# LuoweiZhou/VLP

Hardware: AMD Instinct MI355X
Metric: samples/sec/node (COCO 100-region, seq64, bs64xN) fp16 (higher is better)
Workload: dtype f16; 1 GPU; COCO Captions fine-tune shape: BERT-base 12L, 100 regions x 2048-d, seq_len 64 (L=167), bs 64/GPU, fwd+bwd+FP16 FusedAdam, dropout 0.1, dynamic loss scale; global_batch=64, parallelism=dp1, batch_pool=8, skipped_steps=0, rccl_ranks=1, optimizer=replicated, first_leg_packed=False

## Files before the change

include/vlp_hip.h:

```cpp
#ifndef VLP_HIP_H
#define VLP_HIP_H

#include <stdint.h>

#ifdef __cplusplus
extern "C" {
#endif

#define VLP_ABI_VERSION 5

typedef enum {
    VLP_OK = 0,
    VLP_ERR_BAD_ARG = -1,
    VLP_ERR_HIP = -2,
    VLP_ERR_WORKSPACE = -3
} vlp_status;

enum { VLP_ACT_NONE = 0, VLP_ACT_GELU = 1, VLP_ACT_RELU = 2, VLP_ACT_TANH = 3,
       VLP_ACT_GELU_SAVE_GRAD = 4  };
enum { VLP_MUL_NONE = 0, VLP_MUL_GELU_GRAD = 1, VLP_MUL_RELU_MASK = 2, VLP_MUL_PLAIN = 3  };

int vlp_version(void);
const char* vlp_last_error_string(void);
int vlp_lab_build(void);
void vlp_debug_device_lookup_stats(unsigned long long* lookups, unsigned long long* driver_queries);

typedef struct {
    const void* X; int64_t ldx;
    const void* W; int64_t ldw;
    void* Y; int64_t ldy;
    const void* bias;
    const void* residual; int64_t ldr;
    void* preact; int64_t ldp;
    const void* mul_src; int64_t ldm;
    int32_t M, N, K;
    int32_t act;
    int32_t mul_mode;
    float alpha;
    float dropout_p; uint64_t seed; uint32_t rng_stream;
    int32_t variant;
    const int32_t* row_map;
} vlp_gemm_nt_args;
int vlp_gemm_nt(const vlp_gemm_nt_args* a, void* stream);
int vlp_gemm_nt_resolved_variant(void);
int64_t vlp_gemm_nt_splitk_workspace_bytes(int32_t M, int32_t N, int32_t splits);
int vlp_gemm_nt_splitk(const vlp_gemm_nt_args* a, int32_t splits, void* workspace, int64_t workspace_bytes, void* stream);

typedef struct {
    const void* A; int64_t lda;
    const void* B; int64_t ldb;
    void* C; int64_t ldc;
    int32_t M, N, K;
    int32_t beta;
    void* workspace; int64_t workspace_bytes;
    int32_t variant;
    int32_t splits;
    void* bias_out;
} vlp_gemm_tn_args;
int64_t vlp_gemm_tn_workspace_bytes(int32_t M, int32_t N, int32_t K);
int vlp_gemm_tn(const vlp_gemm_tn_args* a, void* stream);
int vlp_gemm_tn_grouped(const vlp_gemm_tn_args* list, int32_t count, void* stream);
int64_t vlp_gemm_tn_grouped_workspace_bytes(int32_t tiles);

typedef struct {
    const void* A; int64_t lda; int32_t M, N;
    void* out;
    int32_t beta;
    void* workspace; int64_t workspace_bytes;
} vlp_colsum_args;
int64_t vlp_colsum_workspace_bytes(int32_t M, int32_t N);
int vlp_colsum(const vlp_colsum_args* a, void* stream);

typedef struct {
    const void* qkv; int64_t ld_qkv;
    const uint8_t* mask;
    void* ctx; int64_t ld_ctx;
    float* lse;
    int32_t B, L, heads;
    float scale;
    float dropout_p; uint64_t seed; uint32_t rng_stream;
    const int32_t* row_off;
} vlp_attn_fwd_args;
int vlp_attn_fwd(const vlp_attn_fwd_args* a, void* stream);

typedef struct {
    const void* q; int64_t ld_q; int64_t q_rows_per_batch;
    const void* k; const void* v; int64_t ld_kv; int64_t kv_rows_per_batch;
    const uint8_t* mask;
    void* ctx; int64_t ld_ctx;
    int32_t B, Lq, Lk, heads;
    float scale;
    const void* k_prefix; const void* v_prefix;
    int64_t prefix_rows_per_batch;
    int32_t n_prefix, beams;
} vlp_attn_decode_args;
int vlp_attn_decode(const vlp_attn_decode_args* a, void* stream);

typedef struct {
    const void* qkv; int64_t ld_qkv;
    const uint8_t* mask;
    const uint8_t* mask_t;
    const void* ctx; int64_t ld_ctx;
    const void* dctx; int64_t ld_dctx;
    const float* lse;
    void* dqkv; int64_t ld_dqkv;
    float* delta;
    int32_t B, L, heads;
    float scale;
    float dropout_p; uint64_t seed; uint32_t rng_stream;
    const int32_t* row_off;
} vlp_attn_bwd_args;
int vlp_attn_bwd(const vlp_attn_bwd_args* a, void* stream);

int vlp_mask_pack(const int64_t* mask, uint8_t* out, uint8_t* out_t, int32_t B, int32_t L, int32_t Lp, void* stream);

typedef struct {
    const void* x; int64_t ldx;
    const void* gamma; const void* beta;
    void* y; int64_t ldy;
    float* mean; float* rstd;
    int32_t M, H; float eps;
    float dropout_p; uint64_t seed; uint32_t rng_stream;
    const int32_t* row_map;
} vlp_layernorm_fwd_args;
int vlp_layernorm_fwd(const vlp_layernorm_fwd_args* a, void* stream);

typedef struct {
    const void* dy; int64_t lddy;
    const void* x; int64_t ldx;
    const void* gamma;
    const float* mean; const float* rstd;
    void* dx; int64_t lddx;
    void* dx_drop; int64_t lddxd;
    void* dgamma; void* dbeta;
    int32_t M, H; int32_t beta;
    float dy_drop_p; uint64_t dy_seed; uint32_t dy_stream;
    float out_drop_p; uint64_t out_seed; uint32_t out_stream;
    void* workspace; int64_t workspace_bytes;
    int32_t defer_reduce;
    const int32_t* row_map;
} vlp_layernorm_bwd_args;
int64_t vlp_layernorm_bwd_workspace_bytes(int32_t H);
int vlp_layernorm_bwd(const vlp_layernorm_bwd_args* a, void* stream);
int vlp_layernorm_bwd_reduce_batched(const float* parts, const void* const* dst, int32_t count, int32_t M, int32_t H, int32_t beta, void* stream);

int vlp_region_mask_build(const int64_t* vis_masked_pos, int32_t B, int32_t Pm, int32_t Nv, uint8_t* out, void* stream);
typedef struct {
    const void* vis_h; const void* vispe_h;
    const void* pooled;
    const int64_t* vis_masked_pos;
    float* probs;
    float* sample_loss;
    float* loss;
    int32_t B, Nv, Pm, H;
} vlp_pretext_fwd_args;
int vlp_pretext_fwd(const vlp_pretext_fwd_args* a, void* stream);
typedef struct {
    const void* vis_h; const void* vispe_h; const void* pooled;
    const int64_t* vis_masked_pos;
    const float* probs;
    const float* gscale;
    void* d_vis_h; void* d_vispe_h;
    void* d_pooled_pre;
    int32_t B, Nv, Pm, H;
    float drop_p; uint64_t seed; uint32_t vis_stream; uint32_t vispe_stream;
} vlp_pretext_bwd_args;
int vlp_pretext_bwd(const vlp_pretext_bwd_args* a, void* stream);

typedef struct {
    const int64_t* input_ids; const int64_t* segment_ids;
    const void* word_emb; const void* pos_emb; const void* type_emb;
    const void* vis_h; const void* vispe_h;
    void* pre;
    int32_t B, L, Nv, H, vocab, type_vocab;
    const int64_t* position_ids;
    int32_t max_pos;
    const uint8_t* region_mask;
    const int32_t* row_map; int32_t rows;
} vlp_embed_fwd_args;
int vlp_embed_fwd(const vlp_embed_fwd_args* a, void* stream);

int64_t vlp_embed_bwd_workspace_floats(int32_t B, int32_t L, int32_t Nv, int32_t H);
typedef struct {
    const void* dpre;
    const int64_t* input_ids; const int64_t* segment_ids;
    const void* vis_h; const void* vispe_h;
    void* d_word_emb; void* d_pos_emb; void* d_type_emb;
    void* d_vis_h; void* d_vispe_h;
    float* acc32;
    int32_t B, L, Nv, H, vocab, type_vocab;
    float drop_p; uint64_t seed; uint32_t vis_stream; uint32_t vispe_stream;
    const uint8_t* region_mask;
    int32_t parts;
} vlp_embed_bwd_args;
int vlp_embed_bwd(const vlp_embed_bwd_args* a, void* stream);
typedef struct {
// ... 240 lines not shown
```

vlp_amd/_lib.py:

```python
import ctypes as C
import os

import torch

_HERE = os.path.dirname(os.path.abspath(__file__))
LIB_PATH = os.environ.get("VLP_HIP_LIB") or os.path.join(_HERE, "libvlp_hip.so")

ACT_NONE, ACT_GELU, ACT_RELU, ACT_TANH, ACT_GELU_SAVE_GRAD = 0, 1, 2, 3, 4
MUL_NONE, MUL_GELU_GRAD, MUL_RELU_MASK, MUL_PLAIN = 0, 1, 2, 3

vp, i64, i32, f32, u64, u32 = C.c_void_p, C.c_int64, C.c_int32, C.c_float, C.c_uint64, C.c_uint32


class GemmNtArgs(C.Structure):
    _fields_ = [("X", vp), ("ldx", i64), ("W", vp), ("ldw", i64), ("Y", vp), ("ldy", i64), ("bias", vp),
                ("residual", vp), ("ldr", i64), ("preact", vp), ("ldp", i64), ("mul_src", vp), ("ldm", i64),
                ("M", i32), ("N", i32), ("K", i32), ("act", i32), ("mul_mode", i32), ("alpha", f32),
                ("dropout_p", f32), ("seed", u64), ("rng_stream", u32), ("variant", i32), ("row_map", vp)]


class GemmTnArgs(C.Structure):
    _fields_ = [("A", vp), ("lda", i64), ("B", vp), ("ldb", i64), ("C", vp), ("ldc", i64),
                ("M", i32), ("N", i32), ("K", i32), ("beta", i32), ("workspace", vp), ("workspace_bytes", i64),
                ("variant", i32), ("splits", i32), ("bias_out", vp)]


class ColsumArgs(C.Structure):
    _fields_ = [("A", vp), ("lda", i64), ("M", i32), ("N", i32), ("out", vp), ("beta", i32),
                ("workspace", vp), ("workspace_bytes", i64)]


class AttnFwdArgs(C.Structure):
    _fields_ = [("qkv", vp), ("ld_qkv", i64), ("mask", vp), ("ctx", vp), ("ld_ctx", i64), ("lse", vp),
                ("B", i32), ("L", i32), ("heads", i32), ("scale", f32),
                ("dropout_p", f32), ("seed", u64), ("rng_stream", u32), ("row_off", vp)]


class AttnBwdArgs(C.Structure):
    _fields_ = [("qkv", vp), ("ld_qkv", i64), ("mask", vp), ("mask_t", vp), ("ctx", vp), ("ld_ctx", i64), ("dctx", vp), ("ld_dctx", i64),
                ("lse", vp), ("dqkv", vp), ("ld_dqkv", i64), ("delta", vp),
                ("B", i32), ("L", i32), ("heads", i32), ("scale", f32),
                ("dropout_p", f32), ("seed", u64), ("rng_stream", u32), ("row_off", vp)]


class LayerNormFwdArgs(C.Structure):
    _fields_ = [("x", vp), ("ldx", i64), ("gamma", vp), ("beta", vp), ("y", vp), ("ldy", i64), ("mean", vp), ("rstd", vp),
                ("M", i32), ("H", i32), ("eps", f32), ("dropout_p", f32), ("seed", u64), ("rng_stream", u32), ("row_map", vp)]


class LayerNormBwdArgs(C.Structure):
    _fields_ = [("dy", vp), ("lddy", i64), ("x", vp), ("ldx", i64), ("gamma", vp), ("mean", vp), ("rstd", vp),
                ("dx", vp), ("lddx", i64), ("dx_drop", vp), ("lddxd", i64), ("dgamma", vp), ("dbeta", vp),
                ("M", i32), ("H", i32), ("beta", i32),
                ("dy_drop_p", f32), ("dy_seed", u64), ("dy_stream", u32),
                ("out_drop_p", f32), ("out_seed", u64), ("out_stream", u32),
                ("workspace", vp), ("workspace_bytes", i64), ("defer_reduce", i32), ("row_map", vp)]


class EmbedFwdArgs(C.Structure):
    _fields_ = [("input_ids", vp), ("segment_ids", vp), ("word_emb", vp), ("pos_emb", vp), ("type_emb", vp),
                ("vis_h", vp), ("vispe_h", vp), ("pre", vp),
                ("B", i32), ("L", i32), ("Nv", i32), ("H", i32), ("vocab", i32), ("type_vocab", i32),
# ... 66 lines not shown
                ("drop_p", f32), ("seed", u64), ("vis_stream", u32), ("vispe_stream", u32)]


class TransposeDesc(C.Structure):
    _fields_ = [("src", vp), ("dst", vp), ("lds", i64), ("ldd", i64), ("rows", i32), ("cols", i32), ("rows_pad", i32), ("reserved", i32)]


class CiderDArgs(C.Structure):
    _fields_ = [("hyp", vp), ("hyp_ld", i64), ("ref", vp), ("ref_group_stride", i64), ("ref_ld", i64), ("ref_count", vp),
                ("G", i32), ("R", i32), ("T", i32), ("mult", i32), ("sigma", f32), ("scores", vp), ("reward", vp),
                ("workspace", vp), ("workspace_bytes", i64)]


class CiderDDfArgs(C.Structure):
    _fields_ = [("s", CiderDArgs), ("df_keys", vp), ("df_vals", vp), ("df_n", i64), ("n_docs", i64)]


class MlmLossFwdArgs(C.Structure):
    _fields_ = [("logits", vp), ("ld_logits", i64), ("labels", vp), ("weights", vp), ("loss", vp), ("lse", vp), ("coef", vp),
                ("row_loss", vp), ("B", i32), ("P", i32), ("V", i32), ("drop_worst_ratio", f32)]


class MlmLossBwdArgs(C.Structure):
    _fields_ = [("logits", vp), ("ld_logits", i64), ("labels", vp), ("lse", vp), ("coef", vp), ("grad_scale", vp),
                ("dlogits", vp), ("ld_dlogits", i64), ("rows", i32), ("V", i32)]


class MlmLossLsFwdArgs(C.Structure):
    _fields_ = MlmLossFwdArgs._fields_ + [("smooth", f32), ("confidence", f32), ("q_sum", f32), ("q_log_q", f32), ("ignore_index", i32)]


class MlmLossLsBwdArgs(C.Structure):
    _fields_ = MlmLossBwdArgs._fields_ + [("smooth", f32), ("confidence", f32), ("q_sum", f32), ("ignore_index", i32)]


class FusedAdamArgs(C.Structure):
    _fields_ = [("p32", vp), ("m", vp), ("v", vp), ("g16", vp), ("p16", vp), ("n", i64),
                ("b1", f32), ("b2", f32), ("eps", f32), ("decay", f32), ("eps_inside_sqrt", i32), ("hyper", vp)]


class BertAdamArgs(C.Structure):
    _fields_ = [("p32", vp), ("m", vp), ("v", vp), ("g", vp), ("g_is_f32", i32), ("p16", vp),
                ("seg_off", vp), ("ntensors", i32), ("n", i64), ("norms", vp), ("norms_floats", i64),
                ("lr", f32), ("b1", f32), ("b2", f32), ("eps", f32), ("decay", f32), ("max_grad_norm", f32), ("grad_scale", f32),
                ("active", vp)]


SYMBOLS = {
    "vlp_version": (C.c_int, []),
    "vlp_last_error_string": (C.c_char_p, []),
    "vlp_lab_build": (C.c_int, []),
    "vlp_debug_device_lookup_stats": (None, [vp, vp]),
    "vlp_gemm_nt": (C.c_int, [C.POINTER(GemmNtArgs), vp]),
    "vlp_gemm_nt_resolved_variant": (C.c_int, []),
    "vlp_gemm_nt_splitk_workspace_bytes": (C.c_int64, [i32, i32, i32]),
    "vlp_gemm_nt_splitk": (C.c_int, [C.POINTER(GemmNtArgs), i32, vp, i64, vp]),
    "vlp_gemm_tn_workspace_bytes": (i64, [i32, i32, i32]),
    "vlp_gemm_tn": (C.c_int, [C.POINTER(GemmTnArgs), vp]),
    "vlp_gemm_tn_grouped": (C.c_int, [C.POINTER(GemmTnArgs), i32, vp]),
    "vlp_gemm_tn_grouped_workspace_bytes": (i64, [i32]),
    "vlp_colsum_workspace_bytes": (i64, [i32, i32]),
    "vlp_colsum": (C.c_int, [C.POINTER(ColsumArgs), vp]),
    "vlp_attn_fwd": (C.c_int, [C.POINTER(AttnFwdArgs), vp]),
    "vlp_attn_bwd": (C.c_int, [C.POINTER(AttnBwdArgs), vp]),
    "vlp_attn_decode": (C.c_int, [C.POINTER(AttnDecodeArgs), vp]),
    "vlp_mask_pack_rect": (C.c_int, [vp, i64, i64, vp, i32, i32, i32, i32, vp]),
    "vlp_kv_append": (C.c_int, [vp, i64, vp, i32, i32, i32, i32, i32, vp]),
    "vlp_dec_gemm": (C.c_int, [C.POINTER(DecGemmArgs), vp]),
    "vlp_dec_reduce_ln": (C.c_int, [C.POINTER(DecReduceLnArgs), vp]),
    "vlp_argmax_rows2": (C.c_int, [vp, i64, i32, i32, vp, i64, vp, i64, vp, i64, vp]),
    "vlp_logsoftmax_topk": (C.c_int, [vp, i64, i32, i32, i32, vp, i32, i32, vp, vp, vp]),
    "vlp_beam_select": (C.c_int, [C.POINTER(BeamSelectArgs), vp]),
    "vlp_ngram_candidates": (C.c_int, [vp, vp, i32, i32, i32, i32, vp, i32, vp, i64, vp, vp]),
    "vlp_logsoftmax_topk_list": (C.c_int, [vp, i64, i32, i32, i32, vp, i64, vp, i32, i32, vp, vp, vp]),
    "vlp_kv_gather": (C.c_int, [vp, i64, vp, i64, vp, i32, i32, i32, i32, vp]),
    "vlp_embed_bwd_workspace_floats": (C.c_int64, [i32, i32, i32, i32]),
    "vlp_mask_build": (C.c_int, [vp, vp, vp, vp, vp, i32, i32, i32, vp, i32, vp]),
    "vlp_vis_pe_prep": (C.c_int, [C.POINTER(VisPePrepArgs), vp]),
    "vlp_sample_rows": (C.c_int, [vp, i64, i32, i32, C.c_uint64, C.c_uint32, vp, i64, vp, i64, vp]),
    "vlp_argmax_rows": (C.c_int, [vp, i64, i32, i32, vp, i64, vp, i64, vp]),
    "vlp_mask_pack": (C.c_int, [vp, vp, vp, i32, i32, i32, vp]),
    "vlp_layernorm_fwd": (C.c_int, [C.POINTER(LayerNormFwdArgs), vp]),
    "vlp_layernorm_bwd_workspace_bytes": (i64, [i32]),
    "vlp_layernorm_bwd": (C.c_int, [C.POINTER(LayerNormBwdArgs), vp]),
    "vlp_layernorm_bwd_reduce_batched": (C.c_int, [vp, vp, i32, i32, i32, i32, vp]),
    "vlp_embed_fwd": (C.c_int, [C.POINTER(EmbedFwdArgs), vp]),
    "vlp_embed_bwd": (C.c_int, [C.POINTER(EmbedBwdArgs), vp]),
    "vlp_embed_bwd_pos": (C.c_int, [C.POINTER(EmbedBwdPosArgs), vp]),
    "vlp_scst_layout": (C.c_int, [C.POINTER(ScstLayoutArgs), vp]),
    "vlp_token_logprob_fwd": (C.c_int, [C.POINTER(TokenLogprobFwdArgs), vp]),
    "vlp_token_logprob_bwd": (C.c_int, [C.POINTER(TokenLogprobBwdArgs), vp]),
    "vlp_region_mask_build": (C.c_int, [vp, i32, i32, i32, vp, vp]),
    "vlp_pretext_fwd": (C.c_int, [C.POINTER(PretextFwdArgs), vp]),
    "vlp_pretext_bwd": (C.c_int, [C.POINTER(PretextBwdArgs), vp]),
    "vlp_copy2d": (C.c_int, [vp, i64, i32, vp, i64, i32, i32, i32, i32, vp]),
    "vlp_transpose": (C.c_int, [vp, i64, vp, i64, i32, i32, i32, vp]),
    "vlp_transpose_batched": (C.c_int, [vp, vp, i32, i32, vp]),
    "vlp_gather_rows": (C.c_int, [vp, i64, vp, vp, i64, i32, i32, i32, i32, vp, vp]),
    "vlp_scatter_add_rows": (C.c_int, [vp, i64, vp, vp, i64, i32, i32, i32, i32, vp, vp]),
    "vlp_rowmap_build": (C.c_int, [vp, i32, i32, vp, vp]),
    "vlp_rows_unpack": (C.c_int, [vp, i64, vp, i32, vp, i64, i32, vp]),
    "vlp_rows_pack": (C.c_int, [vp, i64, vp, i32, vp, i64, i32, vp]),
    "vlp_vqa_mul_fwd": (C.c_int, [vp, vp, i32, i32, i32, i32, vp, vp]),
    "vlp_vqa_mul_bwd": (C.c_int, [vp, vp, vp, i32, i32, i32, i32, vp, vp]),
    "vlp_relu_dropout_bwd": (C.c_int, [vp, vp, vp, i64, i64, f32, u64, u32, vp]),
    "vlp_gelu_bwd": (C.c_int, [vp, vp, vp, i64, vp]),
    "vlp_cider_d_workspace_bytes": (i64, [i32, i32, i32, i32]),
    "vlp_cider_d": (C.c_int, [C.POINTER(CiderDArgs), vp]),
    "vlp_cider_d_df_workspace_bytes": (i64, [i32, i32, i32, i32]),
    "vlp_cider_d_df": (C.c_int, [C.POINTER(CiderDDfArgs), vp]),
    "vlp_mlm_loss_fwd": (C.c_int, [C.POINTER(MlmLossFwdArgs), vp]),
    "vlp_mlm_loss_bwd": (C.c_int, [C.POINTER(MlmLossBwdArgs), vp]),
    "vlp_mlm_loss_ls_fwd": (C.c_int, [C.POINTER(MlmLossLsFwdArgs), vp]),
    "vlp_mlm_loss_ls_bwd": (C.c_int, [C.POINTER(MlmLossLsBwdArgs), vp]),
    "vlp_bce_loss_fwd": (C.c_int, [vp, i64, vp, i64, i32, i32, vp, vp]),
    "vlp_bce_loss_bwd": (C.c_int, [vp, i64, vp, i64, i32, i32, vp, vp, i64, vp]),
    "vlp_bce_sparse_loss_fwd": (C.c_int, [vp, i64, vp, vp, i32, i32, i32, vp, vp]),
    "vlp_bce_sparse_loss_bwd": (C.c_int, [vp, i64, vp, vp, i32, i32, i32, vp, vp, i64, vp]),
    "vlp_vqa_answer_rows": (C.c_int, [vp, i64, i32, i32, i32, vp, vp, i32, vp, vp, vp, vp]),
    "vlp_sumsq": (C.c_int, [vp, i64, vp, vp, vp]),
    "vlp_sumsq_acc": (C.c_int, [vp, i64, vp, vp, vp]),
    "vlp_fused_adam": (C.c_int, [C.POINTER(FusedAdamArgs), vp]),
    "vlp_adam_hyper": (C.c_int, [vp, vp, vp, f32, f32, vp, vp]),
    "vlp_loss_scale_update": (C.c_int, [vp, vp, vp]),
    "vlp_bert_adam": (C.c_int, [C.POINTER(BertAdamArgs), vp]),
    "vlp_bert_adam_norms_floats": (i64, [i64, i32]),
}

_lib = None


_recording = None


class _Recorder(object):

    def __init__(self, lib, plan):
        self._lib, self._plan = lib, plan

    def __getattr__(self, name):
        fn = getattr(self._lib, name)

        def call(*args):
            self._plan.append((fn, args))
            return fn(*args)
        return call


class record(object):

    def __enter__(self):
        global _recording
# ... 33 lines not shown
    if lib.vlp_version() != 5:
        raise RuntimeError("libvlp_hip.so ABI version mismatch")
    _lib = lib
    return lib


def lab_build():
    return bool(load().vlp_lab_build())


def _check(rc):
    if rc != 0:
        lib = _lib if _lib is not None else load()
        raise RuntimeError("libvlp_hip: %s (status %d)" % (lib.vlp_last_error_string().decode(), rc))


def stream_ptr():
    return C.c_void_p(torch.cuda.current_stream().cuda_stream)


def ptr(t):
    return None if t is None else C.c_void_p(t.data_ptr())


def _nbytes(t):
    return 0 if t is None else t.numel() * t.element_size()


def _req_cuda(*ts):
    for t in ts:
        if t is not None and not t.is_cuda:
            raise RuntimeError("vlp_amd kernels need device tensors (got a CPU tensor); there is no CPU fallback")


def _gemm_nt_args(x, w, y, M, N, K, ldx, ldw, ldy, bias, residual, ldr, preact, ldp, mul_src, ldm, act, mul_mode, alpha, dropout_p, seed, rng_stream,
                  variant=0, row_map=None):
    return GemmNtArgs(ptr(x), ldx if ldx is not None else x.stride(0), ptr(w), ldw if ldw is not None else w.stride(0),
                      ptr(y), ldy if ldy is not None else y.stride(0), ptr(bias),
                      ptr(residual), (ldr if ldr is not None else (residual.stride(0) if residual is not None else 0)),
                      ptr(preact), (ldp if ldp is not None else (preact.stride(0) if preact is not None else 0)),
                      ptr(mul_src), (ldm if ldm is not None else (mul_src.stride(0) if mul_src is not None else 0)),
                      M, N, K, act, mul_mode, alpha, dropout_p, seed, rng_stream, variant, ptr(row_map))


def gemm_nt(x, w, y, M, N, K, ldx=None, ldw=None, ldy=None, bias=None, residual=None, ldr=None, preact=None, ldp=None,
            mul_src=None, ldm=None, act=ACT_NONE, mul_mode=MUL_NONE, alpha=1.0, dropout_p=0.0, seed=0, rng_stream=0,
            variant=0, row_map=None):
    _req_cuda(x, w, y, row_map)
    a = _gemm_nt_args(x, w, y, M, N, K, ldx, ldw, ldy, bias, residual, ldr, preact, ldp, mul_src, ldm, act, mul_mode, alpha, dropout_p, seed,
                      rng_stream, variant, row_map)
    _check(load().vlp_gemm_nt(C.byref(a), stream_ptr()))


def gemm_nt_resolved_variant():
    return int(load().vlp_gemm_nt_resolved_variant())


def gemm_nt_splitk_workspace_bytes(M, N, splits):
    return int(load().vlp_gemm_nt_splitk_workspace_bytes(M, N, splits))


def gemm_nt_splitk(x, w, y, M, N, K, splits, workspace, ldx=None, ldw=None, ldy=None, bias=None, residual=None, ldr=None, preact=None, ldp=None,
                   mul_src=None, ldm=None, act=ACT_NONE, mul_mode=MUL_NONE, alpha=1.0, dropout_p=0.0, seed=0, rng_stream=0):
    _req_cuda(x, w, y, workspace)
    a = _gemm_nt_args(x, w, y, M, N, K, ldx, ldw, ldy, bias, residual, ldr, preact, ldp, mul_src, ldm, act, mul_mode, alpha, dropout_p, seed,
                      rng_stream)
    _check(load().vlp_gemm_nt_splitk(C.byref(a), splits, ptr(workspace), _nbytes(workspace), stream_ptr()))


def gemm_tn_workspace_bytes(M, N, K):
    return int(load().vlp_gemm_tn_workspace_bytes(M, N, K))


def gemm_tn(a_, b_, c_, M, N, K, lda=None, ldb=None, ldc=None, beta=0, workspace=None, variant=0, splits=0, bias_out=None):
    _req_cuda(a_, b_, c_)
    a = GemmTnArgs(ptr(a_), lda if lda is not None else a_.stride(0), ptr(b_), ldb if ldb is not None else b_.stride(0),
                   ptr(c_), ldc if ldc is not None else c_.stride(0), M, N, K, beta,
                   ptr(workspace), _nbytes(workspace), variant, splits,
                   ptr(bias_out))
    _check(load().vlp_gemm_tn(C.byref(a), stream_ptr()))


def gemm_tn_grouped_workspace_bytes(tiles):
    return int(load().vlp_gemm_tn_grouped_workspace_bytes(tiles))


def gemm_tn_grouped(problems, workspace=None):
    arr = (GemmTnArgs * len(problems))()
    for i, (a_, b_, c_, M, N, K, beta, bias_out) in enumerate(problems):
        _req_cuda(a_, b_, c_, bias_out)
        w = workspace if i == 0 else None
        if w is not None:
            _req_cuda(w)
        arr[i] = GemmTnArgs(ptr(a_), a_.stride(0), ptr(b_), b_.stride(0), ptr(c_), c_.stride(0), M, N, K, beta, ptr(w),
                            _nbytes(w), 0, 0, ptr(bias_out))
    _check(load().vlp_gemm_tn_grouped(arr, len(problems), stream_ptr()))


def colsum_workspace_bytes(M, N):
    return int(load().vlp_colsum_workspace_bytes(M, N))


def colsum(a_, out, M, N, lda=None, beta=0, workspace=None):
    _req_cuda(a_, out)
    a = ColsumArgs(ptr(a_), lda if lda is not None else a_.stride(0), M, N, ptr(out), beta, ptr(workspace),
                   _nbytes(workspace))
    _check(load().vlp_colsum(C.byref(a), stream_ptr()))


def attn_fwd(qkv, mask, ctx, lse, B, L, heads, scale, dropout_p=0.0, seed=0, rng_stream=0, row_off=None):
    _req_cuda(qkv, mask, ctx, lse, row_off)
    a = AttnFwdArgs(ptr(qkv), qkv.stride(0), ptr(mask), ptr(ctx), ctx.stride(0), ptr(lse), B, L, heads, scale, dropout_p, seed, rng_stream,
                    ptr(row_off))
    _check(load().vlp_attn_fwd(C.byref(a), stream_ptr()))


def attn_bwd(qkv, mask, mask_t, ctx, dctx, lse, dqkv, delta, B, L, heads, scale, dropout_p=0.0, seed=0, rng_stream=0, row_off=None):
    _req_cuda(qkv, mask, mask_t, ctx, dctx, lse, dqkv, delta, row_off)
    a = AttnBwdArgs(ptr(qkv), qkv.stride(0), ptr(mask), ptr(mask_t), ptr(ctx), ctx.stride(0), ptr(dctx), dctx.stride(0), ptr(lse),
                    ptr(dqkv), dqkv.stride(0), ptr(delta), B, L, heads, scale, dropout_p, seed, rng_stream, ptr(row_off))
    _check(load().vlp_attn_bwd(C.byref(a), stream_ptr()))


def attn_decode(q, ld_q, q_rows, k, v, ld_kv, kv_rows, mask, ctx, B, Lq, Lk, heads, scale, k_prefix=None, v_prefix=None, prefix_rows=0,
                n_prefix=0, beams=1):
    _req_cuda(q, k, v, mask, ctx, k_prefix, v_prefix)
    a = AttnDecodeArgs(ptr(q), ld_q, q_rows, ptr(k), ptr(v), ld_kv, kv_rows, ptr(mask), ptr(ctx), ctx.stride(0), B, Lq, Lk, heads, scale,
                       ptr(k_prefix), ptr(v_prefix), prefix_rows, n_prefix, beams)
    _check(load().vlp_attn_decode(C.byref(a), stream_ptr()))


def dec_gemm(x, w, M, N, Kd, y=None, bias=None, act=0, slab=None, splits=1, kv_cache=None, kv_col0=0, kv_Lcap=0, kv_T=1, kv_start=0,
             residual=None, ln_gamma=None, ln_beta=None, ln_eps=1e-5, ln_out=None):
    _req_cuda(x, w, y, bias, slab, kv_cache, residual, ln_gamma, ln_beta, ln_out)
    a = DecGemmArgs(ptr(x), x.stride(0), ptr(w), w.stride(0), ptr(bias), ptr(y), y.stride(0) if y is not None else 0,
                    ptr(slab), slab.stride(1) if slab is not None else 0, ptr(kv_cache), kv_cache.stride(1) if kv_cache is not None else 0,
                    kv_col0, kv_Lcap, kv_T, kv_start, M, N, Kd, splits, act,
                    ptr(residual), residual.stride(0) if residual is not None else 0, ptr(ln_gamma), ptr(ln_beta), ln_eps,
                    ptr(ln_out), ln_out.stride(0) if ln_out is not None else 0)
    _check(load().vlp_dec_gemm(C.byref(a), stream_ptr()))


def dec_reduce_ln(slab, splits, bias, residual, gamma, beta, y, M, H, eps=1e-5):
    _req_cuda(slab, bias, residual, gamma, beta, y)
    a = DecReduceLnArgs(ptr(slab), slab.stride(1), splits, ptr(bias), ptr(residual), residual.stride(0) if residual is not None else 0,
                        ptr(gamma), ptr(beta), eps, ptr(y), y.stride(0), M, H)
    _check(load().vlp_dec_reduce_ln(C.byref(a), stream_ptr()))


# ... 52 lines not shown
    a = BeamSelectArgs(ptr(kk_scores), ptr(kk_ids), ptr(last_total), ptr(last_eos), ptr(out_scores), ptr(out_ids), ptr(out_ptrs), ptr(out_eos),
                       ptr(src_rows), ptr(next_ids), next_ids.stride(0), B, K, 1 if first else 0, eos_id)
    _check(load().vlp_beam_select(C.byref(a), stream_ptr()))


def kv_gather(src, src_rows, dst, dst_rows, idx, R, lo, hi, row_elems):
    _req_cuda(src, dst, idx)
    _check(load().vlp_kv_gather(ptr(src), src_rows, ptr(dst), dst_rows, ptr(idx), R, lo, hi, row_elems, stream_ptr()))


def mask_build(second_st, second_end, is_s2s, out_u8, B, L, Lp, out_t=None, region_mask=None, Nv=0):
    _req_cuda(second_st, second_end, is_s2s, out_u8, out_t, region_mask)
    for t in (second_st, second_end, is_s2s):
        assert t.dtype == torch.int32 and t.is_contiguous() and t.numel() == B
    _check(load().vlp_mask_build(ptr(second_st), ptr(second_end), ptr(is_s2s), ptr(out_u8), ptr(out_t), B, L, Lp, ptr(region_mask), Nv, stream_ptr()))


def vis_pe_prep(bbox, cls, out, B, Nv, n_cls, pad_to, eps=1e-5):
    _req_cuda(bbox, cls, out)
    assert bbox.dtype == torch.float32 and bbox.is_contiguous() and cls.dtype in (torch.float16, torch.float32) and cls.stride(-1) == 1
    a = VisPePrepArgs(ptr(bbox), ptr(cls), cls.stride(0), ptr(out), out.stride(0), B, Nv, n_cls, pad_to, 1 if cls.dtype == torch.float32 else 0, eps)
    _check(load().vlp_vis_pe_prep(C.byref(a), stream_ptr()))


def sample_rows(logits, ld, rows, V, seed, rng_stream, ids, logp):
    _req_cuda(logits, ids, logp)
    _check(load().vlp_sample_rows(ptr(logits), ld, rows, V, seed, rng_stream, ptr(ids), ids.stride(0), ptr(logp), logp.stride(0), stream_ptr()))


def mask_pack(mask_i64, out_u8, B, L, Lp, out_t=None):
    _req_cuda(mask_i64, out_u8, out_t)
    _check(load().vlp_mask_pack(ptr(mask_i64), ptr(out_u8), ptr(out_t), B, L, Lp, stream_ptr()))


def layernorm_fwd(x, gamma, beta, y, M, H, mean=None, rstd=None, eps=1e-5, dropout_p=0.0, seed=0, rng_stream=0, ldx=None, ldy=None, row_map=None):
    _req_cuda(x, gamma, beta, y, row_map)
    a = LayerNormFwdArgs(ptr(x), ldx if ldx is not None else x.stride(0), ptr(gamma), ptr(beta), ptr(y),
                         ldy if ldy is not None else y.stride(0), ptr(mean), ptr(rstd), M, H, eps, dropout_p, seed, rng_stream, ptr(row_map))
    _check(load().vlp_layernorm_fwd(C.byref(a), stream_ptr()))


def layernorm_bwd_workspace_bytes(H):
    return int(load().vlp_layernorm_bwd_workspace_bytes(H))


def layernorm_bwd(dy, x, gamma, mean, rstd, dx, dgamma, dbeta, M, H, workspace, beta=0, dx_drop=None,
                  dy_drop=(0.0, 0, 0), out_drop=(0.0, 0, 0), defer_reduce=False, row_map=None):
    _req_cuda(dy, x, gamma, mean, rstd, dx, dgamma, dbeta, workspace, row_map)
    a = LayerNormBwdArgs(ptr(dy), dy.stride(0), ptr(x), x.stride(0), ptr(gamma), ptr(mean), ptr(rstd), ptr(dx), dx.stride(0),
                         ptr(dx_drop), dx_drop.stride(0) if dx_drop is not None else 0, ptr(dgamma), ptr(dbeta), M, H, beta,
                         dy_drop[0], dy_drop[1], dy_drop[2], out_drop[0], out_drop[1], out_drop[2],
                         ptr(workspace), _nbytes(workspace), 1 if defer_reduce else 0, ptr(row_map))
    _check(load().vlp_layernorm_bwd(C.byref(a), stream_ptr()))


def layernorm_bwd_reduce_batched(parts, dst_table, count, M, H, beta=0):
    _req_cuda(parts, dst_table)
    _check(load().vlp_layernorm_bwd_reduce_batched(ptr(parts), ptr(dst_table), count, M, H, beta, stream_ptr()))


def embed_fwd(input_ids, segment_ids, word_emb, pos_emb, type_emb, vis_h, vispe_h, pre, B, L, Nv, H, position_ids=None, region_mask=None,
              row_map=None, rows=0):
    _req_cuda(input_ids, segment_ids, word_emb, pos_emb, type_emb, pre, position_ids, region_mask, row_map)
    a = EmbedFwdArgs(ptr(input_ids), ptr(segment_ids), ptr(word_emb), ptr(pos_emb), ptr(type_emb), ptr(vis_h), ptr(vispe_h),
                     ptr(pre), B, L, Nv, H, word_emb.shape[0], type_emb.shape[0], ptr(position_ids), pos_emb.shape[0], ptr(region_mask),
                     ptr(row_map), rows)
    _check(load().vlp_embed_fwd(C.byref(a), stream_ptr()))


def embed_bwd_workspace_floats(B, L, Nv, H):
    return int(load().vlp_embed_bwd_workspace_floats(B, L, Nv, H))


def _embed_bwd_args(dpre, input_ids, segment_ids, vis_h, vispe_h, d_word, d_pos, d_type, d_vis_h, d_vispe_h, acc32,
                    B, L, Nv, H, vocab, type_vocab, drop_p, seed, vis_stream, vispe_stream, region_mask, parts):
    _req_cuda(dpre, input_ids, segment_ids, d_word, d_pos, d_type, acc32, region_mask)
    return EmbedBwdArgs(ptr(dpre), ptr(input_ids), ptr(segment_ids), ptr(vis_h), ptr(vispe_h), ptr(d_word), ptr(d_pos), ptr(d_type),
                        ptr(d_vis_h), ptr(d_vispe_h), ptr(acc32), B, L, Nv, H, vocab, type_vocab, drop_p, seed, vis_stream, vispe_stream,
                        ptr(region_mask), parts)


def embed_bwd(dpre, input_ids, segment_ids, vis_h, vispe_h, d_word, d_pos, d_type, d_vis_h, d_vispe_h, acc32,
              B, L, Nv, H, vocab, type_vocab, drop_p=0.0, seed=0, vis_stream=0, vispe_stream=0, region_mask=None, parts=0):
    a = _embed_bwd_args(dpre, input_ids, segment_ids, vis_h, vispe_h, d_word, d_pos, d_type, d_vis_h, d_vispe_h, acc32,
                        B, L, Nv, H, vocab, type_vocab, drop_p, seed, vis_stream, vispe_stream, region_mask, parts)
    _check(load().vlp_embed_bwd(C.byref(a), stream_ptr()))


def embed_bwd_pos(dpre, input_ids, segment_ids, position_ids, vis_h, vispe_h, d_word, d_pos, d_type, d_vis_h, d_vispe_h, acc32,
                  B, L, Nv, H, vocab, type_vocab, drop_p=0.0, seed=0, vis_stream=0, vispe_stream=0, region_mask=None, parts=0):
    _req_cuda(position_ids)
    base = _embed_bwd_args(dpre, input_ids, segment_ids, vis_h, vispe_h, d_word, d_pos, d_type, d_vis_h, d_vispe_h, acc32,
                           B, L, Nv, H, vocab, type_vocab, drop_p, seed, vis_stream, vispe_stream, region_mask, parts)
    a = EmbedBwdPosArgs(base, ptr(position_ids), d_pos.shape[0])
    _check(load().vlp_embed_bwd_pos(C.byref(a), stream_ptr()))


def scst_layout(prefix_ids, sample_ids, segment_ids, position_ids, mask, out_ids, out_segment_ids, out_position_ids, out_mask, masked_pos,
                mask_word_id):
    _req_cuda(prefix_ids, sample_ids, segment_ids, position_ids, mask, out_ids, out_segment_ids, out_position_ids, out_mask, masked_pos)
    B, in_len = prefix_ids.shape
    T, L = sample_ids.shape[1], segment_ids.shape[1]
    for t in (prefix_ids, sample_ids, segment_ids, position_ids, mask, out_ids, out_segment_ids, out_position_ids, out_mask, masked_pos):
        if t.dtype != torch.long or not t.is_contiguous():
            raise RuntimeError("vlp_amd.scst_layout: operands must be contiguous int64")
    Lo = in_len + 2 * T - 1
# ... 72 lines not shown
    _req_cuda(vis_h, vispe_h, pooled, vis_masked_pos, probs, sample_loss, loss)
    a = PretextFwdArgs(ptr(vis_h), ptr(vispe_h), ptr(pooled), ptr(vis_masked_pos), ptr(probs), ptr(sample_loss), ptr(loss), B, Nv, Pm, H)
    _check(load().vlp_pretext_fwd(C.byref(a), stream_ptr()))


def pretext_bwd(vis_h, vispe_h, pooled, vis_masked_pos, probs, gscale, d_vis_h, d_vispe_h, d_pooled_pre, B, Nv, Pm, H,
                drop_p=0.0, seed=0, vis_stream=0, vispe_stream=0):
    _req_cuda(vis_h, vispe_h, pooled, vis_masked_pos, probs, gscale, d_vis_h, d_vispe_h, d_pooled_pre)
    a = PretextBwdArgs(ptr(vis_h), ptr(vispe_h), ptr(pooled), ptr(vis_masked_pos), ptr(probs), ptr(gscale), ptr(d_vis_h), ptr(d_vispe_h),
                       ptr(d_pooled_pre), B, Nv, Pm, H, drop_p, seed, vis_stream, vispe_stream)
    _check(load().vlp_pretext_bwd(C.byref(a), stream_ptr()))


def copy2d(src, lds, src_f32, dst, ldd, rows, cols_src, cols_dst, beta=0):
    _req_cuda(src, dst)
    _check(load().vlp_copy2d(ptr(src), lds, int(src_f32), ptr(dst), ldd, rows, cols_src, cols_dst, beta, stream_ptr()))


def transpose(src, lds, dst, ldd, rows, cols, rows_pad):
    _req_cuda(src, dst)
    _check(load().vlp_transpose(ptr(src), lds, ptr(dst), ldd, rows, cols, rows_pad, stream_ptr()))


def make_transpose_batch(items, device):
    import numpy as np
    arr = (TransposeDesc * len(items))()
    starts, tot = [], 0
    for i, (src, lds, dst, ldd, rows, cols, rows_pad) in enumerate(items):
        _req_cuda(src, dst)
        arr[i] = TransposeDesc(src.data_ptr(), dst.data_ptr(), lds, ldd, rows, cols, rows_pad, 0)
        starts.append(tot)
        tot += ((rows_pad + 63) // 64) * ((cols + 63) // 64)
    raw = np.frombuffer(bytes(arr), dtype=np.uint8).copy()
    descs = torch.from_numpy(raw).to(device)
    ts = torch.tensor(starts, dtype=torch.int32, device=device)
    return descs, ts, len(items), tot


def transpose_batched(batch):
    descs, ts, n, tot = batch
    _check(load().vlp_transpose_batched(ptr(descs), ptr(ts), n, tot, stream_ptr()))


def gather_rows(src, lds, pos, out, ldo, B, P, L, H, row_off=None):
    _req_cuda(src, pos, out, row_off)
    _check(load().vlp_gather_rows(ptr(src), lds, ptr(pos), ptr(out), ldo, B, P, L, H, ptr(row_off), stream_ptr()))


def scatter_add_rows(src, lds, pos, dst, ldd, B, P, L, H, row_off=None):
    _req_cuda(src, pos, dst, row_off)
    _check(load().vlp_scatter_add_rows(ptr(src), lds, ptr(pos), ptr(dst), ldd, B, P, L, H, ptr(row_off), stream_ptr()))


def rowmap_build(row_off, B, L, row_map):
    _req_cuda(row_off, row_map)
    _check(load().vlp_rowmap_build(ptr(row_off), B, L, ptr(row_map), stream_ptr()))


def rows_unpack(src, row_map, rows, dst, H):
    _req_cuda(src, row_map, dst)
    _check(load().vlp_rows_unpack(ptr(src), src.stride(0), ptr(row_map), rows, ptr(dst), dst.stride(0), H, stream_ptr()))


def rows_pack(src, row_map, rows, dst, H):
    _req_cuda(src, row_map, dst)
    _check(load().vlp_rows_pack(ptr(src), src.stride(0), ptr(row_map), rows, ptr(dst), dst.stride(0), H, stream_ptr()))


def vqa_mul_fwd(h, out, B, L, Nv, H, row_off=None):
    _req_cuda(h, out, row_off)
    _check(load().vlp_vqa_mul_fwd(ptr(h), ptr(out), B, L, Nv, H, ptr(row_off), stream_ptr()))


def vqa_mul_bwd(h, dout, dh, B, L, Nv, H, row_off=None):
    _req_cuda(h, dout, dh, row_off)
    _check(load().vlp_vqa_mul_bwd(ptr(h), ptr(dout), ptr(dh), B, L, Nv, H, ptr(row_off), stream_ptr()))


def relu_dropout_bwd(dy, y, dz, n, ncols, drop_p=0.0, seed=0, rng_stream=0):
    _req_cuda(dy, y, dz)
    _check(load().vlp_relu_dropout_bwd(ptr(dy), ptr(y), ptr(dz), n, ncols, drop_p, seed, rng_stream, stream_ptr()))


def gelu_bwd(dy, z, dz, n):
    _req_cuda(dy, z, dz)
    _check(load().vlp_gelu_bwd(ptr(dy), ptr(z), ptr(dz), n, stream_ptr()))


def mlm_loss_fwd(logits, ld, labels, weights, loss, lse, coef, row_loss, B, P, V, drop_worst_ratio=0.0):
    _req_cuda(logits, labels, weights, loss, lse, coef, row_loss)
    a = MlmLossFwdArgs(ptr(logits), ld, ptr(labels), ptr(weights), ptr(loss), ptr(lse), ptr(coef), ptr(row_loss), B, P, V, drop_worst_ratio)
    _check(load().vlp_mlm_loss_fwd(C.byref(a), stream_ptr()))


def mlm_loss_bwd(logits, ld, labels, lse, coef, grad_scale, dlogits, ldd, rows, V):
    _req_cuda(logits, labels, lse, coef, grad_scale, dlogits)
    a = MlmLossBwdArgs(ptr(logits), ld, ptr(labels), ptr(lse), ptr(coef), ptr(grad_scale), ptr(dlogits), ldd, rows, V)
    _check(load().vlp_mlm_loss_bwd(C.byref(a), stream_ptr()))


def mlm_loss_ls_fwd(logits, ld, labels, weights, loss, lse, coef, row_loss, B, P, V, smooth, confidence, q_sum, q_log_q, ignore_index=0,
                    drop_worst_ratio=0.0):
    _req_cuda(logits, labels, weights, loss, lse, coef, row_loss)
    a = MlmLossLsFwdArgs(ptr(logits), ld, ptr(labels), ptr(weights), ptr(loss), ptr(lse), ptr(coef), ptr(row_loss), B, P, V, drop_worst_ratio,
                         smooth, confidence, q_sum, q_log_q, ignore_index)
    _check(load().vlp_mlm_loss_ls_fwd(C.byref(a), stream_ptr()))
# ... 87 lines not shown
```

vlp_amd/csrc/elementwise.hip:

```cpp
#include <hip/hip_fp16.h>
#include "vocab_row.h"

__global__ __launch_bounds__(256) void embed_fwd_kernel(vlp_embed_fwd_args a) {
    const int nch = a.H >> 3;
    const int64_t total = (a.row_map ? (int64_t)a.rows : (int64_t)a.B * a.L) * nch;
    const f16* word = (const f16*)a.word_emb;
    const f16* pos = (const f16*)a.pos_emb;
    const f16* typ = (const f16*)a.type_emb;
    const f16* vis = (const f16*)a.vis_h;
    const f16* vpe = (const f16*)a.vispe_h;
    f16* pre = (f16*)a.pre;
    for (int64_t i = (int64_t)blockIdx.x * blockDim.x + threadIdx.x; i < total; i += (int64_t)gridDim.x * blockDim.x) {
        const int c = (int)(i % nch);
        const int64_t prow = i / nch;
        const int64_t row = a.row_map ? (int64_t)a.row_map[prow] : prow;
        const int l = (int)(row % a.L);
        const int b = (int)(row / a.L);
        f16x8 w, p;
        if (l >= 1 && l <= a.Nv) {
            const int64_t vr = (int64_t)b * a.Nv + (l - 1);
            if (a.region_mask && a.region_mask[vr]) {
#pragma unroll
                for (int e = 0; e < 8; ++e) { w[e] = (f16)0.f; p[e] = (f16)0.f; }
            } else {
// ... 372 lines not shown

DEVFN int64_t sample_base(const int32_t* row_off, int64_t b, int L, int& n) {
    if (row_off) { const int lo = row_off[b]; n = row_off[b + 1] - lo; return lo; }
    n = L;
    return b * L;
}
__global__ void gather_rows_kernel(const f16* src, int64_t lds, const int64_t* pos, f16* out, int64_t ldo, int B, int P, int L, int H, const int32_t* row_off) {
    const int nch = H >> 3;
    const int64_t total = (int64_t)B * P * nch;
    for (int64_t i = (int64_t)blockIdx.x * blockDim.x + threadIdx.x; i < total; i += (int64_t)gridDim.x * blockDim.x) {
        const int c = (int)(i % nch);
        const int64_t r = i / nch;
        int n;
        const int64_t base = sample_base(row_off, r / P, L, n);
        int64_t ps = pos[r];
        ps = ps < 0 ? 0 : (ps >= n ? n - 1 : ps);
        st8(out + r * ldo + c * 8, ld8(src + (base + ps) * lds + c * 8));
    }
}
extern "C" int vlp_gather_rows(const void* src, int64_t lds, const int64_t* pos, void* out, int64_t ldo, int32_t B, int32_t P, int32_t L,
                               int32_t H, const int32_t* row_off, void* stream) {
    VLP_CHECK_ARG(src && pos && out && B > 0 && P > 0 && L > 0 && H % 8 == 0 && lds % 8 == 0 && ldo % 8 == 0, "vlp_gather_rows: bad args");
    VLP_ENTER(src, "vlp_gather_rows");
    const int64_t total = (int64_t)B * P * (H / 8);
    hipLaunchKernelGGL(gather_rows_kernel, dim3((int)((total + 255) / 256)), dim3(256), 0, (hipStream_t)stream, (const f16*)src, lds, pos,
                       (f16*)out, ldo, B, P, L, H, row_off);
    VLP_CHECK_LAUNCH("vlp_gather_rows");
    return VLP_OK;
}
__global__ void scatter_add_rows_kernel(const f16* src, int64_t lds, const int64_t* pos, f16* dst, int64_t ldd, int B, int P, int L, int H, const int32_t* row_off) {
    const int nch = H >> 3;
    const int64_t total = (int64_t)B * P * nch;
    for (int64_t i = (int64_t)blockIdx.x * blockDim.x + threadIdx.x; i < total; i += (int64_t)gridDim.x * blockDim.x) {
        const int c = (int)(i % nch);
        const int64_t r = i / nch;
        int n;
        const int64_t base = sample_base(row_off, r / P, L, n);
        int64_t ps = pos[r];
        ps = ps < 0 ? 0 : (ps >= n ? n - 1 : ps);
        const f16x8 v = ld8(src + r * lds + c * 8);
        __half2* d = reinterpret_cast<__half2*>(dst + (base + ps) * ldd + c * 8);
#pragma unroll
        for (int e = 0; e < 4; ++e) unsafeAtomicAdd(d + e, __floats2half2_rn((float)v[2 * e], (float)v[2 * e + 1]));
    }
}
extern "C" int vlp_scatter_add_rows(const void* src, int64_t lds, const int64_t* pos, void* dst, int64_t ldd, int32_t B, int32_t P, int32_t L,
                                    int32_t H, const int32_t* row_off, void* stream) {
    VLP_CHECK_ARG(src && pos && dst && B > 0 && P > 0 && L > 0 && H % 8 == 0 && lds % 8 == 0 && ldd % 8 == 0, "vlp_scatter_add_rows: bad args");
    VLP_ENTER(src, "vlp_scatter_add_rows");
    const int64_t total = (int64_t)B * P * (H / 8);
    hipLaunchKernelGGL(scatter_add_rows_kernel, dim3((int)((total + 255) / 256)), dim3(256), 0, (hipStream_t)stream, (const f16*)src, lds,
                       pos, (f16*)dst, ldd, B, P, L, H, row_off);
    VLP_CHECK_LAUNCH("vlp_scatter_add_rows");
    return VLP_OK;
}

__global__ void vqa_mul_fwd_kernel(const f16* h, f16* out, int B, int L, int Nv, int H, const int32_t* row_off) {
    const int64_t total = (int64_t)B * H;
    for (int64_t i = (int64_t)blockIdx.x * blockDim.x + threadIdx.x; i < total; i += (int64_t)gridDim.x * blockDim.x) {
        const int64_t b = i / H;
        const int c = (int)(i % H);
        const int64_t r0 = row_off ? (int64_t)row_off[b] : b * L;
        const float a0 = (float)h[r0 * H + c], a1 = (float)h[(r0 + Nv + 1) * H + c];
        out[i] = (f16)(a0 * a1);
    }
}
extern "C" int vlp_vqa_mul_fwd(const void* h, void* out, int32_t B, int32_t L, int32_t Nv, int32_t H, const int32_t* row_off, void* stream) {
    VLP_CHECK_ARG(h && out && B > 0 && Nv + 1 < L, "vlp_vqa_mul_fwd: bad args");
    VLP_ENTER(h, "vlp_vqa_mul_fwd");
    hipLaunchKernelGGL(vqa_mul_fwd_kernel, dim3(cdiv((int64_t)B * H, 256)), dim3(256), 0, (hipStream_t)stream, (const f16*)h, (f16*)out, B, L, Nv, H, row_off);
    VLP_CHECK_LAUNCH("vlp_vqa_mul_fwd");
    return VLP_OK;
}
__global__ void vqa_mul_bwd_kernel(const f16* h, const f16* dout, f16* dh, int B, int L, int Nv, int H, const int32_t* row_off) {
    const int64_t total = (int64_t)B * H;
    for (int64_t i = (int64_t)blockIdx.x * blockDim.x + threadIdx.x; i < total; i += (int64_t)gridDim.x * blockDim.x) {
        const int64_t b = i / H;
        const int c = (int)(i % H);
        const int64_t r0 = row_off ? (int64_t)row_off[b] : b * L;
        const int64_t i0 = r0 * H + c, i1 = (r0 + Nv + 1) * H + c;
        const float d = (float)dout[i], a0 = (float)h[i0], a1 = (float)h[i1];
        dh[i0] = (f16)((float)dh[i0] + d * a1);
        dh[i1] = (f16)((float)dh[i1] + d * a0);
    }
}
extern "C" int vlp_vqa_mul_bwd(const void* h, const void* dout, void* dh, int32_t B, int32_t L, int32_t Nv, int32_t H, const int32_t* row_off, void* stream) {
    VLP_CHECK_ARG(h && dout && dh && B > 0 && Nv + 1 < L, "vlp_vqa_mul_bwd: bad args");
    VLP_ENTER(h, "vlp_vqa_mul_bwd");
    hipLaunchKernelGGL(vqa_mul_bwd_kernel, dim3(cdiv((int64_t)B * H, 256)), dim3(256), 0, (hipStream_t)stream, (const f16*)h, (const f16*)dout,
                       (f16*)dh, B, L, Nv, H, row_off);
    VLP_CHECK_LAUNCH("vlp_vqa_mul_bwd");
    return VLP_OK;
}

__global__ void rowmap_build_kernel(const int32_t* row_off, int L, int32_t* row_map) {
    const int b = blockIdx.x;
    const int lo = row_off[b], n = row_off[b + 1] - lo;
    for (int l = threadIdx.x; l < n; l += blockDim.x) row_map[lo + l] = b * L + l;
}
extern "C" int vlp_rowmap_build(const int32_t* row_off, int32_t B, int32_t L, int32_t* row_map, void* stream) {
    VLP_CHECK_ARG(row_off && row_map && B > 0 && L > 0, "vlp_rowmap_build: bad args");
    VLP_ENTER(row_off, "vlp_rowmap_build");
    hipLaunchKernelGGL(rowmap_build_kernel, dim3(B), dim3(256), 0, (hipStream_t)stream, row_off, L, row_map);
    VLP_CHECK_LAUNCH("vlp_rowmap_build");
    return VLP_OK;
}
// ... 646 lines not shown
```

vlp_amd/csrc/gemm_nt.hip:

```cpp
#include "common.h"
#include "gemm_nt.h"
#include "gemm_nt_epilogue.h"

#define BM 128
#define BK 64


#ifdef VLP_NT_DEBUG
__device__ unsigned long long g_nt_trace[4096 * 4];
#define NT_TRACE(slot) do { if (wid == 0 && lane == 0 && blockIdx.x < 4096) g_nt_trace[blockIdx.x * 4 + (slot)] = wall_clock64(); } while (0)
extern "C" int vlp_debug_read_nt_trace(void* dst, int64_t bytes) { return (int)hipMemcpyFromSymbol(dst, HIP_SYMBOL(g_nt_trace), bytes); }
#else
#define NT_TRACE(slot) do { } while (0)
#endif
DEVFN int swz_x(int r) { return r & 7; }
DEVFN int swz_w(int r) { return (((r >> 4) & 3) << 1) | ((r >> 1) & 1); }

template <int VARIANT, int BM_T, int BN_T, bool SG, int NSR = 0, int EPI = 0>
__global__ __launch_bounds__((BM_T / 64) * (BN_T / 64) * 64, (VARIANT == 3 ? (BN_T == 256 ? 4 : BM_T / 128) : ((VARIANT == 2 || BN_T == 256) ? 4 : 2))) void gemm_nt_kernel(GemmNtParams p) {
    extern __shared__ __attribute__((aligned(16))) char smem_raw[];
    f16* smem = reinterpret_cast<f16*>(smem_raw);
    constexpr int WN_ = BN_T / 64;
    constexpr int T = (BM_T / 64) * WN_ * 64;
    constexpr int RPP = T / 8;
    constexpr int XP = BM_T / RPP;
    constexpr int WP = BN_T / RPP;
    constexpr int XT = BM_T * BK, WT = BN_T * BK;
    const int tid = threadIdx.x;
    const int lane = tid & 63;
    const int wid = __builtin_amdgcn_readfirstlane(tid >> 6);
    const int wm = wid / WN_, wn = wid % WN_;
    const int g = lane >> 4, li = lane & 15;

    int bid = blockIdx.x;
    if (p.xcd_remap) {
        const int nb = gridDim.x, q = nb >> 3, r = nb & 7, xcd = bid & 7, loc = bid >> 3;
        bid = (xcd < r ? xcd * (q + 1) : r * (q + 1) + (xcd - r) * q) + loc;
    }
    const int tile_m = bid / p.tiles_n;
    const int tile_n = bid % p.tiles_n;
    const int m0 = tile_m * BM_T, n0 = tile_n * BN_T;

    const int srow = tid >> 3;
    const int sx = tid & 7;
    const f16* xsrc[XP];
    const f16* wsrc[WP];
    int lds_off[XP];
#pragma unroll
    for (int i = 0; i < XP; ++i) {
        const int r = srow + RPP * i;
        const int mr = min(m0 + r, p.M - 1);
        xsrc[i] = p.X + (int64_t)mr * p.ldx + (sx ^ swz_x(r)) * 8;
        lds_off[i] = r * BK + sx * 8;
    }
#pragma unroll
    for (int i = 0; i < WP; ++i) {
        const int r = srow + RPP * i;
        const int nr = min(n0 + r, p.N - 1);
        wsrc[i] = p.W + (int64_t)nr * p.ldw + (sx ^ swz_w(r)) * 8;
    }

    f32x4 acc[4][4];
#pragma unroll
    for (int a = 0; a < 4; ++a)
#pragma unroll
        for (int b = 0; b < 4; ++b) acc[a][b] = (f32x4){0.f, 0.f, 0.f, 0.f};

#ifdef VLP_NT_DEBUG
    if ((p.dbg >> 8) && ((blockIdx.x >> 3) & 1) && blockIdx.x < 256) {
        const uint64_t t0 = wall_clock64();
        while (wall_clock64() - t0 < (uint64_t)(p.dbg >> 8) * 10u) __builtin_amdgcn_s_sleep(8);
    }
#endif
    const int nk = p.K / BK;
    NT_TRACE(0);

    int xrow[4], wrow[4];
#pragma unroll
    for (int t = 0; t < 4; ++t) {
        xrow[t] = wm * 64 + 16 * t + li;
        wrow[t] = wn * 64 + 16 * (li >> 2) + 4 * t + (li & 3);
    }

    u32x4 xreg[XP], wreg[WP];

    auto gload = [&](int kt) {
#pragma unroll
        for (int i = 0; i < XP; ++i) xreg[i] = *reinterpret_cast<const u32x4*>(xsrc[i] + (int64_t)kt * BK);
#pragma unroll
        for (int i = 0; i < WP; ++i) wreg[i] = *reinterpret_cast<const u32x4*>(wsrc[i] + (int64_t)kt * BK);
    };
    auto lstore = [&](int buf) {
        f16* xs = smem + buf * (XT + WT);
        f16* ws = xs + XT;
#pragma unroll
        for (int i = 0; i < XP; ++i) *reinterpret_cast<u32x4*>(xs + lds_off[i]) = xreg[i];
#pragma unroll
        for (int i = 0; i < WP; ++i) *reinterpret_cast<u32x4*>(ws + lds_off[i]) = wreg[i];
    };
    const uint32_t smem_lds = lds_addr_of(smem);
    auto glds = [&](int kt, int buf) {
        const uint32_t xs = smem_lds + (uint32_t)(buf * (XT + WT)) * 2u;
        const uint32_t ws = xs + (uint32_t)XT * 2u;
#ifdef VLP_NT_DEBUG
// ... 140 lines not shown
    }

    NT_TRACE(1);
#ifdef VLP_NT_DEBUG
    if ((p.dbg & 4) && acc[0][0][0] != 12345.678f) return;
#endif
    const int ncol0 = n0 + wn * 64 + 16 * g;
    const bool full_n = (ncol0 + 16 <= p.N);
    float bias_v[16];
#pragma unroll
    for (int j = 0; j < 16; ++j) bias_v[j] = 0.f;
    if (p.bias) {
        if (full_n) {
            f16x8 b0 = ld8(p.bias + ncol0), b1 = ld8(p.bias + ncol0 + 8);
#pragma unroll
            for (int j = 0; j < 8; ++j) { bias_v[j] = (float)b0[j]; bias_v[8 + j] = (float)b1[j]; }
        } else {
#pragma unroll
            for (int j = 0; j < 16; ++j) if (ncol0 + j < p.N) bias_v[j] = (float)p.bias[ncol0 + j];
        }
    }
    if constexpr (EPI == 1) {
        if (ncol0 >= p.N) return;
        f16x8 mv[4][2];
#pragma unroll
        for (int tm = 0; tm < 4; ++tm) {
            const int mc = min(m0 + wm * 64 + 16 * tm + li, p.M - 1);
#pragma unroll
            for (int h = 0; h < 2; ++h) mv[tm][h] = ld8(p.mulsrc + (int64_t)mc * p.ldm + ncol0 + 8 * h);
        }
#pragma unroll
        for (int tm = 0; tm < 4; ++tm) {
            const int m = m0 + wm * 64 + 16 * tm + li;
            if (m >= p.M) continue;
#pragma unroll
            for (int h = 0; h < 2; ++h) {
                f16x8 o;
#pragma unroll
                for (int j = 0; j < 8; ++j) {
                    const int c = 8 * h + j;
                    float vj = acc[tm][c >> 2][c & 3] * p.alpha + bias_v[c];
                    vj *= (float)mv[tm][h][j];
                    o[j] = (f16)vj;
                }
                ST8_OUT(p, p.Y + (int64_t)m * p.ldy + ncol0 + 8 * h, o);
            }
        }
        return;
    }
#pragma unroll
    for (int tm = 0; tm < 4; ++tm) {
        const int m = m0 + wm * 64 + 16 * tm + li;
        if (m >= p.M) continue;
        const uint32_t rkey = p.drop.thresh ? drop_rowkey(p.drop, nt_drop_row(p, m)) : 0u;
        float v[16];
#pragma unroll
        for (int tn = 0; tn < 4; ++tn)
#pragma unroll
            for (int r = 0; r < 4; ++r) v[tn * 4 + r] = acc[tm][tn][r] * p.alpha + bias_v[tn * 4 + r];
#pragma unroll
        for (int h = 0; h < 2; ++h)
            nt_epilogue8<SG>(p, m, ncol0 + 8 * h, v + 8 * h, rkey, true);
    }
#ifdef VLP_NT_DEBUG
    NT_TRACE(2);
    asm volatile("s_waitcnt vmcnt(0)" ::: "memory");
    NT_TRACE(3);
#endif
}

int vlp_gemm_nt_fill_params(const vlp_gemm_nt_args* a, GemmNtParams& p) {
    VLP_CHECK_ARG(a != nullptr, "vlp_gemm_nt: null args");
    VLP_CHECK_ARG(a->X && a->W && a->Y, "vlp_gemm_nt: null operand");
    VLP_CHECK_ARG(a->M > 0 && a->N > 0 && a->K > 0, "vlp_gemm_nt: bad shape M=%d N=%d K=%d", a->M, a->N, a->K);
    VLP_CHECK_ARG(a->K % BK == 0, "vlp_gemm_nt: K=%d must be a multiple of %d (pad with vlp_copy2d)", a->K, BK);
    VLP_CHECK_ARG(a->ldx % 8 == 0 && a->ldw % 8 == 0 && a->ldy % 8 == 0, "vlp_gemm_nt: leading dims must be multiples of 8 halfs");
    VLP_CHECK_ARG(a->ldx >= a->K && a->ldw >= a->K, "vlp_gemm_nt: ldx/ldw < K");
    const int n8 = (a->N + 7) / 8 * 8;
    VLP_CHECK_ARG(a->ldy >= n8, "vlp_gemm_nt: ldy=%lld < roundup8(N)=%d", (long long)a->ldy, n8);
    VLP_CHECK_ARG(((uintptr_t)a->X | (uintptr_t)a->W | (uintptr_t)a->Y) % 16 == 0, "vlp_gemm_nt: operands must be 16-byte aligned");
    if (a->residual) VLP_CHECK_ARG(a->ldr % 8 == 0 && a->ldr >= n8 && (uintptr_t)a->residual % 16 == 0, "vlp_gemm_nt: bad residual layout");
    if (a->preact) VLP_CHECK_ARG(a->ldp % 8 == 0 && a->ldp >= n8 && (uintptr_t)a->preact % 16 == 0, "vlp_gemm_nt: bad preact layout");
    if (a->mul_mode != VLP_MUL_NONE)
        VLP_CHECK_ARG(a->mul_src && a->ldm % 8 == 0 && a->ldm >= n8 && (uintptr_t)a->mul_src % 16 == 0, "vlp_gemm_nt: bad mul_src layout");
    if (a->bias) VLP_CHECK_ARG((uintptr_t)a->bias % 16 == 0, "vlp_gemm_nt: bias must be 16-byte aligned");
    VLP_CHECK_ARG(a->act >= VLP_ACT_NONE && a->act <= VLP_ACT_GELU_SAVE_GRAD, "vlp_gemm_nt: bad act %d", a->act);
    VLP_CHECK_ARG(a->act != VLP_ACT_GELU_SAVE_GRAD || a->preact, "vlp_gemm_nt: VLP_ACT_GELU_SAVE_GRAD needs `preact` (receives gelu'(z))");
    VLP_CHECK_ARG(a->mul_mode >= VLP_MUL_NONE && a->mul_mode <= VLP_MUL_PLAIN, "vlp_gemm_nt: bad mul_mode %d", a->mul_mode);
    VLP_CHECK_ARG(a->dropout_p >= 0.f && a->dropout_p < 1.f, "vlp_gemm_nt: bad dropout p");

    p.X = (const f16*)a->X; p.ldx = a->ldx;
    p.W = (const f16*)a->W; p.ldw = a->ldw;
    p.Y = (f16*)a->Y; p.ldy = a->ldy;
    p.bias = (const f16*)a->bias;
    p.residual = (const f16*)a->residual; p.ldr = a->ldr;
    p.preact = (f16*)a->preact; p.ldp = a->ldp;
    p.mulsrc = (const f16*)a->mul_src; p.ldm = a->ldm;
    p.M = a->M; p.N = a->N; p.K = a->K;
    p.act = a->act; p.mulmode = a->mul_mode;
    p.alpha = a->alpha;
    p.drop = make_drop(a->dropout_p, a->seed, a->rng_stream);
    p.row_map = a->row_map;
    p.tiles_n = 0;
    p.xcd_remap = 0;
#ifdef VLP_NT_DEBUG
    { const char* e = getenv("VLP_NT_DEBUG"); p.dbg = e ? atoi(e) : 0; }
#endif
    return VLP_OK;
}

static thread_local int t_last_variant = -1;
extern "C" int vlp_gemm_nt_resolved_variant(void) { return t_last_variant; }

extern "C" int vlp_gemm_nt(const vlp_gemm_nt_args* a, void* stream) {
    VLP_ENTER(a ? a->X : nullptr, "vlp_gemm_nt");
    GemmNtParams p;
    const int frc = vlp_gemm_nt_fill_params(a, p);
    if (frc != VLP_OK) return frc;
    hipStream_t s = (hipStream_t)stream;
#define LAUNCH_NT_(V, BMT, BNT, NBUF, SGV, NSRV)                                                                  \
    do {                                                                                                                \
// ... 32 lines not shown
        return VLP_OK;
    }
    if (variant & 64) {
        const int rc = vlp_gemm_nt_wp_launch(p, (variant & 7) + ((variant & 128) ? 8 : 0), sg, s);
        if (rc != VLP_OK) return rc;
        VLP_CHECK_LAUNCH("vlp_gemm_nt");
        return VLP_OK;
    }
    switch (variant & 7) {
#ifdef VLP_LAB_BUILD
        case 6: case 7: {
            const int rc = vlp_gemm_nt_ph_launch(p, (variant & 7) == 6 ? 256 : 128, (variant >> 4) & 3, s);
            if (rc != VLP_OK) return rc;
            break;
        }
#endif
        case 0: LAUNCH_NT(0, 128, 128, 2); break;
        case 1: if (variant & 16) LAUNCH_NT(3, 128, 128, 4); else LAUNCH_NT(1, 128, 128, 2); break;
        case 3:
            if (variant & 16) LAUNCH_NT(3, 256, 128, 3);
            else LAUNCH_NT(1, 256, 128, 2);
            break;
        case 2: LAUNCH_NT(2, 128, 128, 1); break;
        case 4: LAUNCH_NT(2, 256, 128, 1); break;
        case 5:
#ifdef VLP_LAB_BUILD
            if ((variant & 48) == 48) { const int rc = vlp_gemm_nt_k32_launch(p, sg, s); if (rc != VLP_OK) return rc; }
            else
#endif
            if (variant & 16) {
                static const int lean_on = [] { const char* e = getenv("VLP_NT_LEAN_EPI"); return (e && e[0] == '0') ? 0 : 1; }();
                const bool lean = lean_on && !sg && p.act == VLP_ACT_NONE && !p.preact && p.mulmode == VLP_MUL_PLAIN && !p.drop.thresh && !p.residual &&
                                  p.N % 16 == 0 && p.ldm % 8 == 0 && ((uintptr_t)p.mulsrc & 15) == 0;
                if (lean) {
                    const size_t smem = (size_t)2 * (256 + 256) * BK * sizeof(f16);
                    VLP_ONCE_PER_DEVICE((void)hipFuncSetAttribute((const void*)gemm_nt_kernel<3, 256, 256, false, 2, 1>, hipFuncAttributeMaxDynamicSharedMemorySize, (int)smem));
                    p.tiles_n = cdiv(a->N, 256);
                    hipLaunchKernelGGL((gemm_nt_kernel<3, 256, 256, false, 2, 1>), dim3(cdiv(a->M, 256) * p.tiles_n), dim3(1024), smem, s, p);
                } else {
                    LAUNCH_RING(256, 256, 2);
                }
            }
            else LAUNCH_NT(1, 256, 256, 2);
            break;
        default: LAUNCH_NT(1, 128, 128, 2); break;
    }
#undef LAUNCH_RING
#undef LAUNCH_NT
#undef LAUNCH_NT_
    VLP_CHECK_LAUNCH("vlp_gemm_nt");
    return VLP_OK;
}

extern "C" int vlp_gemm_nt_splitk(const vlp_gemm_nt_args* a, int32_t splits, void* workspace, int64_t workspace_bytes, void* stream) {
    VLP_ENTER(a ? a->X : nullptr, "vlp_gemm_nt_splitk");
    GemmNtParams p;
    const int frc = vlp_gemm_nt_fill_params(a, p);
    if (frc != VLP_OK) return frc;
    VLP_CHECK_ARG(a->act != VLP_ACT_GELU_SAVE_GRAD, "vlp_gemm_nt_splitk: VLP_ACT_GELU_SAVE_GRAD is not provided (training-shape kernels only)");
    return vlp_gemm_nt_splitk_launch(p, splits, (float*)workspace, workspace_bytes, (hipStream_t)stream);
}
```

vlp_amd/csrc/gemm_nt_epilogue.h:

```cpp
#pragma once
#include "gemm_nt.h"

#ifdef VLP_NT_DEBUG
DEVFN void st8_pol(const GemmNtParams& p, f16* dst, f16x8 v) {
    if (p.dbg & 32) __builtin_nontemporal_store(v, reinterpret_cast<f16x8*>(dst));
    else if (p.dbg & 64) asm volatile("global_store_dwordx4 %0, %1, off sc1" ::"v"(dst), "v"(v) : "memory");
    else st8(dst, v);
}
#define ST8_OUT(p, dst, v) st8_pol(p, dst, v)
#else
#define ST8_OUT(p, dst, v) st8_out<VLP_SS_NT>(dst, v)
#endif
static inline bool nt_epilogue_is_light(const GemmNtParams& p) {
    return (p.act == VLP_ACT_NONE || p.act == VLP_ACT_RELU) && p.mulmode != VLP_MUL_GELU_GRAD;
}
template <bool SG = false, bool LIGHT = false>
DEVFN void nt_epilogue8(const GemmNtParams& p, int m, int nc, float* vv, uint32_t rkey, bool bias_done = false) {
    if (nc >= p.N) return;
    if (p.bias && !bias_done) {
        if (nc + 8 <= p.N) {
            const f16x8 b = ld8(p.bias + nc);
#pragma unroll
            for (int j = 0; j < 8; ++j) vv[j] += (float)b[j];
        } else {
#pragma unroll
            for (int j = 0; j < 8; ++j) if (nc + j < p.N) vv[j] += (float)p.bias[nc + j];
        }
    }
    if (SG) {
        f16x8 d, o;
#pragma unroll
        for (int j = 0; j < 8; ++j) {
            float gl, gp;
            gelu_and_grad_f((float)(f16)vv[j], gl, gp);
            o[j] = (f16)gl;
            d[j] = (f16)gp;
        }
        if ((p.N & 7) && nc + 8 > p.N) {
#pragma unroll
            for (int j = 0; j < 8; ++j)
                if (nc + j >= p.N) { o[j] = (f16)0.f; d[j] = (f16)0.f; }
        }
        st8_out<VLP_SS_SAVED>(p.preact + (int64_t)m * p.ldp + nc, d);
        ST8_OUT(p, p.Y + (int64_t)m * p.ldy + nc, o);
        return;
    } else {
        if (p.preact) {
            f16x8 z;
#pragma unroll
            for (int j = 0; j < 8; ++j) z[j] = (nc + j < p.N) ? (f16)vv[j] : (f16)0.f;
            st8_out<VLP_SS_SAVED>(p.preact + (int64_t)m * p.ldp + nc, z);
#pragma unroll
            for (int j = 0; j < 8; ++j) vv[j] = (float)z[j];
        }
        if (!LIGHT && p.act == VLP_ACT_GELU) {
#pragma unroll
            for (int j = 0; j < 8; ++j) vv[j] = gelu_f(vv[j]);
        } else if (p.act == VLP_ACT_RELU) {
#pragma unroll
            for (int j = 0; j < 8; ++j) vv[j] = fmaxf(vv[j], 0.f);
        } else if (!LIGHT && p.act == VLP_ACT_TANH) {
#pragma unroll
            for (int j = 0; j < 8; ++j) vv[j] = tanhf(vv[j]);
        }
    }
    if (p.mulmode != VLP_MUL_NONE) {
        const f16x8 s = ld8(p.mulsrc + (int64_t)m * p.ldm + nc);
        if (!LIGHT && p.mulmode == VLP_MUL_GELU_GRAD) {
#pragma unroll
            for (int j = 0; j < 8; ++j) vv[j] *= gelu_grad_f((float)s[j]);
        } else if (p.mulmode == VLP_MUL_PLAIN) {
#pragma unroll
            for (int j = 0; j < 8; ++j) vv[j] *= (float)s[j];
        } else {
#pragma unroll
            for (int j = 0; j < 8; ++j) vv[j] = ((float)s[j] > 0.f) ? vv[j] : 0.f;
        }
    }
    if (p.drop.thresh) {
        drop_mult8(p.drop, rkey, (uint32_t)nc, vv);
    }
    if (p.residual) {
        const f16x8 r = ld8(p.residual + (int64_t)m * p.ldr + nc);
#pragma unroll
        for (int j = 0; j < 8; ++j) vv[j] += (float)r[j];
    }
    f16x8 o;
#pragma unroll
    for (int j = 0; j < 8; ++j) o[j] = (nc + j < p.N) ? (f16)vv[j] : (f16)0.f;
    ST8_OUT(p, p.Y + (int64_t)m * p.ldy + nc, o);
}
```

vlp_amd/csrc/gemm_tn.hip:

```cpp
#include "common.h"
#include <cstdlib>

#define TN_BN 128
#define TN_BK 128
#define TN_BM 64
#define TN_THREADS 256
#define TN_PITCH (128 + 8)

struct GemmTnParams {
    const f16* A; int64_t lda;
    const f16* B; int64_t ldb;
    f16* C; int64_t ldc;
    float* slab;
    float* bias_slab;
    f16* bias_out;
    int M, N, K, beta, splits, rows_per_split;
    int tiles_k, tiles_n, xcd_remap, split_major;
};

typedef __fp16 fp16x4_t __attribute__((__vector_size__(4 * sizeof(__fp16))));

DEVFN f16x4 lds_tr_read(const f16* p) {
    fp16x4_t t = __builtin_amdgcn_ds_read_tr16_b64_v4f16((__attribute__((address_space(3))) fp16x4_t*)(p));
    return __builtin_bit_cast(f16x4, t);
}

template <int VARIANT>
__global__ __launch_bounds__(TN_THREADS, 2) void gemm_tn_kernel(GemmTnParams p) {
    extern __shared__ __attribute__((aligned(16))) char smem_raw[];
    f16* smem = reinterpret_cast<f16*>(smem_raw);
    const int TILE = TN_BM * TN_PITCH;
    const int tid = threadIdx.x;
    const int lane = tid & 63;
    const int wid = __builtin_amdgcn_readfirstlane(tid >> 6);
    const int wn = wid >> 1, wk = wid & 1;
    const int g = lane >> 4, li = lane & 15;

    int bid = blockIdx.x;
    if (p.xcd_remap) {
        const int nb = gridDim.x, q = nb >> 3, r = nb & 7, xcd = bid & 7, loc = bid >> 3;
        bid = (xcd < r ? xcd * (q + 1) : r * (q + 1) + (xcd - r) * q) + loc;
    }
    int split, ktile, ntile;
    if (p.split_major) {
        ktile = bid % p.tiles_k;
        ntile = (bid / p.tiles_k) % p.tiles_n;
        split = bid / (p.tiles_k * p.tiles_n);
    } else {
        split = bid % p.splits;
        ktile = (bid / p.splits) % p.tiles_k;
        ntile = bid / (p.splits * p.tiles_k);
    }
    const int n0 = ntile * TN_BN;
    const int k0 = ktile * TN_BK;
    const int m_begin = split * p.rows_per_split;
    const int m_end = min(p.M, m_begin + p.rows_per_split);
    const int nstages = (m_end - m_begin + TN_BM - 1) / TN_BM;

    const int srow = tid >> 4, sch = tid & 15;
    const bool a_ok = (n0 + sch * 8) < p.N;
    const bool b_ok = (k0 + sch * 8) < p.K;

    f32x4 acc[4][4];
#pragma unroll
    for (int a = 0; a < 4; ++a)
#pragma unroll
        for (int b = 0; b < 4; ++b) acc[a][b] = (f32x4){0.f, 0.f, 0.f, 0.f};
    const bool do_bias = (p.bias_out != nullptr) && ktile == 0 && wk == 0;
    f32x4 bacc[4];
#pragma unroll
// ... 61 lines not shown
        }
    };

    if (nstages > 0) {
        gload(0);
        lstore(0);
        __syncthreads();
        for (int st = 0; st < nstages; ++st) {
            const int buf = st & 1;
            if (st + 1 < nstages) gload(st + 1);
            compute(buf);
            if (st + 1 < nstages) lstore(buf ^ 1);
            __syncthreads();
        }
    }

    const int kc0 = k0 + wk * 64 + 16 * g;
#pragma unroll
    for (int tn = 0; tn < 4; ++tn) {
        const int n = n0 + wn * 64 + 16 * tn + li;
        if (n >= p.N) continue;
        if (do_bias && g == 0) {
            if (p.splits > 1) p.bias_slab[(int64_t)split * p.N + n] = bacc[tn][0];
            else p.bias_out[n] = (f16)(p.beta ? (float)p.bias_out[n] + bacc[tn][0] : bacc[tn][0]);
        }
        if (p.splits > 1) {
            float* dst = p.slab + ((int64_t)split * p.N + n) * p.K + kc0;
#pragma unroll
            for (int tk = 0; tk < 4; ++tk)
                if (kc0 + 4 * tk < p.K) *reinterpret_cast<f32x4*>(dst + 4 * tk) = acc[tn][tk];
        } else {
            f16* dst = p.C + (int64_t)n * p.ldc + kc0;
#pragma unroll
            for (int h = 0; h < 2; ++h) {
                if (kc0 + 8 * h >= p.K) continue;
                f16x8 o;
                if (p.beta) o = ld8(dst + 8 * h);
#pragma unroll
                for (int j = 0; j < 8; ++j) {
                    float v = acc[tn][2 * h + (j >> 2)][j & 3];
                    o[j] = (f16)(p.beta ? (float)o[j] + v : v);
                }
                st8_out<VLP_SS_TN>(dst + 8 * h, o);
            }
        }
    }
}

DEVFN int tn_swz(int r) { return ((r & 3) | (((r >> 3) & 1) << 2)) << 1; }

#define TN_SK_WRITE 1
#define TN_SK_FINAL 2
#define TN_SK_SLOTS 20
template <int BN_T, int BK_T, int NS = 2, int BM_T = TN_BM, bool SK = false>
DEVFN void tn_glds_tile(const GemmTnParams& p, int bid, f16* smem, int sk_m_begin = 0, int sk_m_end = 0, int sk_role = 0, float* sk_part = nullptr,
                        int* sk_flag = nullptr) {
    constexpr int WK_ = BK_T / 64;
    constexpr int T = (BN_T / 64) * WK_ * 64;
    constexpr int ATILE = BM_T * BN_T, BTILE = BM_T * BK_T;
    constexpr int ACH = BN_T / 8, BCH = BK_T / 8;
    constexpr int AP = BM_T * ACH / T, BP = BM_T * BCH / T;
    constexpr int ARP = T / ACH, BRP = T / BCH;
    const int tid = threadIdx.x;
    const int lane = tid & 63;
    const int wid = __builtin_amdgcn_readfirstlane(tid >> 6);
    const int wn = wid / WK_, wk = wid % WK_;
    const int g = lane >> 4, li = lane & 15;

    int split, ktile, ntile;
    if (p.split_major) {
        ktile = bid % p.tiles_k;
        ntile = (bid / p.tiles_k) % p.tiles_n;
        split = bid / (p.tiles_k * p.tiles_n);
    } else {
        split = bid % p.splits;
        ktile = (bid / p.splits) % p.tiles_k;
        ntile = bid / (p.splits * p.tiles_k);
    }
    const int n0 = ntile * BN_T;
    const int k0 = ktile * BK_T;
    const int m_begin = SK ? sk_m_begin : split * p.rows_per_split;
    const int m_end = SK ? sk_m_end : min(p.M, m_begin + p.rows_per_split);
    const int nstages = (m_end - m_begin + BM_T - 1) / BM_T;

    const int arow = tid / ACH, apc = tid % ACH, brow = tid / BCH, bpc = tid % BCH;
    int acol[AP], bcol[BP];
#pragma unroll
    for (int i = 0; i < AP; ++i) acol[i] = min(n0 + (apc ^ tn_swz(arow + ARP * i)) * 8, (int)p.lda - 8);
#pragma unroll
    for (int i = 0; i < BP; ++i) bcol[i] = min(k0 + (bpc ^ tn_swz(brow + BRP * i)) * 8, (int)p.ldb - 8);

    f32x4 acc[4][4];
#pragma unroll
    for (int a = 0; a < 4; ++a)
#pragma unroll
        for (int b = 0; b < 4; ++b) acc[a][b] = (f32x4){0.f, 0.f, 0.f, 0.f};
    const bool do_bias = (p.bias_out != nullptr) && ktile == 0 && wk == 0;
    f32x4 bacc[4];
#pragma unroll
    for (int a = 0; a < 4; ++a) bacc[a] = (f32x4){0.f, 0.f, 0.f, 0.f};
    const f16x8 ones = (f16x8){(f16)1.f, (f16)1.f, (f16)1.f, (f16)1.f, (f16)1.f, (f16)1.f, (f16)1.f, (f16)1.f};

    const uint32_t smem_lds = lds_addr_of(smem);
    const f16* asrc[AP];
    const f16* bsrc[BP];
#pragma unroll
    for (int i = 0; i < AP; ++i) asrc[i] = p.A + (int64_t)(m_begin + arow + ARP * i) * p.lda + acol[i];
#pragma unroll
    for (int i = 0; i < BP; ++i) bsrc[i] = p.B + (int64_t)(m_begin + brow + BRP * i) * p.ldb + bcol[i];
    auto stage = [&](int st, int buf) {
        f16* as = smem + buf * (ATILE + BTILE);
        f16* bs = as + ATILE;
        const int mbase = m_begin + st * BM_T;
        if (mbase + BM_T <= m_end) {
            const uint32_t as_l = smem_lds + (uint32_t)(buf * (ATILE + BTILE)) * 2u, bs_l = as_l + (uint32_t)ATILE * 2u;
            const int64_t aoff = (int64_t)st * BM_T * p.lda, boff = (int64_t)st * BM_T * p.ldb;
#pragma unroll
            for (int i = 0; i < AP; ++i) glds16(asrc[i] + aoff, as_l + (uint32_t)((ARP * i) * BN_T + wid * 512) * 2u);
#pragma unroll
            for (int i = 0; i < BP; ++i) glds16(bsrc[i] + boff, bs_l + (uint32_t)((BRP * i) * BK_T + wid * 512) * 2u);
        } else {
#pragma unroll
            for (int i = 0; i < AP; ++i) {
                const int r = arow + ARP * i, m = mbase + r;
                u32x4 v = (u32x4){0, 0, 0, 0};
                if (m < m_end) v = *reinterpret_cast<const u32x4*>(p.A + (int64_t)m * p.lda + acol[i]);
                *reinterpret_cast<u32x4*>(as + r * BN_T + apc * 8) = v;
            }
#pragma unroll
            for (int i = 0; i < BP; ++i) {
                const int r = brow + BRP * i, m = mbase + r;
                u32x4 v = (u32x4){0, 0, 0, 0};
                if (m < m_end) v = *reinterpret_cast<const u32x4*>(p.B + (int64_t)m * p.ldb + bcol[i]);
                *reinterpret_cast<u32x4*>(bs + r * BK_T + bpc * 8) = v;
            }
        }
    };
    auto read_frags = [&](int buf, int ms, f16x8 (&xf)[4], f16x8 (&yf)[4]) {
        const f16* as = smem + buf * (ATILE + BTILE);
        const f16* bs = as + ATILE;
        const int r0 = ms * 32 + 8 * g + (li >> 2);
        const int sw = tn_swz(r0);
#pragma unroll
        for (int t = 0; t < 4; ++t) {
            const int cx = wk * 64 + 16 * t + 4 * (li & 3), cy = wn * 64 + 16 * t + 4 * (li & 3);
            const f16* px = bs + r0 * BK_T + (((cx >> 3) ^ sw) << 3) + (cx & 4);
            const f16* py = as + r0 * BN_T + (((cy >> 3) ^ sw) << 3) + (cy & 4);
            const u32x2 x0 = __builtin_bit_cast(u32x2, lds_tr_read(px)), x1 = __builtin_bit_cast(u32x2, lds_tr_read(px + 4 * BK_T));
            const u32x2 y0 = __builtin_bit_cast(u32x2, lds_tr_read(py)), y1 = __builtin_bit_cast(u32x2, lds_tr_read(py + 4 * BN_T));
            xf[t] = __builtin_bit_cast(f16x8, (u32x4){x0[0], x0[1], x1[0], x1[1]});
            yf[t] = __builtin_bit_cast(f16x8, (u32x4){y0[0], y0[1], y1[0], y1[1]});
        }
    };
    auto mfma_frags = [&](const f16x8 (&xf)[4], const f16x8 (&yf)[4]) {
#pragma unroll
        for (int tn = 0; tn < 4; ++tn)
#pragma unroll
            for (int tk = 0; tk < 4; ++tk)
                acc[tn][tk] = __builtin_amdgcn_mfma_f32_16x16x32_f16(xf[tk], yf[tn], acc[tn][tk], 0, 0, 0);
        if (do_bias) {
#pragma unroll
            for (int tn = 0; tn < 4; ++tn) bacc[tn] = __builtin_amdgcn_mfma_f32_16x16x32_f16(ones, yf[tn], bacc[tn], 0, 0, 0);
        }
    };

    if (nstages > 0) {
        constexpr int LPS = AP + BP;
#pragma unroll
        for (int i = 0; i < NS - 1; ++i)
            if (i < nstages) stage(i, i);
        int buf = 0, nbuf = NS - 1;
        const bool tail_ragged = ((m_end - m_begin) % BM_T) != 0;
        for (int st = 0; st < nstages; ++st) {
            const int left = nstages - 1 - st;
            int younger = left < NS - 2 ? left : NS - 2;
            if (tail_ragged && st + younger >= nstages - 1) younger = 0;
            if (NS >= 4 && younger == 2) asm volatile("s_waitcnt vmcnt(%0) lgkmcnt(0)" ::"n"(2 * LPS) : "memory");
            else if (NS >= 3 && younger >= 1) asm volatile("s_waitcnt vmcnt(%0) lgkmcnt(0)" ::"n"(LPS) : "memory");
            else asm volatile("s_waitcnt vmcnt(0) lgkmcnt(0)" ::: "memory");
            __builtin_amdgcn_s_barrier();
            f16x8 x0[4], y0[4], x1[4], y1[4];
            read_frags(buf, 0, x0, y0);
            __builtin_amdgcn_sched_barrier(0);
            if (st + NS - 1 < nstages) stage(st + NS - 1, nbuf);
            if (BM_T == 64) read_frags(buf, 1, x1, y1);
            __builtin_amdgcn_sched_barrier(0);
            mfma_frags(x0, y0);
            if (BM_T == 64) mfma_frags(x1, y1);
            buf = (buf + 1 == NS) ? 0 : buf + 1;
            nbuf = (nbuf + 1 == NS) ? 0 : nbuf + 1;
        }
    }

    if (SK) {
        f32x4* part = reinterpret_cast<f32x4*>(sk_part) + tid;
        if (sk_role == TN_SK_WRITE) {
#pragma unroll
            for (int tn = 0; tn < 4; ++tn)
#pragma unroll
                for (int tk = 0; tk < 4; ++tk) part[(tn * 4 + tk) * T] = acc[tn][tk];
            if (do_bias) {
#pragma unroll
                for (int tn = 0; tn < 4; ++tn) part[(16 + tn) * T] = bacc[tn];
            }
            __syncthreads();
            return;
        }
        if (tid == 0) {
            while (__hip_atomic_load(sk_flag, __ATOMIC_RELAXED, __HIP_MEMORY_SCOPE_AGENT) == 0) __builtin_amdgcn_s_sleep(8);
            __builtin_amdgcn_fence(__ATOMIC_ACQUIRE, "agent");
        }
        __syncthreads();
#pragma unroll
        for (int tn = 0; tn < 4; ++tn)
#pragma unroll
            for (int tk = 0; tk < 4; ++tk) acc[tn][tk] += part[(tn * 4 + tk) * T];
        if (do_bias) {
#pragma unroll
            for (int tn = 0; tn < 4; ++tn) bacc[tn] += part[(16 + tn) * T];
        }
    }
#pragma unroll
    for (int tn = 0; tn < 4; ++tn) {
        const int n = n0 + wn * 64 + 16 * tn + li;
        if (n >= p.N) continue;
        if (do_bias && g == 0) {
            if (p.splits > 1) p.bias_slab[(int64_t)split * p.N + n] = bacc[tn][0];
            else p.bias_out[n] = (f16)(p.beta ? (float)p.bias_out[n] + bacc[tn][0] : bacc[tn][0]);
        }
#pragma unroll
        for (int tk = 0; tk < 4; ++tk) {
            const int kc = k0 + wk * 64 + 16 * tk + 4 * g;
            if (kc >= p.K) continue;
            if (p.splits > 1) {
                *reinterpret_cast<f32x4*>(p.slab + ((int64_t)split * p.N + n) * p.K + kc) = acc[tn][tk];
            } else {
                f16* dst = p.C + (int64_t)n * p.ldc + kc;
                f16x4 o;
                if (p.beta) o = ld4(dst);
#pragma unroll
                for (int j = 0; j < 4; ++j) o[j] = (f16)(p.beta ? (float)o[j] + acc[tn][tk][j] : acc[tn][tk][j]);
                st4_out<VLP_SS_TN>(dst, o);
            }
        }
    }
}

DEVFN int tn_xcd_remap(int bid, int nb) {
    const int q = nb >> 3, r = nb & 7, xcd = bid & 7, loc = bid >> 3;
    return (xcd < r ? xcd * (q + 1) : r * (q + 1) + (xcd - r) * q) + loc;
}

template <int BN_T, int BK_T>
__global__ __launch_bounds__((BN_T / 64) * (BK_T / 64) * 64, 2) void gemm_tn_glds_kernel(GemmTnParams p) {
    extern __shared__ __attribute__((aligned(16))) char smem_raw[];
    int bid = blockIdx.x;
    if (p.xcd_remap) bid = tn_xcd_remap(bid, gridDim.x);
    tn_glds_tile<BN_T, BK_T>(p, bid, reinterpret_cast<f16*>(smem_raw));
}

#define TN_GROUP_MAX 8
struct TnGroupEntry {
    const f16* A; int64_t lda;
    const f16* B; int64_t ldb;
    f16* C; int64_t ldc;
    f16* bias_out;
    int M, N, K, beta, tiles_k, tile_begin;
};
struct TnGroupParams {
    TnGroupEntry e[TN_GROUP_MAX];
    int count, total_tiles, xcd_remap;
    int nst, tail;
};

template <int BN_T, int BK_T, int NS, int BM_T>
__global__ __launch_bounds__((BN_T / 64) * (BK_T / 64) * 64, 2) void gemm_tn_grouped_kernel(TnGroupParams gp) {
    extern __shared__ __attribute__((aligned(16))) char smem_raw[];
    int bid = blockIdx.x;
    if (gp.xcd_remap) bid = tn_xcd_remap(bid, gridDim.x);
    int j = 0;
#pragma unroll
    for (int i = 1; i < TN_GROUP_MAX; ++i)
        if (i < gp.count && bid >= gp.e[i].tile_begin) j = i;
    const TnGroupEntry& e = gp.e[j];
    GemmTnParams p;
    p.A = e.A; p.lda = e.lda; p.B = e.B; p.ldb = e.ldb; p.C = e.C; p.ldc = e.ldc;
    p.slab = nullptr; p.bias_slab = nullptr; p.bias_out = e.bias_out;
    p.M = e.M; p.N = e.N; p.K = e.K; p.beta = e.beta; p.splits = 1; p.rows_per_split = (e.M + TN_BM - 1) / TN_BM * TN_BM;
    p.tiles_k = e.tiles_k; p.tiles_n = 0; p.xcd_remap = 0; p.split_major = 0;
    tn_glds_tile<BN_T, BK_T, NS, BM_T>(p, bid - e.tile_begin, reinterpret_cast<f16*>(smem_raw));
}

#ifdef VLP_LAB_BUILD
template <int BN_T, int BK_T, int NS, int BM_T>
__global__ __launch_bounds__((BN_T / 64) * (BK_T / 64) * 64, 2) void gemm_tn_grouped_sk_kernel(TnGroupParams gp, float* part, int* flags) {
    extern __shared__ __attribute__((aligned(16))) char smem_raw[];
    constexpr int T = (BN_T / 64) * (BK_T / 64) * 64;
    int u = blockIdx.x;
    if (gp.xcd_remap) u = tn_xcd_remap(u, gridDim.x);
    const int grp = u / 7, j = u % 7;
    const int nst = gp.nst, cut = gp.nst - gp.tail;
    const int nseg = (j < 6) ? 1 : 6;
    for (int seg = 0; seg < nseg; ++seg) {
        const int tile = 6 * grp + ((j < 6) ? j : seg);
        int ei = 0;
#pragma unroll
        for (int i = 1; i < TN_GROUP_MAX; ++i)
            if (i < gp.count && tile >= gp.e[i].tile_begin) ei = i;
        const TnGroupEntry& e = gp.e[ei];
        GemmTnParams p;
        p.A = e.A; p.lda = e.lda; p.B = e.B; p.ldb = e.ldb; p.C = e.C; p.ldc = e.ldc;
        p.slab = nullptr; p.bias_slab = nullptr; p.bias_out = e.bias_out;
        p.M = e.M; p.N = e.N; p.K = e.K; p.beta = e.beta; p.splits = 1; p.rows_per_split = 0;
        p.tiles_k = e.tiles_k; p.tiles_n = 0; p.xcd_remap = 0; p.split_major = 0;
        if (j < 6)
            tn_glds_tile<BN_T, BK_T, NS, BM_T, true>(p, tile - e.tile_begin, reinterpret_cast<f16*>(smem_raw), 0, cut * BM_T, TN_SK_FINAL,
                                                       part + (int64_t)tile * (TN_SK_SLOTS * T * 4), flags + grp);
        else
            tn_glds_tile<BN_T, BK_T, NS, BM_T, true>(p, tile - e.tile_begin, reinterpret_cast<f16*>(smem_raw), cut * BM_T, min(e.M, nst * BM_T), TN_SK_WRITE,
                                                       part + (int64_t)tile * (TN_SK_SLOTS * T * 4), flags + grp);
    }
    if (j == 6) {
        asm volatile("s_waitcnt vmcnt(0)" ::: "memory");
        __syncthreads();
        if (threadIdx.x == 0) {
            __builtin_amdgcn_fence(__ATOMIC_RELEASE, "agent");
            asm volatile("s_waitcnt vmcnt(0)" ::: "memory");
            __hip_atomic_store(flags + grp, 1, __ATOMIC_RELAXED, __HIP_MEMORY_SCOPE_AGENT);
        }
    }
}

#endif

__global__ void gemm_tn_reduce_kernel(const float* slab, f16* C, int64_t ldc, int N, int K, int splits, int beta,
                                      const float* bias_slab, f16* bias_out, int main_blocks) {
    if ((int)blockIdx.x >= main_blocks) {
        const int n = ((int)blockIdx.x - main_blocks) * blockDim.x + threadIdx.x;
        if (n < N) {
            float s = 0.f;
            for (int sp = 0; sp < splits; ++sp) s += bias_slab[(int64_t)sp * N + n];
            bias_out[n] = (f16)(beta ? (float)bias_out[n] + s : s);
        }
        return;
    }
    const int64_t total8 = (int64_t)N * (K / 8);
    const int64_t stride = (int64_t)N * K;
    for (int64_t i = (int64_t)blockIdx.x * blockDim.x + threadIdx.x; i < total8; i += (int64_t)main_blocks * blockDim.x) {
        const int n = (int)(i / (K / 8));
        const int k = (int)(i % (K / 8)) * 8;
        const float* s = slab + (int64_t)n * K + k;
        float v[8];
        f32x4 a0 = *reinterpret_cast<const f32x4*>(s), a1 = *reinterpret_cast<const f32x4*>(s + 4);
#pragma unroll
        for (int j = 0; j < 4; ++j) { v[j] = a0[j]; v[4 + j] = a1[j]; }
        for (int sp = 1; sp < splits; ++sp) {
            a0 = *reinterpret_cast<const f32x4*>(s + sp * stride);
            a1 = *reinterpret_cast<const f32x4*>(s + sp * stride + 4);
#pragma unroll
            for (int j = 0; j < 4; ++j) { v[j] += a0[j]; v[4 + j] += a1[j]; }
        }
        f16* dst = C + (int64_t)n * ldc + k;
        f16x8 o;
        if (beta) o = ld8(dst);
#pragma unroll
        for (int j = 0; j < 8; ++j) o[j] = (f16)(beta ? (float)o[j] + v[j] : v[j]);
        st8_out<VLP_SS_TN>(dst, o);
    }
}

static int choose_splits(int M, int N, int K) {
    const int tiles = cdiv(N, TN_BN) * cdiv(K, TN_BK);
    int s = cdiv(512, tiles);
    const int max_by_rows = M / 256 > 0 ? M / 256 : 1;
    if (s > max_by_rows) s = max_by_rows;
    if (s > 16) s = 16;
    if (s < 1) s = 1;
    return s;
}

extern "C" int64_t vlp_gemm_tn_workspace_bytes(int32_t M, int32_t N, int32_t K) {
    const int s = 16;
    (void)M;
    return (int64_t)s * N * K * (int64_t)sizeof(float) + (int64_t)s * ((N + 63) / 64 * 64) * (int64_t)sizeof(float);
}

extern "C" int vlp_gemm_tn(const vlp_gemm_tn_args* a, void* stream) {
    VLP_CHECK_ARG(a != nullptr, "vlp_gemm_tn: null args");
    VLP_ENTER(a->A, "vlp_gemm_tn");
    VLP_CHECK_ARG(a->A && a->B && a->C, "vlp_gemm_tn: null operand");
    VLP_CHECK_ARG(a->M > 0 && a->N > 0 && a->K > 0, "vlp_gemm_tn: bad shape");
    VLP_CHECK_ARG(a->K % 8 == 0, "vlp_gemm_tn: K=%d must be a multiple of 8", a->K);
    VLP_CHECK_ARG(a->lda % 8 == 0 && a->ldb % 8 == 0 && a->ldc % 8 == 0, "vlp_gemm_tn: leading dims must be multiples of 8");
    VLP_CHECK_ARG(a->lda >= (a->N + 7) / 8 * 8 && a->ldb >= a->K && a->ldc >= a->K, "vlp_gemm_tn: leading dim too small");
    VLP_CHECK_ARG(((uintptr_t)a->A | (uintptr_t)a->B | (uintptr_t)a->C) % 16 == 0, "vlp_gemm_tn: operands must be 16-byte aligned");
    VLP_CHECK_ARG(a->beta == 0 || a->beta == 1, "vlp_gemm_tn: beta must be 0 or 1");
    int splits = a->splits > 0 ? a->splits : choose_splits(a->M, a->N, a->K);
    if (splits > 16) splits = 16;
    GemmTnParams p;
    p.A = (const f16*)a->A; p.lda = a->lda;
    p.B = (const f16*)a->B; p.ldb = a->ldb;
    p.C = (f16*)a->C; p.ldc = a->ldc;
    p.M = a->M; p.N = a->N; p.K = a->K; p.beta = a->beta;
    int rps = cdiv(a->M, splits);
    rps = (rps + TN_BM - 1) / TN_BM * TN_BM;
    splits = cdiv(a->M, rps);
    p.splits = splits; p.rows_per_split = rps;
    p.slab = (float*)a->workspace;
    p.bias_out = (f16*)a->bias_out;
    p.bias_slab = p.slab ? p.slab + (int64_t)splits * a->N * a->K : nullptr;
    p.tiles_k = cdiv(a->K, TN_BK);
    p.tiles_n = cdiv(a->N, TN_BN);
    p.xcd_remap = (a->variant & 8) ? 1 : 0;
    p.split_major = (a->variant & 16) ? 1 : 0;
    if (splits > 1) {
        const int64_t need = (int64_t)splits * a->N * a->K * (int64_t)sizeof(float) + (a->bias_out ? (int64_t)splits * a->N * (int64_t)sizeof(float) : 0);
        if (!a->workspace || a->workspace_bytes < need)
            return vlp_set_error(VLP_ERR_WORKSPACE, "vlp_gemm_tn: workspace %lld < %lld bytes", (long long)a->workspace_bytes, (long long)need);
        VLP_CHECK_ARG((uintptr_t)a->workspace % 16 == 0, "vlp_gemm_tn: workspace must be 16-byte aligned");
    }
    hipStream_t s = (hipStream_t)stream;
    const int base = a->variant & 7;
#define LAUNCH_TN_GLDS(BNT, BKT)                                                                                        \
    do {                                                                                                                \
        const size_t smem2 = (size_t)2 * TN_BM * ((BNT) + (BKT)) * sizeof(f16);                                         \
        VLP_ONCE_PER_DEVICE((void)hipFuncSetAttribute((const void*)gemm_tn_glds_kernel<BNT, BKT>, hipFuncAttributeMaxDynamicSharedMemorySize, (int)smem2));                                                            \
        p.tiles_k = cdiv(a->K, (BKT)); p.tiles_n = cdiv(a->N, (BNT));                                                   \
        hipLaunchKernelGGL((gemm_tn_glds_kernel<BNT, BKT>), dim3(p.tiles_k * p.tiles_n * splits), dim3(((BNT) / 64) * ((BKT) / 64) * 64), smem2, s, p); \
    } while (0)
    if (base == 2) LAUNCH_TN_GLDS(128, 128);
    else if (base == 3) LAUNCH_TN_GLDS(256, 128);
    else if (base == 4) LAUNCH_TN_GLDS(128, 256);
    else if (base == 5) return vlp_set_error(VLP_ERR_BAD_ARG, "vlp_gemm_tn: variant 5 (256x256 tiles, 16 waves) was removed: it needed 139 VGPRs under a "
                                             "128-register cap (spills) and lost to the 128x128 kernel on every training shape");
    else {
        dim3 grid(p.tiles_k * p.tiles_n * splits), block(TN_THREADS);
        const size_t smem = 2 * 2 * TN_BM * TN_PITCH * sizeof(f16);
        if (base == 1) {
            VLP_ONCE_PER_DEVICE((void)hipFuncSetAttribute((const void*)gemm_tn_kernel<1>, hipFuncAttributeMaxDynamicSharedMemorySize, (int)smem));
            hipLaunchKernelGGL(gemm_tn_kernel<1>, grid, block, smem, s, p);
        } else {
            VLP_ONCE_PER_DEVICE((void)hipFuncSetAttribute((const void*)gemm_tn_kernel<0>, hipFuncAttributeMaxDynamicSharedMemorySize, (int)smem));
            hipLaunchKernelGGL(gemm_tn_kernel<0>, grid, block, smem, s, p);
        }
    }
#undef LAUNCH_TN_GLDS
    VLP_CHECK_LAUNCH("vlp_gemm_tn");
    if (splits > 1) {
        const int64_t total8 = (int64_t)a->N * (a->K / 8);
        int blocks = (int)((total8 + 255) / 256);
        if (blocks > 2048) blocks = 2048;
        const int bias_blocks = a->bias_out ? cdiv(a->N, 256) : 0;
        hipLaunchKernelGGL(gemm_tn_reduce_kernel, dim3(blocks + bias_blocks), dim3(256), 0, s, p.slab, p.C, p.ldc, a->N, a->K, splits, a->beta,
                           p.bias_slab, p.bias_out, blocks);
        VLP_CHECK_LAUNCH("vlp_gemm_tn_reduce");
    }
    return VLP_OK;
}

#define TN_GROUP_DEFAULT_MODE 0
extern "C" int64_t vlp_gemm_tn_grouped_workspace_bytes(int32_t tiles) {
    return (int64_t)tiles * TN_SK_SLOTS * 256 * 16 + (int64_t)((tiles + 63) / 64 * 64) * (int64_t)sizeof(int);
}

static int tn_check_one(const vlp_gemm_tn_args* a) {
    VLP_CHECK_ARG(a->A && a->B && a->C, "vlp_gemm_tn: null operand");
    VLP_CHECK_ARG(a->M > 0 && a->N > 0 && a->K > 0, "vlp_gemm_tn: bad shape");
    VLP_CHECK_ARG(a->K % 8 == 0, "vlp_gemm_tn: K=%d must be a multiple of 8", a->K);
    VLP_CHECK_ARG(a->lda % 8 == 0 && a->ldb % 8 == 0 && a->ldc % 8 == 0, "vlp_gemm_tn: leading dims must be multiples of 8");
    VLP_CHECK_ARG(a->lda >= (a->N + 7) / 8 * 8 && a->ldb >= a->K && a->ldc >= a->K, "vlp_gemm_tn: leading dim too small");
    VLP_CHECK_ARG(((uintptr_t)a->A | (uintptr_t)a->B | (uintptr_t)a->C) % 16 == 0, "vlp_gemm_tn: operands must be 16-byte aligned");
    VLP_CHECK_ARG(a->beta == 0 || a->beta == 1, "vlp_gemm_tn: beta must be 0 or 1");
    return VLP_OK;
}

extern "C" int vlp_gemm_tn_grouped(const vlp_gemm_tn_args* list, int32_t count, void* stream) {
    VLP_CHECK_ARG(list != nullptr && count >= 1 && count <= TN_GROUP_MAX, "vlp_gemm_tn_grouped: 1..%d problems", TN_GROUP_MAX);
    VLP_ENTER(list[0].A, "vlp_gemm_tn_grouped");
    int mode = TN_GROUP_DEFAULT_MODE;
#ifdef VLP_LAB_BUILD
    if (const char* e = getenv("VLP_TN_GROUP_MODE")) { mode = atoi(e); if (mode < 0 || mode > 5) mode = 0; }
#endif
    const int bn = (mode == 0 || mode >= 3) ? 128 : 256, bk = mode == 3 ? 256 : 128;
    TnGroupParams gp;
    int tiles = 0;
    for (int i = 0; i < count; ++i) {
        const vlp_gemm_tn_args* a = list + i;
        const int rc = tn_check_one(a);
        if (rc != VLP_OK) return rc;
        TnGroupEntry& e = gp.e[i];
        e.A = (const f16*)a->A; e.lda = a->lda; e.B = (const f16*)a->B; e.ldb = a->ldb; e.C = (f16*)a->C; e.ldc = a->ldc;
        e.bias_out = (f16*)a->bias_out;
        e.M = a->M; e.N = a->N; e.K = a->K; e.beta = a->beta;
        e.tiles_k = cdiv(a->K, bk);
        e.tile_begin = tiles;
        tiles += e.tiles_k * cdiv(a->N, bn);
    }
    for (int i = count; i < TN_GROUP_MAX; ++i) { gp.e[i] = gp.e[0]; gp.e[i].tile_begin = 0x7fffffff; }
    gp.count = count; gp.total_tiles = tiles; gp.xcd_remap = 1;
#define LAUNCH_TN_GROUP(BNT, BKT, NSV, BMV)                                                                                             \
    do {                                                                                                                                \
        const size_t smem = (size_t)(NSV) * (BMV) * ((BNT) + (BKT)) * sizeof(f16);                                                      \
        VLP_ONCE_PER_DEVICE((void)hipFuncSetAttribute((const void*)gemm_tn_grouped_kernel<BNT, BKT, NSV, BMV>, hipFuncAttributeMaxDynamicSharedMemorySize, (int)smem));                                                            \
        hipLaunchKernelGGL((gemm_tn_grouped_kernel<BNT, BKT, NSV, BMV>), dim3(tiles), dim3(((BNT) / 64) * ((BKT) / 64) * 64), smem, (hipStream_t)stream, gp); \
    } while (0)
#ifdef VLP_LAB_BUILD
    bool sk = (mode == 5);
    if (sk) {
        const int64_t need = vlp_gemm_tn_grouped_workspace_bytes(tiles);
        sk = tiles % 6 == 0 && list[0].workspace != nullptr && list[0].workspace_bytes >= need && (uintptr_t)list[0].workspace % 16 == 0 && cdiv(list[0].M, 64) >= 14;
        for (int i = 1; i < count && sk; ++i) sk = list[i].M == list[0].M;
    }
    if (sk) {
        float* part = (float*)list[0].workspace;
        int* flags = (int*)((char*)list[0].workspace + (int64_t)tiles * TN_SK_SLOTS * 256 * 16);
        gp.nst = cdiv(list[0].M, 64);
        gp.tail = (gp.nst - 18) / 7;
        if (const char* e = getenv("VLP_TN_SK_TAIL")) { const int v = atoi(e); if (v >= 1 && v < gp.nst) gp.tail = v; }
        if (gp.tail < 1) gp.tail = 1;
        if (hipMemsetAsync(flags, 0, (size_t)tiles * sizeof(int), (hipStream_t)stream) != hipSuccess)
            return vlp_set_error(VLP_ERR_HIP, "vlp_gemm_tn_grouped: hipMemsetAsync(flags): %s", hipGetErrorString(hipGetLastError()));
        const size_t smem = (size_t)2 * 64 * (128 + 128) * sizeof(f16);
        VLP_ONCE_PER_DEVICE((void)hipFuncSetAttribute((const void*)gemm_tn_grouped_sk_kernel<128, 128, 2, 64>, hipFuncAttributeMaxDynamicSharedMemorySize, (int)smem));
        hipLaunchKernelGGL((gemm_tn_grouped_sk_kernel<128, 128, 2, 64>), dim3(tiles / 6 * 7), dim3(256), smem, (hipStream_t)stream, gp, part, flags);
    } else if (mode == 1) LAUNCH_TN_GROUP(256, 128, 2, 64);
    else if (mode == 2) LAUNCH_TN_GROUP(256, 128, 3, 64);
    else if (mode == 3) LAUNCH_TN_GROUP(128, 256, 3, 64);
    else if (mode == 4) LAUNCH_TN_GROUP(128, 128, 4, 32);
    else
#endif
    LAUNCH_TN_GROUP(128, 128, 2, 64);
#undef LAUNCH_TN_GROUP
    VLP_CHECK_LAUNCH("vlp_gemm_tn_grouped");
    return VLP_OK;
}
```

vlp_amd/csrc/layernorm.hip:

```cpp
#include "common.h"
#include <climits>
#include <cstdlib>

#define LN_THREADS 256
#define LN_WAVES 4

DEVFN uint32_t ln_fwd_rowkey(const DropCtx& drop, const int32_t* __restrict__ row_map, int row) {
    return drop.thresh ? drop_rowkey(drop, row_map ? (uint64_t)(uint32_t)row_map[row] : (uint64_t)row) : 0u;
}
DEVFN f16 ln_fwd_out(float v, float mu, float rs, f16 gamma, f16 beta, float m) { return (f16)(((float)gamma * ((v - mu) * rs) + (float)beta) * m); }

template <int NP>
__global__ __launch_bounds__(LN_THREADS) void layernorm_fwd_kernel(
    const f16* __restrict__ x, int64_t ldx, const f16* __restrict__ gamma, const f16* __restrict__ beta,
    f16* __restrict__ y, int64_t ldy, float* __restrict__ mean, float* __restrict__ rstd, int M, int H, float eps, DropCtx drop, const int32_t* __restrict__ row_map) {
    const int lane = threadIdx.x & 63;
    const int wave = blockIdx.x * LN_WAVES + (threadIdx.x >> 6);
    const int nwaves = gridDim.x * LN_WAVES;
    const float invH = 1.f / (float)H;
    for (int row = wave; row < M; row += nwaves) {
        const f16* xr = x + (int64_t)row * ldx;
        float v[NP][4];
        float s = 0.f;
#pragma unroll
// ... 111 lines not shown
    VLP_CHECK_ARG(a->ldx % 8 == 0 && a->ldy % 8 == 0 && a->ldx >= a->H && a->ldy >= a->H, "vlp_layernorm_fwd: leading dims");
    VLP_CHECK_ARG(((uintptr_t)a->x | (uintptr_t)a->y | (uintptr_t)a->gamma | (uintptr_t)a->beta) % 16 == 0, "vlp_layernorm_fwd: alignment");
    DropCtx d = make_drop(a->dropout_p, a->seed, a->rng_stream);
    const int blocks = ln_fwd_blocks(a->M), hblocks = ln_fwd_blocks((a->M + 1) / 2);
    hipStream_t s = (hipStream_t)stream;
#define LAUNCH_LN_FWD(KERNEL_, BLOCKS_)                                                                                        \
    hipLaunchKernelGGL(KERNEL_, dim3(BLOCKS_), dim3(LN_THREADS), 0, s, (const f16*)a->x, a->ldx, (const f16*)a->gamma,        \
                       (const f16*)a->beta, (f16*)a->y, a->ldy, a->mean, a->rstd, a->M, a->H, a->eps, d, a->row_map)
    switch (a->H) {
        case 256: LAUNCH_LN_FWD(layernorm_fwd_hw_kernel<1>, hblocks); break;
        case 512: LAUNCH_LN_FWD(layernorm_fwd_hw_kernel<2>, hblocks); break;
        case 768: LAUNCH_LN_FWD(layernorm_fwd_hw_kernel<3>, hblocks); break;
        case 1024: LAUNCH_LN_FWD(layernorm_fwd_hw_kernel<4>, hblocks); break;
        case 1536: LAUNCH_LN_FWD(layernorm_fwd_hw_kernel<6>, hblocks); break;
        case 2048: LAUNCH_LN_FWD(layernorm_fwd_hw_kernel<8>, hblocks); break;
        default:
            if (a->H <= 768) LAUNCH_LN_FWD(layernorm_fwd_kernel<3>, blocks);
            else if (a->H <= 1024) LAUNCH_LN_FWD(layernorm_fwd_kernel<4>, blocks);
            else if (a->H <= 2048) LAUNCH_LN_FWD(layernorm_fwd_kernel<8>, blocks);
            else LAUNCH_LN_FWD(layernorm_fwd_kernel<16>, blocks);
    }
#undef LAUNCH_LN_FWD
    VLP_CHECK_LAUNCH("vlp_layernorm_fwd");
    return VLP_OK;
}

#define LNB_WAVES 8
#define LNB_THREADS (64 * LNB_WAVES)
#define LNB_BLOCKS (4096 / LNB_WAVES)

template <int NP, bool EXACT, typename Sums>
DEVFN void lnb_block_partials(Sums sums, float* __restrict__ part, int H) {
    extern __shared__ float lnb_sh[];
    const int lane = threadIdx.x & 63;
    float* sg = lnb_sh + (threadIdx.x >> 6) * 2 * H;
#pragma unroll
    for (int k = 0; k < NP; ++k) {
        const int c = 256 * k + 4 * lane;
        if (EXACT || c < H) {
            *reinterpret_cast<f32x4*>(sg + c) = sums(k, 0);
            *reinterpret_cast<f32x4*>(sg + H + c) = sums(k, 1);
        }
    }
    __syncthreads();
    float* dst = part + (int64_t)blockIdx.x * 2 * H;
    for (int i = threadIdx.x; i < 2 * H; i += LNB_THREADS) {
        float t = 0.f;
#pragma unroll
        for (int w = 0; w < LNB_WAVES; ++w) t += lnb_sh[w * 2 * H + i];
        dst[i] = t;
    }
}

template <int NP, bool EXACT, bool HAS_DXD, bool HAS_MAP>
__global__ __launch_bounds__(LNB_THREADS, NP <= 3 ? 4 : (NP == 4 ? 3 : 2)) void layernorm_bwd_kernel(
    const f16* __restrict__ dy, int64_t lddy, const f16* __restrict__ x, int64_t ldx, const f16* __restrict__ gamma,
    const float* __restrict__ mean, const float* __restrict__ rstd, f16* __restrict__ dx, int64_t lddx,
    f16* __restrict__ dxd, int64_t lddxd, float* __restrict__ part, int M, int H_, DropCtx dyd, DropCtx outd, const int32_t* __restrict__ row_map) {
    const int H = EXACT ? 256 * NP : H_;
    const int lane = threadIdx.x & 63;
    const int wave = blockIdx.x * LNB_WAVES + (threadIdx.x >> 6);
    const int nwaves = gridDim.x * LNB_WAVES;
    const float invH = 1.f / (float)H;
    float g[NP][4], dg[NP][4], db[NP][4];
#pragma unroll
    for (int k = 0; k < NP; ++k) {
        const int c = 256 * k + 4 * lane;
        f16x4 gv = (f16x4){0, 0, 0, 0};
        if (EXACT || c < H) gv = ld4(gamma + c);
#pragma unroll
        for (int e = 0; e < 4; ++e) { g[k][e] = (float)gv[e]; dg[k][e] = 0.f; db[k][e] = 0.f; }
    }
    f16x4 xc[NP], dc[NP], xn[NP], dn[NP];
    float mu_c, rs_c, mu_n, rs_n;
    int map_c = 0, map_n = 0;
    auto fetch = [&](int row, f16x4 (&X)[NP], f16x4 (&D)[NP], float& m_, float& r_, int& mp_) {
#pragma unroll
        for (int k = 0; k < NP; ++k) {
            const int c = 256 * k + 4 * lane;
            if (EXACT || c < H) {
                X[k] = ld4(x + (int64_t)row * ldx + c);
                D[k] = ld4(dy + (int64_t)row * lddy + c);
            }
        }
        m_ = mean[row];
        r_ = rstd[row];
        if constexpr (HAS_MAP) mp_ = row_map[row];
    };
    if (wave >= M) {
        mu_c = rs_c = 0.f;
    } else {
        fetch(wave, xc, dc, mu_c, rs_c, map_c);
    }
    for (int row = wave; row < M; row += nwaves) {
        fetch(min(row + nwaves, M - 1), xn, dn, mu_n, rs_n, map_n);
        const float mu = mu_c, rs = rs_c;
        const uint64_t drow = HAS_MAP ? (uint64_t)(uint32_t)map_c : (uint64_t)row;
        const uint32_t rk_dy = dyd.thresh ? drop_rowkey(dyd, drow) : 0u;
        const uint32_t rk_out = outd.thresh ? drop_rowkey(outd, drow) : 0u;
        float xh[NP][4], d[NP][4];
        float s1 = 0.f, s2 = 0.f;
#pragma unroll
        for (int k = 0; k < NP; ++k) {
            const int c = 256 * k + 4 * lane;
            if (EXACT || c < H) {
                float m4[4] = {1.f, 1.f, 1.f, 1.f};
                if (dyd.thresh) drop_mult4(dyd, rk_dy, (uint32_t)c, m4);
#pragma unroll
                for (int e = 0; e < 4; ++e) {
                    const float dd = (float)dc[k][e] * m4[e];
                    xh[k][e] = ((float)xc[k][e] - mu) * rs;
                    dg[k][e] += dd * xh[k][e];
                    db[k][e] += dd;
                    d[k][e] = dd * g[k][e];
                    s1 += d[k][e];
                    s2 += d[k][e] * xh[k][e];
                }
            } else {
#pragma unroll
                for (int e = 0; e < 4; ++e) { xh[k][e] = 0.f; d[k][e] = 0.f; }
            }
        }
        s1 = wave_sum(s1) * invH;
        s2 = wave_sum(s2) * invH;
#pragma unroll
        for (int k = 0; k < NP; ++k) {
            const int c = 256 * k + 4 * lane;
            if (EXACT || c < H) {
                f16x4 o, od;
                float m4[4] = {1.f, 1.f, 1.f, 1.f};
                if (HAS_DXD) drop_mult4(outd, rk_out, (uint32_t)c, m4);
#pragma unroll
                for (int e = 0; e < 4; ++e) {
                    const float t = rs * (d[k][e] - s1 - xh[k][e] * s2);
                    o[e] = (f16)t;
                    od[e] = (f16)(t * m4[e]);
                }
                st4_out<VLP_SS_LN>(dx + (int64_t)row * lddx + c, o);
                if (HAS_DXD) st4_out<VLP_SS_LN>(dxd + (int64_t)row * lddxd + c, od);
            }
        }
#pragma unroll
        for (int k = 0; k < NP; ++k) { xc[k] = xn[k]; dc[k] = dn[k]; }
        mu_c = mu_n;
        rs_c = rs_n;
        map_c = map_n;
    }
    lnb_block_partials<NP, EXACT>([&](int k, int b) { return b ? (f32x4){db[k][0], db[k][1], db[k][2], db[k][3]} : (f32x4){dg[k][0], dg[k][1], dg[k][2], dg[k][3]}; },
                                  part, H);
}

template <typename DstOf>
DEVFN void reduce_partial_rows(const float* __restrict__ part, int nparts, int W, int beta, DstOf dst_of) {
    __shared__ float sh[16][64];
    const int cl = threadIdx.x & 63, pg = threadIdx.x >> 6;
    const int i = blockIdx.x * 64 + cl;
    float s = 0.f;
    if (i < W)
        for (int p = pg; p < nparts; p += 16) s += part[(int64_t)p * W + i];
    sh[pg][cl] = s;
    __syncthreads();
    if (pg == 0 && i < W) {
        float t = 0.f;
#pragma unroll
        for (int k = 0; k < 16; ++k) t += sh[k][cl];
        f16* dst = dst_of(i);
        *dst = (f16)(beta ? (float)*dst + t : t);
    }
}

__global__ __launch_bounds__(1024) void ln_bwd_reduce_kernel(const float* __restrict__ part, int nparts, int H, f16* dgamma, f16* dbeta, int beta) {
    reduce_partial_rows(part, nparts, 2 * H, beta, [&](int i) { return i < H ? dgamma + i : dbeta + (i - H); });
}

__global__ __launch_bounds__(1024) void ln_bwd_reduce_batched_kernel(const float* __restrict__ parts, int64_t slot_stride, f16* const* __restrict__ dst,
                                                                     int nparts, int H, int beta) {
    reduce_partial_rows(parts + (int64_t)blockIdx.y * slot_stride, nparts, 2 * H, beta,
                        [&](int i) { return i < H ? dst[2 * blockIdx.y] + i : dst[2 * blockIdx.y + 1] + (i - H); });
}

static int lnb_blocks(int M) {
    static const int cap = env_blocks("VLP_LNB_BLOCKS", LNB_BLOCKS, LNB_BLOCKS);
    const int blocks = cdiv(M, LNB_WAVES);
    if (blocks <= cap) return blocks;
    const int R = cdiv(M, cap * LNB_WAVES);
    return cdiv(M, R * LNB_WAVES);
}

extern "C" int64_t vlp_layernorm_bwd_workspace_bytes(int32_t H) {
    return (int64_t)LNB_BLOCKS * 2 * H * (int64_t)sizeof(float);
}

template <int NP, bool EXACT, bool HAS_DXD, bool HAS_MAP>
static void launch_ln_bwd(const vlp_layernorm_bwd_args* a, int blocks, const DropCtx& dyd, const DropCtx& outd, hipStream_t s) {
    const auto kernel = layernorm_bwd_kernel<NP, EXACT, HAS_DXD, HAS_MAP>;
    VLP_ONCE_PER_DEVICE((void)hipFuncSetAttribute((const void*)kernel, hipFuncAttributeMaxDynamicSharedMemorySize, LNB_WAVES * 2 * 256 * NP * 4));
    const size_t lnb_smem = (size_t)LNB_WAVES * 2 * a->H * sizeof(float);
    hipLaunchKernelGGL(kernel, dim3(blocks), dim3(LNB_THREADS), lnb_smem, s, (const f16*)a->dy, a->lddy, (const f16*)a->x, a->ldx, (const f16*)a->gamma,
                       a->mean, a->rstd, (f16*)a->dx, a->lddx, (f16*)a->dx_drop, a->lddxd, (float*)a->workspace, a->M, a->H, dyd, outd, a->row_map);
}
template <int NP, bool EXACT>
static void launch_ln_bwd(const vlp_layernorm_bwd_args* a, int blocks, const DropCtx& dyd, const DropCtx& outd, hipStream_t s) {
    const bool hd = a->dx_drop != nullptr, hm = a->row_map != nullptr && (dyd.thresh || outd.thresh);
    if (hd && hm) launch_ln_bwd<NP, EXACT, true, true>(a, blocks, dyd, outd, s);
    else if (hd) launch_ln_bwd<NP, EXACT, true, false>(a, blocks, dyd, outd, s);
    else if (hm) launch_ln_bwd<NP, EXACT, false, true>(a, blocks, dyd, outd, s);
    else launch_ln_bwd<NP, EXACT, false, false>(a, blocks, dyd, outd, s);
}

extern "C" int vlp_layernorm_bwd(const vlp_layernorm_bwd_args* a, void* stream) {
    VLP_CHECK_ARG(a && a->dy && a->x && a->gamma && a->mean && a->rstd && a->dx && a->dgamma && a->dbeta, "vlp_layernorm_bwd: null operand");
    VLP_ENTER(a->dy, "vlp_layernorm_bwd");
    VLP_CHECK_ARG(a->M > 0 && a->H > 0 && a->H % 8 == 0 && a->H <= 2048, "vlp_layernorm_bwd: H=%d must be a multiple of 8 and <= 2048", a->H);
    VLP_CHECK_ARG(a->lddy % 8 == 0 && a->ldx % 8 == 0 && a->lddx % 8 == 0, "vlp_layernorm_bwd: leading dims");
    VLP_CHECK_ARG(((uintptr_t)a->dy | (uintptr_t)a->x | (uintptr_t)a->dx | (uintptr_t)a->gamma) % 16 == 0, "vlp_layernorm_bwd: alignment");
    if (a->dx_drop) VLP_CHECK_ARG(a->lddxd % 8 == 0 && (uintptr_t)a->dx_drop % 16 == 0 && a->out_drop_p > 0.f, "vlp_layernorm_bwd: dx_drop needs out_drop_p > 0");
    const int64_t need = vlp_layernorm_bwd_workspace_bytes(a->H);
    if (!a->workspace || a->workspace_bytes < need) return vlp_set_error(VLP_ERR_WORKSPACE, "vlp_layernorm_bwd: workspace %lld < %lld", (long long)a->workspace_bytes, (long long)need);
    const DropCtx dyd = make_drop(a->dy_drop_p, a->dy_seed, a->dy_stream);
    const DropCtx outd = make_drop(a->out_drop_p, a->out_seed, a->out_stream);
    const int blocks = lnb_blocks(a->M);
    hipStream_t s = (hipStream_t)stream;
    if (a->H == 768) launch_ln_bwd<3, true>(a, blocks, dyd, outd, s);
    else if (a->H <= 768) launch_ln_bwd<3, false>(a, blocks, dyd, outd, s);
    else if (a->H <= 1024) launch_ln_bwd<4, false>(a, blocks, dyd, outd, s);
    else launch_ln_bwd<8, false>(a, blocks, dyd, outd, s);
    VLP_CHECK_LAUNCH("vlp_layernorm_bwd");
    if (a->defer_reduce) return VLP_OK;
    hipLaunchKernelGGL(ln_bwd_reduce_kernel, dim3(cdiv(2 * a->H, 64)), dim3(1024), 0, s, (const float*)a->workspace, blocks, a->H, (f16*)a->dgamma,
                       (f16*)a->dbeta, a->beta);
    VLP_CHECK_LAUNCH("vlp_layernorm_bwd_reduce");
    return VLP_OK;
}

extern "C" int vlp_layernorm_bwd_reduce_batched(const float* parts, const void* const* dst, int32_t count, int32_t M, int32_t H, int32_t beta, void* stream) {
    VLP_CHECK_ARG(parts && dst && count > 0 && count <= 65535 && M > 0 && H > 0 && H % 8 == 0 && H <= 2048, "vlp_layernorm_bwd_reduce_batched: bad args");
    VLP_ENTER(parts, "vlp_layernorm_bwd_reduce_batched");
    VLP_CHECK_ARG(beta == 0 || beta == 1, "vlp_layernorm_bwd_reduce_batched: beta must be 0 or 1");
    const int blocks = lnb_blocks(M);
    hipLaunchKernelGGL(ln_bwd_reduce_batched_kernel, dim3(cdiv(2 * H, 64), count), dim3(1024), 0, (hipStream_t)stream, parts,
                       (int64_t)LNB_BLOCKS * 2 * H, (f16* const*)dst, blocks, H, beta);
    VLP_CHECK_LAUNCH("vlp_layernorm_bwd_reduce_batched");
    return VLP_OK;
}

#define CS_SPLITS 64

__global__ __launch_bounds__(256) void colsum_kernel(const f16* __restrict__ A, int64_t lda, int M, int N, float* __restrict__ part) {
    __shared__ float red[8][256];
    const int tx = threadIdx.x & 31, ty = threadIdx.x >> 5;
    const int c0 = blockIdx.x * 256 + tx * 8;
    const int rows_per = (M + gridDim.y - 1) / gridDim.y;
    const int r0 = blockIdx.y * rows_per, r1 = min(M, r0 + rows_per);
    float acc[8];
#pragma unroll
    for (int e = 0; e < 8; ++e) acc[e] = 0.f;
    if (c0 < N) {
        for (int r = r0 + ty; r < r1; r += 8) {
            f16x8 v = ld8(A + (int64_t)r * lda + c0);
#pragma unroll
            for (int e = 0; e < 8; ++e) acc[e] += (float)v[e];
        }
    }
#pragma unroll
    for (int e = 0; e < 8; ++e) red[ty][tx * 8 + e] = acc[e];
    __syncthreads();
    const int c = threadIdx.x;
    float s = 0.f;
#pragma unroll
    for (int y = 0; y < 8; ++y) s += red[y][c];
    const int col = blockIdx.x * 256 + c;
    if (col < N) part[(int64_t)blockIdx.y * N + col] = s;
}
__global__ __launch_bounds__(1024) void colsum_reduce_kernel(const float* __restrict__ part, int nparts, int N, f16* out, int beta) {
    reduce_partial_rows(part, nparts, N, beta, [&](int i) { return out + i; });
}

extern "C" int64_t vlp_colsum_workspace_bytes(int32_t M, int32_t N) {
    (void)M;
    return (int64_t)CS_SPLITS * N * (int64_t)sizeof(float);
}
extern "C" int vlp_colsum(const vlp_colsum_args* a, void* stream) {
    VLP_CHECK_ARG(a && a->A && a->out && a->M > 0 && a->N > 0, "vlp_colsum: bad args");
    VLP_ENTER(a->A, "vlp_colsum");
    VLP_CHECK_ARG(a->lda % 8 == 0 && a->lda >= (a->N + 7) / 8 * 8 && (uintptr_t)a->A % 16 == 0, "vlp_colsum: layout (lda must cover roundup8(N))");
// ... 12 lines not shown
```

vlp_amd/engine.py:

```python
import math
import os
import weakref

import numpy as np
import torch

from . import _lib as K
from . import tuning
from .input_prep import MaskSpec, RawRegions, SparseAnswers

ALIGN = 64
NO_DECAY = ("bias", "LayerNorm.bias", "LayerNorm.weight")
PE_DIM = 1607
PE_PAD = 1664


def _ru(x, m):
    return (x + m - 1) // m * m


def is_no_decay(name):
    return any(nd in name for nd in NO_DECAY)


# ... 24 lines not shown
    GEMM_TN_VARIANT = 2
    WGRAD_SIDE_STREAM = os.environ.get("VLP_WGRAD_SIDE_STREAM", "1") == "1"
    BLOCK_MASKED_REGION_KEYS = os.environ.get("VLP_BLOCK_MASKED_REGIONS", "0") == "1"
    VARLEN = {"1": True, "0": False}.get(os.environ.get("VLP_VARLEN", ""), "auto")
    TN_SPLITS = None
    TN_VARIANT_CANDIDATES = (2, 26)
    PROF_EVERY = 8
    _nt_choice = {}
    _tn_choice = {}
    _skinny_choice = {}

    def __init__(self, model):
        self._model = weakref.ref(model)
        self.packed = False
        self.gen = 0
        self.step_seed = 0
        self.base_seed = 0x5EED
        self.grads_dirty = False
        self.grad_ready_hook = None
        self.post_backward_hook = None
        self.names = self.offsets = self.sizes = self.buckets = None
        self.flat = self.gflat = None
        self._params = None
        self._unused = None
        self._anchor = None
        self.device = None
        self._ws = {}
        self._shadow = None
        self._shadow_ev = None
        self._ln_tab = None
        self._zero1 = None
        self._pretext_on = False
        self._pooler_dirty = False
        self.prof = None
        self._opt_stream = None
        self._param_events = None
        self._params_done = None
        self.shard_plan = None
        self._param_works = None
        self.param_gather_stamps = None
        self._side = None
        self._side_done = None
        self._side_busy = False
        self._prof_ctr = 0
        self.varlen = self.VARLEN
        self.varlen_readback_budget = 0
        self._rb_streak = 0
        self._rb_warned = False
        self._pk_stage = None
        self._pk_stage_i = 0
        self._pk_cache = {}
        self._pk_lens = {}
        self.last_packed_rows = None

    def _ordered_names(self, model):
        cfg = model.config
        tasks = model.tasks
        names = {n for n, _ in model.named_parameters()}
        decay, buckets = [], []

        def add(group):
            start = len(decay)
            decay.extend(group)
            buckets.append((start, len(decay)))

        head_unused = []
        if tasks == "vqa2":
            add(["ans_classifier.2.weight", "ans_classifier.0.weight"])
            head_unused.append("cls.predictions.transform.dense.weight")
        else:
            add(["cls.predictions.transform.dense.weight"])
        for i in reversed(range(cfg.num_hidden_layers)):
            L = "bert.encoder.layer.%d." % i
            add([L + "output.dense.weight", L + "intermediate.dense.weight", L + "attention.output.dense.weight",
                 L + "attention.self.query.weight", L + "attention.self.key.weight", L + "attention.self.value.weight"])
        add(["bert.embeddings.position_embeddings.weight", "bert.embeddings.token_type_embeddings.weight",
             "bert.embeddings.word_embeddings.weight"])
        add(["vis_pe_embed.0.weight", "vis_embed.2.weight", "vis_embed.0.weight", "bert.pooler.dense.weight"] + head_unused)
        nodecay = sorted(n for n in names if is_no_decay(n))
        for i in range(cfg.num_hidden_layers):
            L = "bert.encoder.layer.%d.attention.self." % i
            for n in (L + "query.bias", L + "key.bias", L + "value.bias"):
                nodecay.remove(n)
            nodecay.extend([L + "query.bias", L + "key.bias", L + "value.bias"])
        missing = names - set(decay) - set(nodecay)
        extra = (set(decay) | set(nodecay)) - names
        if missing or extra:
            raise RuntimeError("vlp_amd.Engine: unexpected parameter set (missing %s, unknown %s)" % (sorted(missing), sorted(extra)))
        return decay, nodecay, buckets

    def plan_layout(self, model=None):
        model = model if model is not None else self._model()
        numel = {n: p.numel() for n, p in model.named_parameters()}
        decay, nodecay, bucket_idx = self._ordered_names(model)
        names = {"decay": decay, "nodecay": nodecay}
        offsets, sizes = {}, {}
        for grp, ns in names.items():
            off, offs = 0, {}
            for n in ns:
                offs[n] = off
                off += _ru(numel[n], ALIGN)
            offsets[grp], sizes[grp] = offs, _ru(off, 8)
        buckets = []
        for s_, e_ in bucket_idx:
            lo = offsets["decay"][decay[s_]]
            hi = offsets["decay"][decay[e_ - 1]] + _ru(numel[decay[e_ - 1]], ALIGN)
# ... 97 lines not shown
            self._params_done.synchronize()
            self._param_events, self._params_done = None, None
        else:
            torch.cuda.current_stream().wait_event(self._params_done)

    def zero_placeholder(self, device):
        z = self._zero1
        if z is None or z.device != device:
            z = self._zero1 = torch.zeros(1, device=device, dtype=torch.float32)
        return z

    def is_zero_placeholder(self, t):
        return t is self._zero1

    def zero_grad(self):
        self.grads_dirty = False

    def _workspace(self, B, L, P):
        key = (B, L, P)
        ws = self._ws.get(key)
        if ws is not None:
            return ws
        model = self._model()
        cfg = model.config
        H, I, A, NL, Nv, V = cfg.hidden_size, cfg.intermediate_size, cfg.num_attention_heads, cfg.num_hidden_layers, model.len_vis_input, cfg.vocab_size
        M, Mv = B * L, B * Nv
        dev = self.device

        def h(*s):
            return torch.empty(*s, device=dev, dtype=torch.float16)

        def f(*s):
            return torch.empty(*s, device=dev, dtype=torch.float32)

        ws = {"Lp": _ru(L, 32)}
        ws["maskb"] = torch.empty(B, L, ws["Lp"], device=dev, dtype=torch.uint8)
        ws["maskt"] = torch.empty(B, ws["Lp"], ws["Lp"], device=dev, dtype=torch.uint8)
        ws["img16"], ws["vpe_in"], ws["wpe_pad"] = h(Mv, 2048), h(Mv, PE_PAD), h(H, PE_PAD)
        ws["h1"], ws["vis_h"], ws["vispe_h"] = h(Mv, 2048), h(Mv, H), h(Mv, H)
        ws["emb_pre"], ws["x0"] = h(M, H), h(M, H)
        ws["stat0"] = (f(M), f(M))
        lay = []
        for _ in range(NL):
            lay.append({"qkv": h(M, 3 * H), "ctx": h(M, H), "lse": f(B, A, L), "pre1": h(M, H), "x1": h(M, H),
                        "st1": (f(M), f(M)), "z": h(M, I), "g": h(M, I), "pre2": h(M, H), "x2": h(M, H), "st2": (f(M), f(M))})
        ws["layers"] = lay
        Vp = _ru(V, 64)
        ws["Vp"] = Vp
        if P > 0:
            R = B * P
            ws.update(sel=h(R, H), tz=h(R, H), tg=h(R, H), tln=h(R, H), tstat=(f(R), f(R)), logits=h(R, Vp), dlogits=h(R, Vp),
                      dlT=h(Vp, _ru(R, 64)),
                      lse_ce=f(R), coef=f(R), row_loss=f(R), dtln=h(R, H), dtg=h(R, H), dtz=h(R, H), dsel=h(R, H))
        ws["loss"] = f(260)
        if model.tasks == "vqa2":
            NA = model.num_answers
            NAp = _ru(NA, 64)
            ws.update(NAp=NAp, vq_e=h(B, H), vq_a1=h(B, 2 * H), vq_logits=h(B, NAp), vq_dlogits=h(B, NAp), vq_dz1=h(B, 2 * H), vq_de=h(B, H))
        ws.update(dx=h(M, H), dx_alt=h(M, H), dpre=h(M, H), dpre_d=h(M, H), dz=h(M, I), dctx=h(M, H), dqkv=h(M, 3 * H),
                  delta=f(B, A, L), d_vis_h=h(Mv, H), d_vispe_h=h(Mv, H), dz1v=h(Mv, 2048), dwpe_pad=h(H, PE_PAD), acc32=f(K.embed_bwd_workspace_floats(B, L, Nv, H)))
        ws["dyset"] = [{"dpre2": h(M, H), "dpre2_d": h(M, H), "dpre1": h(M, H), "dpre1_d": h(M, H), "dz": h(M, I), "dqkv": h(M, 3 * H)}
                       for _ in range(2)]
        tn_bytes = max(K.gemm_tn_workspace_bytes(M, I, H), K.gemm_tn_workspace_bytes(Mv, 2048, 2048), K.gemm_tn_workspace_bytes(M, 3 * H, H))
        ws["tn_ws"] = torch.empty(tn_bytes, device=dev, dtype=torch.uint8)
        ws["tn_ws_main"] = torch.empty(max(K.gemm_tn_workspace_bytes(V, _ru(B * max(P, 1), 64), H), 1 << 20), device=dev, dtype=torch.uint8)
        ws["cs_ws"] = torch.empty(max(K.colsum_workspace_bytes(M, I), K.colsum_workspace_bytes(B * max(P, 1), Vp)), device=dev, dtype=torch.uint8)
        ws["ln_ws"] = torch.empty(K.layernorm_bwd_workspace_bytes(max(H, 8)), device=dev, dtype=torch.uint8)
        ws["ln_slot_bytes"] = K.layernorm_bwd_workspace_bytes(max(H, 8))
        ws["ln_slots"] = torch.empty((2 * NL + 1) * ws["ln_slot_bytes"], device=dev, dtype=torch.uint8)
        self._ws[key] = ws
        return ws

    def _shadows(self):
        if self._shadow is not None:
            return self._shadow
        model = self._model()
        cfg = model.config
        H, I, V = cfg.hidden_size, cfg.intermediate_size, cfg.vocab_size
        dev = self.device

        def h(*s):
            return torch.zeros(*s, device=dev, dtype=torch.float16)

        sh = {"layers": [{"qkvT": h(H, 3 * H), "oT": h(H, H), "w1T": h(H, I), "w2T": h(I, H)} for _ in range(cfg.num_hidden_layers)],
              "v2T": h(2048, H)}
        if model.tasks == "vqa2":
            NAp = _ru(model.num_answers, 64)
            sh.update(a2T=h(2 * H, NAp), a0T=h(H, 2 * H))
        else:
            sh.update(tT=h(H, H))
        self._shadow = sh
        return sh

    def _ln_table(self):
        if self._ln_tab is None:
            NL = self._model().config.num_hidden_layers
            rows = []
            for i in range(NL):
                L = "bert.encoder.layer.%d." % i
                for n in ("attention.output.LayerNorm", "output.LayerNorm"):
                    rows.append([self.G(L + n + ".weight").data_ptr(), self.G(L + n + ".bias").data_ptr()])
            rows.append([self.G("bert.embeddings.LayerNorm.weight").data_ptr(), self.G("bert.embeddings.LayerNorm.bias").data_ptr()])
            self._ln_tab = torch.tensor(rows, dtype=torch.int64, device=self.device)
        return self._ln_tab

    def _refresh_shadows(self):
# ... 732 lines not shown
        T = out_len - in_len
        if tuple(sample_ids.shape) != (B, T):
            raise RuntimeError("vlp_amd: score_samples expects sampled ids [B, %d] (output length - input length), got %s" % (T, tuple(sample_ids.shape)))
        Lo = in_len + 2 * T - 1
        if Lo > 256:
            raise RuntimeError("vlp_amd: the SCST scoring sequence has %d + 2 x %d - 1 = %d positions, more than the attention kernels' 256; "
                               "lower --max_len_b" % (in_len, T, Lo))
        key = ("scst", B, in_len, T)
        sw = self._ws.get(key)
        if sw is None:
            dev = self.device

            def i64(*sh):
                return torch.empty(*sh, device=dev, dtype=torch.long)
            sw = self._ws[key] = dict(ids=i64(B, Lo), seg=i64(B, Lo), pos=i64(B, Lo), mask=i64(B, Lo, Lo), mpos=i64(B, T), labels=i64(B, T),
                                      logp=torch.empty(B, T, device=dev, dtype=torch.float32))
        am = attention_mask[:, :out_len, :out_len].to(torch.long).contiguous()
        tt = token_type_ids[:, :out_len].to(torch.long).contiguous()
        pid = position_ids[:, :out_len].to(torch.long).contiguous()
        sw["labels"].copy_(sample_ids)
        K.scst_layout(input_ids.to(torch.long).contiguous(), sw["labels"], tt, pid, am, sw["ids"], sw["seg"], sw["pos"], sw["mask"], sw["mpos"],
                      mask_word_id)
        st = self.forward(vis_feats, vis_pe, sw["ids"], sw["seg"], sw["mask"], sw["mpos"], True, True, False, position_ids=sw["pos"],
                          dropout=False, dense=True)
        st.task_labels = sw["labels"].view(-1)
        K.token_logprob_fwd(st.ws["logits"], st.ws["Vp"], st.task_labels, sw["logp"], st.ws["lse_ce"], B * T, V)
        return st, sw["logp"]

    def _tn_splits(self, a, b, c, M, N, Kd, ws):
        if self.TN_SPLITS is not None:
            return (self.GEMM_TN_VARIANT, self.TN_SPLITS)
        key = (M, N, Kd)
        sp = Engine._tn_choice.get(key)
        if sp is not None:
            return sp
        if not tuning.AUTOTUNE:
            sp = Engine._tn_choice[key] = tuning.tn_choice(M, N, Kd)
            return sp
        best = (self.GEMM_TN_VARIANT, 0)
        if M >= 1024:
            cands = [(var, sp) for var in self.TN_VARIANT_CANDIDATES for sp in tuning.TN_SPLIT_CANDIDATES if not (sp > 1 and M // sp < 128)]
            torch.cuda.synchronize()
            scratch = torch.empty(N, Kd, device=c.device, dtype=torch.float16)
            best = tuning.best_of(cands, lambda vs, i: K.gemm_tn(a, b, scratch, M, N, Kd, beta=0, workspace=ws["tn_ws"], variant=vs[0], splits=vs[1]),
                                  rounds=2, reps=3)
        Engine._tn_choice[key] = best
        tuning.remember("tn", M, N, Kd, best)
        return best

    def _tn(self, a, b, c, M, N, Kd, ws, beta, bias=None, ws_key="tn_ws", **kw):
        var, sp = self._tn_splits(a, b, c, M, N, Kd, ws)
        K.gemm_tn(a, b, c, M, N, Kd, beta=beta, workspace=ws[ws_key], variant=var, bias_out=bias, splits=sp, **kw)

    def _bucket_done(self, idx):
        if self.grad_ready_hook is not None:
            self.grad_ready_hook(idx)

    def backward(self, st, gscale, task, g_pretext=None, g_rows=None):
        if st.gen != self.gen:
            raise RuntimeError("vlp_amd: the activations of this forward were overwritten by a later forward "
                               "(one in-flight forward per model; run backward before the next forward)")
        model = self._model()
        cfg = model.config
        H, I, A, NL, Nv, V = cfg.hidden_size, cfg.intermediate_size, cfg.num_attention_heads, cfg.num_hidden_layers, model.len_vis_input, cfg.vocab_size
        B, L, P, ws, seed = st.B, st.L, st.P, st.ws, st.seed
        p, pa = st.p_drop
        M, Mv = B * L, B * Nv
        ro = rm = None
        if st.pk is not None:
            ro, rm, M = st.pk
        beta = 1 if self.grads_dirty else 0
        if beta and self.shard_plan is not None:
            raise RuntimeError("vlp_amd: VLP_DDP_MODE=sharded keeps only this rank's chunk of the reduced gradient, so gradients cannot be "
                               "accumulated over several backward passes (--gradient_accumulation_steps > 1); use allreduce or rs_ag")
        img, input_ids, token_type_ids, masked_pos = st.batch
        self.wait_params()
        if self._shadow_ev is not None:
            torch.cuda.current_stream().wait_event(self._shadow_ev)
            self._shadow_ev = None
        else:
            self._refresh_shadows()
        sh = self._shadows()
        x_last = ws["layers"][NL - 1]["x2"]
        dx = ws["dx"]
        dx.zero_()
        E = "bert.embeddings."
        if beta == 0:
            self.G(E + "position_embeddings.weight").zero_()
            self.G(E + "token_type_embeddings.weight").zero_()

        main = torch.cuda.current_stream()
        use_side = self.WGRAD_SIDE_STREAM
        side = self._side_stream() if use_side else None

        def on_side(fn):
            if not use_side:
                fn()
                return
            side.wait_stream(main)
            with torch.cuda.stream(side):
                fn()

        if use_side:
            self._side_busy = True
        head_wgrads = []

        if task == "vqa2":
            NA, NAp = model.num_answers, ws["NAp"]
            if isinstance(st.task_labels, SparseAnswers):
                K.bce_sparse_loss_bwd(ws["vq_logits"], NAp, st.task_labels.idx, st.task_labels.score, B, NA, gscale, ws["vq_dlogits"], NAp)
            else:
                K.bce_loss_bwd(ws["vq_logits"], NAp, st.task_labels, st.task_labels.stride(0), B, NA, gscale, ws["vq_dlogits"], NAp)
            self._tn(ws["vq_dlogits"], ws["vq_a1"], self.G("ans_classifier.2.weight"), B, NA, 2 * H, ws, beta, bias=self.G("ans_classifier.2.bias"))
            self._nt(ws["vq_dlogits"], sh["a2T"], ws["vq_dz1"], B, 2 * H, NAp, mul_src=ws["vq_a1"], mul_mode=K.MUL_RELU_MASK)
            self._tn(ws["vq_dz1"], ws["vq_e"], self.G("ans_classifier.0.weight"), B, 2 * H, H, ws, beta, bias=self.G("ans_classifier.0.bias"))
            self._nt(ws["vq_dz1"], sh["a0T"], ws["vq_de"], B, H, 2 * H)
            K.vqa_mul_bwd(x_last, ws["vq_de"], dx, B, L, Nv, H, row_off=ro)
            if beta == 0:
                self.G(E + "word_embeddings.weight").zero_()
        elif not st.has_mlm:
            if beta == 0:
                self.G(E + "word_embeddings.weight").zero_()
                for n in ("bias", "transform.dense.weight", "transform.dense.bias", "transform.LayerNorm.weight", "transform.LayerNorm.bias"):
                    self.G("cls.predictions." + n).zero_()
        else:
            C = "cls.predictions."
            R, Vp = B * P, ws["Vp"]
            if task == "logprob":
                if g_rows is None or g_rows.numel() != R:
                    raise RuntimeError("vlp_amd: backward(task='logprob') needs g_rows with %d elements" % R)
                K.token_logprob_bwd(ws["logits"], Vp, st.task_labels, ws["lse_ce"], g_rows, ws["dlogits"], Vp, R, V)
            elif st.mlm_smooth is None:
                K.mlm_loss_bwd(ws["logits"], Vp, st.task_labels, ws["lse_ce"], ws["coef"], gscale, ws["dlogits"], Vp, R, V)
            else:
                K.mlm_loss_ls_bwd(ws["logits"], Vp, st.task_labels, ws["lse_ce"], ws["coef"], gscale, ws["dlogits"], Vp, R, V, *st.mlm_smooth)
            head_wgrads.append(lambda: self._tn(ws["dlogits"], ws["tln"], self.G(E + "word_embeddings.weight"), R, V, H, ws, beta, bias=self.G(C + "bias")))
            Rp = _ru(R, 64)
            K.transpose(ws["dlogits"], Vp, ws["dlT"], Rp, R, Vp, Rp)
            self._tn(ws["dlT"], self.P(E + "word_embeddings.weight"), ws["dtln"], V, R, H, ws, 0, ws_key="tn_ws_main")
            K.layernorm_bwd(ws["dtln"], ws["tg"], self.P(C + "transform.LayerNorm.weight"), ws["tstat"][0], ws["tstat"][1], ws["dtg"],
                            self.G(C + "transform.LayerNorm.weight"), self.G(C + "transform.LayerNorm.bias"), R, H, ws["ln_ws"], beta=beta)
            K.gelu_bwd(ws["dtg"], ws["tz"], ws["dtz"], R * H)
            head_wgrads.append(lambda: self._tn(ws["dtz"], ws["sel"], self.G(C + "transform.dense.weight"), R, H, H, ws, beta, bias=self.G(C + "transform.dense.bias")))
            self._nt(ws["dtz"], sh["tT"], ws["dsel"], R, H, H)
            K.scatter_add_rows(ws["dsel"], H, masked_pos.contiguous(), dx, H, B, P, L, H, row_off=ro)
        pt = st.pretext
        if pt is not None:
            ptw, vmp = pt
            if g_pretext is None:
                g_pretext = torch.zeros(1, device=self.device, dtype=torch.float32)
            K.pretext_bwd(ws["vis_h"], ws["vispe_h"], ptw["pooled"], vmp, ptw["probs"], g_pretext, ws["d_vis_h"], ws["d_vispe_h"], ptw["dpool"],
                          B, Nv, vmp.shape[1], H, drop_p=p, seed=seed, vis_stream=1001, vispe_stream=1002)
            self._tn(ptw["dpool"], ptw["sel0"], self.G("bert.pooler.dense.weight"), B, H, H, ws, beta, bias=self.G("bert.pooler.dense.bias"))
            K.transpose(self.P("bert.pooler.dense.weight"), H, ptw["pT"], H, H, H, H)
            self._nt(ptw["dpool"], ptw["pT"], ptw["dsel0"], B, H, H)
            K.scatter_add_rows(ptw["dsel0"], H, ptw["pos0"], dx, H, B, 1, L, H, row_off=ro)
        elif beta == 0 and self._pooler_dirty:
            self.G("bert.pooler.dense.weight").zero_()
            self.G("bert.pooler.dense.bias").zero_()
        self._pooler_dirty = pt is not None

        def head_tail():
            for fn in head_wgrads:
                fn()
            self._bucket_done(0)
        on_side(head_tail)

        dctx = ws["dctx"]
        scale = 1.0 / math.sqrt(H // A)
        slot_bytes = ws["ln_slot_bytes"]

        def ln_slot(k):
            return ws["ln_slots"][k * slot_bytes:(k + 1) * slot_bytes]

        grouped = M >= 2048
        for i in reversed(range(NL)):
            Ln = "bert.encoder.layer.%d." % i
            a = ws["layers"][i]
            s = sh["layers"][i]
            x_in = ws["layers"][i - 1]["x2"] if i > 0 else ws["x0"]
            ds = ws["dyset"][i & 1]
            if use_side and self._side_done[i & 1] is not None:
                main.wait_event(self._side_done[i & 1])
            dpre = ds["dpre2"]
            K.layernorm_bwd(dx, a["pre2"], self.P(Ln + "output.LayerNorm.weight"), a["st2"][0], a["st2"][1], dpre,
                            self.G(Ln + "output.LayerNorm.weight"), self.G(Ln + "output.LayerNorm.bias"), M, H, ln_slot(2 * i + 1), beta=beta,
                            dx_drop=ds["dpre2_d"] if p > 0 else None, out_drop=(p, seed, 16 * i + 3), defer_reduce=True, row_map=rm)
            dy2 = ds["dpre2_d"] if p > 0 else dpre
            if not grouped:
                on_side(lambda: self._tn(dy2, a["g"], self.G(Ln + "output.dense.weight"), M, H, I, ws, beta, bias=self.G(Ln + "output.dense.bias")))
            self._nt(dy2, s["w2T"], ds["dz"], M, I, H, mul_src=a["z"], mul_mode=K.MUL_PLAIN)
            if not grouped:
                on_side(lambda: self._tn(ds["dz"], a["x1"], self.G(Ln + "intermediate.dense.weight"), M, I, H, ws, beta,
                                         bias=self.G(Ln + "intermediate.dense.bias")))
            self._nt(ds["dz"], s["w1T"], dx, M, H, I, residual=dpre)
            dpre = ds["dpre1"]
            K.layernorm_bwd(dx, a["pre1"], self.P(Ln + "attention.output.LayerNorm.weight"), a["st1"][0], a["st1"][1], dpre,
                            self.G(Ln + "attention.output.LayerNorm.weight"), self.G(Ln + "attention.output.LayerNorm.bias"), M, H, ln_slot(2 * i),
                            beta=beta, dx_drop=ds["dpre1_d"] if p > 0 else None, out_drop=(p, seed, 16 * i + 2), defer_reduce=True, row_map=rm)
            dy1 = ds["dpre1_d"] if p > 0 else dpre
            if not grouped:
                on_side(lambda: self._tn(dy1, a["ctx"], self.G(Ln + "attention.output.dense.weight"), M, H, H, ws, beta,
                                         bias=self.G(Ln + "attention.output.dense.bias")))
            self._nt(dy1, s["oT"], dctx, M, H, H)
            dqkv = ds["dqkv"]
            K.attn_bwd(a["qkv"], ws["maskb"], ws["maskt"], a["ctx"], dctx, a["lse"], dqkv, ws["delta"], B, L, A, scale, dropout_p=pa, seed=seed,
                       rng_stream=16 * i + 1, row_off=ro)

            def last_wgrad():
                if grouped:
                    K.gemm_tn_grouped([
                        (dy2, a["g"], self.G(Ln + "output.dense.weight"), M, H, I, beta, self.G(Ln + "output.dense.bias")),
                        (ds["dz"], a["x1"], self.G(Ln + "intermediate.dense.weight"), M, I, H, beta, self.G(Ln + "intermediate.dense.bias")),
                        (dqkv, x_in, self.G(Ln + "attention.self.query.weight"), M, 3 * H, H, beta, self.G(Ln + "attention.self.query.bias")),
                        (dy1, a["ctx"], self.G(Ln + "attention.output.dense.weight"), M, H, H, beta, self.G(Ln + "attention.output.dense.bias"))])
                else:
                    self._tn(dqkv, x_in, self.G(Ln + "attention.self.query.weight"), M, 3 * H, H, ws, beta,
                             bias=self.G(Ln + "attention.self.query.bias"))
                self._bucket_done(NL - i)
                if use_side:
                    ev = torch.cuda.Event()
                    ev.record(side)
                    self._side_done[i & 1] = ev
            on_side(last_wgrad)
            self._nt(dqkv, s["qkvT"], dx, M, H, 3 * H, residual=dpre)
        if use_side and not grouped:
            main.wait_stream(side)
            self._side_busy = False
        dpre = ws["dpre"]

        K.layernorm_bwd(dx, ws["emb_pre"], self.P(E + "LayerNorm.weight"), ws["stat0"][0], ws["stat0"][1], dpre,
                        self.G(E + "LayerNorm.weight"), self.G(E + "LayerNorm.bias"), M, H, ln_slot(2 * NL), beta=beta, dy_drop=(p, seed, 1000),
                        defer_reduce=True, row_map=rm)
        if rm is not None:
            dense = ws["dx_alt"]
            dense.zero_()
# ... 44 lines not shown
```

Before: 6823 samples/s.

## Restrict last-layer backward to masked-LM live rows before attention

```diff
diff --git a/include/vlp_hip.h b/include/vlp_hip.h
--- a/include/vlp_hip.h
+++ b/include/vlp_hip.h
@@ -43,6 +43,12 @@
 } vlp_gemm_nt_args;
 int vlp_gemm_nt(const vlp_gemm_nt_args* a, void* stream);
 int vlp_gemm_nt_resolved_variant(void);
+enum { VLP_ROWS_X = 1,
+       VLP_ROWS_MUL = 2,
+       VLP_ROWS_RES = 4,
+       VLP_ROWS_Y = 8      };
+int vlp_live_rows_build(const int64_t* pos, int32_t B, int32_t P, int32_t L, const int32_t* row_off, int32_t* live, int32_t* count, void* stream);
+int vlp_gemm_nt_rows(const vlp_gemm_nt_args* a, const int32_t* live, int32_t flags, void* stream);
 int64_t vlp_gemm_nt_splitk_workspace_bytes(int32_t M, int32_t N, int32_t splits);
 int vlp_gemm_nt_splitk(const vlp_gemm_nt_args* a, int32_t splits, void* workspace, int64_t workspace_bytes, void* stream);
 
@@ -61,6 +67,7 @@
 int vlp_gemm_tn(const vlp_gemm_tn_args* a, void* stream);
 int vlp_gemm_tn_grouped(const vlp_gemm_tn_args* list, int32_t count, void* stream);
 int64_t vlp_gemm_tn_grouped_workspace_bytes(int32_t tiles);
+int vlp_gemm_tn_grouped_rows(const vlp_gemm_tn_args* list, const int32_t* const* live, const int32_t* flags, int32_t count, void* stream);
 
 typedef struct {
     const void* A; int64_t lda; int32_t M, N;
@@ -142,6 +149,7 @@
 } vlp_layernorm_bwd_args;
 int64_t vlp_layernorm_bwd_workspace_bytes(int32_t H);
 int vlp_layernorm_bwd(const vlp_layernorm_bwd_args* a, void* stream);
+int vlp_layernorm_bwd_rows(const vlp_layernorm_bwd_args* a, const int32_t* live, int32_t flags, int32_t part_M, void* stream);
 int vlp_layernorm_bwd_reduce_batched(const float* parts, const void* const* dst, int32_t count, int32_t M, int32_t H, int32_t beta, void* stream);
 
 int vlp_region_mask_build(const int64_t* vis_masked_pos, int32_t B, int32_t Pm, int32_t Nv, uint8_t* out, void* stream);
diff --git a/vlp_amd/_lib.py b/vlp_amd/_lib.py
--- a/vlp_amd/_lib.py
+++ b/vlp_amd/_lib.py
@@ -8,6 +8,7 @@
 
 ACT_NONE, ACT_GELU, ACT_RELU, ACT_TANH, ACT_GELU_SAVE_GRAD = 0, 1, 2, 3, 4
 MUL_NONE, MUL_GELU_GRAD, MUL_RELU_MASK, MUL_PLAIN = 0, 1, 2, 3
+ROWS_X, ROWS_MUL, ROWS_RES, ROWS_Y = 1, 2, 4, 8
 
 vp, i64, i32, f32, u64, u32 = C.c_void_p, C.c_int64, C.c_int32, C.c_float, C.c_uint64, C.c_uint32
 
@@ -180,12 +181,14 @@
     "vlp_lab_build": (C.c_int, []),
     "vlp_debug_device_lookup_stats": (None, [vp, vp]),
     "vlp_gemm_nt": (C.c_int, [C.POINTER(GemmNtArgs), vp]),
+    "vlp_gemm_nt_rows": (C.c_int, [C.POINTER(GemmNtArgs), vp, i32, vp]),
     "vlp_gemm_nt_resolved_variant": (C.c_int, []),
     "vlp_gemm_nt_splitk_workspace_bytes": (C.c_int64, [i32, i32, i32]),
     "vlp_gemm_nt_splitk": (C.c_int, [C.POINTER(GemmNtArgs), i32, vp, i64, vp]),
     "vlp_gemm_tn_workspace_bytes": (i64, [i32, i32, i32]),
     "vlp_gemm_tn": (C.c_int, [C.POINTER(GemmTnArgs), vp]),
     "vlp_gemm_tn_grouped": (C.c_int, [C.POINTER(GemmTnArgs), i32, vp]),
+    "vlp_gemm_tn_grouped_rows": (C.c_int, [C.POINTER(GemmTnArgs), C.POINTER(vp), C.POINTER(i32), i32, vp]),
     "vlp_gemm_tn_grouped_workspace_bytes": (i64, [i32]),
     "vlp_colsum_workspace_bytes": (i64, [i32, i32]),
     "vlp_colsum": (C.c_int, [C.POINTER(ColsumArgs), vp]),
@@ -211,6 +214,7 @@
     "vlp_layernorm_fwd": (C.c_int, [C.POINTER(LayerNormFwdArgs), vp]),
     "vlp_layernorm_bwd_workspace_bytes": (i64, [i32]),
     "vlp_layernorm_bwd": (C.c_int, [C.POINTER(LayerNormBwdArgs), vp]),
+    "vlp_layernorm_bwd_rows": (C.c_int, [C.POINTER(LayerNormBwdArgs), vp, i32, i32, vp]),
     "vlp_layernorm_bwd_reduce_batched": (C.c_int, [vp, vp, i32, i32, i32, i32, vp]),
     "vlp_embed_fwd": (C.c_int, [C.POINTER(EmbedFwdArgs), vp]),
     "vlp_embed_bwd": (C.c_int, [C.POINTER(EmbedBwdArgs), vp]),
@@ -226,6 +230,7 @@
     "vlp_transpose_batched": (C.c_int, [vp, vp, i32, i32, vp]),
     "vlp_gather_rows": (C.c_int, [vp, i64, vp, vp, i64, i32, i32, i32, i32, vp, vp]),
     "vlp_scatter_add_rows": (C.c_int, [vp, i64, vp, vp, i64, i32, i32, i32, i32, vp, vp]),
+    "vlp_live_rows_build": (C.c_int, [vp, i32, i32, i32, vp, vp, vp, vp]),
     "vlp_rowmap_build": (C.c_int, [vp, i32, i32, vp, vp]),
     "vlp_rows_unpack": (C.c_int, [vp, i64, vp, i32, vp, i64, i32, vp]),
     "vlp_rows_pack": (C.c_int, [vp, i64, vp, i32, vp, i64, i32, vp]),
@@ -365,6 +370,14 @@
     _check(load().vlp_gemm_nt(C.byref(a), stream_ptr()))
 
 
+def gemm_nt_rows(x, w, y, live, flags, M, N, K, ldx=None, ldw=None, ldy=None, bias=None, residual=None, ldr=None, mul_src=None, ldm=None,
+                 mul_mode=MUL_NONE, alpha=1.0, dropout_p=0.0, seed=0, rng_stream=0, variant=0, row_map=None):
+    _req_cuda(x, w, y, live, row_map)
+    a = _gemm_nt_args(x, w, y, M, N, K, ldx, ldw, ldy, bias, residual, ldr, None, None, mul_src, ldm, ACT_NONE, mul_mode, alpha, dropout_p, seed,
+                      rng_stream, variant, row_map)
+    _check(load().vlp_gemm_nt_rows(C.byref(a), ptr(live), flags, stream_ptr()))
+
+
 def gemm_nt_resolved_variant():
     return int(load().vlp_gemm_nt_resolved_variant())
 
@@ -408,6 +421,19 @@
         arr[i] = GemmTnArgs(ptr(a_), a_.stride(0), ptr(b_), b_.stride(0), ptr(c_), c_.stride(0), M, N, K, beta, ptr(w),
                             _nbytes(w), 0, 0, ptr(bias_out))
     _check(load().vlp_gemm_tn_grouped(arr, len(problems), stream_ptr()))
+
+
+def gemm_tn_grouped_rows(problems):
+    n = len(problems)
+    arr = (GemmTnArgs * n)()
+    lives = (vp * n)()
+    flags = (i32 * n)()
+    for i, (a_, b_, c_, M, N, K, beta, bias_out, live, fl) in enumerate(problems):
+        _req_cuda(a_, b_, c_, bias_out, live)
+        arr[i] = GemmTnArgs(ptr(a_), a_.stride(0), ptr(b_), b_.stride(0), ptr(c_), c_.stride(0), M, N, K, beta, None, 0, 0, 0, ptr(bias_out))
+        lives[i] = live.data_ptr() if live is not None else None
+        flags[i] = fl
+    _check(load().vlp_gemm_tn_grouped_rows(arr, lives, flags, n, stream_ptr()))
 
 
 def colsum_workspace_bytes(M, N):
@@ -566,6 +592,16 @@
                          dy_drop[0], dy_drop[1], dy_drop[2], out_drop[0], out_drop[1], out_drop[2],
                          ptr(workspace), _nbytes(workspace), 1 if defer_reduce else 0, ptr(row_map))
     _check(load().vlp_layernorm_bwd(C.byref(a), stream_ptr()))
+
+
+def layernorm_bwd_rows(dy, x, gamma, mean, rstd, dx, dgamma, dbeta, live, flags, M, H, workspace, part_M, beta=0, dx_drop=None,
+                       out_drop=(0.0, 0, 0), defer_reduce=False, row_map=None):
+    _req_cuda(dy, x, gamma, mean, rstd, dx, dgamma, dbeta, workspace, row_map, live)
+    a = LayerNormBwdArgs(ptr(dy), dy.stride(0), ptr(x), x.stride(0), ptr(gamma), ptr(mean), ptr(rstd), ptr(dx), dx.stride(0),
+                         ptr(dx_drop), dx_drop.stride(0) if dx_drop is not None else 0, ptr(dgamma), ptr(dbeta), M, H, beta,
+                         0.0, 0, 0, out_drop[0], out_drop[1], out_drop[2],
+                         ptr(workspace), _nbytes(workspace), 1 if defer_reduce else 0, ptr(row_map))
+    _check(load().vlp_layernorm_bwd_rows(C.byref(a), ptr(live), flags, part_M, stream_ptr()))
 
 
 def layernorm_bwd_reduce_batched(parts, dst_table, count, M, H, beta=0):
@@ -744,6 +780,11 @@
     _check(load().vlp_scatter_add_rows(ptr(src), lds, ptr(pos), ptr(dst), ldd, B, P, L, H, ptr(row_off), stream_ptr()))
 
 
+def live_rows_build(pos, B, P, L, live, count, row_off=None):
+    _req_cuda(pos, live, count, row_off)
+    _check(load().vlp_live_rows_build(ptr(pos), B, P, L, ptr(row_off), ptr(live), ptr(count), stream_ptr()))
+
+
 def rowmap_build(row_off, B, L, row_map):
     _req_cuda(row_off, row_map)
     _check(load().vlp_rowmap_build(ptr(row_off), B, L, ptr(row_map), stream_ptr()))
diff --git a/vlp_amd/csrc/elementwise.hip b/vlp_amd/csrc/elementwise.hip
--- a/vlp_amd/csrc/elementwise.hip
+++ b/vlp_amd/csrc/elementwise.hip
@@ -448,6 +448,49 @@
     hipLaunchKernelGGL(scatter_add_rows_kernel, dim3((int)((total + 255) / 256)), dim3(256), 0, (hipStream_t)stream, (const f16*)src, lds,
                        pos, (f16*)dst, ldd, B, P, L, H, row_off);
     VLP_CHECK_LAUNCH("vlp_scatter_add_rows");
+    return VLP_OK;
+}
+
+__global__ __launch_bounds__(256) void live_rows_build_kernel(const int64_t* __restrict__ pos, int B, int P, int L, const int32_t* __restrict__ row_off,
+                                                              int32_t* __restrict__ live, int32_t* __restrict__ count) {
+    extern __shared__ int32_t lrb_rows[];
+    __shared__ int lrb_count;
+    const int n = B * P;
+    int32_t* keep = lrb_rows + n;
+    if (threadIdx.x == 0) lrb_count = 0;
+    for (int t = threadIdx.x; t < n; t += blockDim.x) {
+        int nb;
+        const int64_t base = sample_base(row_off, t / P, L, nb);
+        int64_t ps = pos[t];
+        ps = ps < 0 ? 0 : (ps >= nb ? nb - 1 : ps);
+        lrb_rows[t] = (int32_t)(base + ps);
+        live[t] = -1;
+    }
+    __syncthreads();
+    for (int t = threadIdx.x; t < n; t += blockDim.x) {
+        const int32_t r = lrb_rows[t];
+        int first = 1;
+        for (int j = 0; j < t; ++j) first &= (lrb_rows[j] != r);
+        keep[t] = first;
+    }
+    __syncthreads();
+    for (int t = threadIdx.x; t < n; t += blockDim.x) {
+        if (!keep[t]) continue;
+        const int32_t r = lrb_rows[t];
+        int rank = 0;
+        for (int j = 0; j < n; ++j) rank += (keep[j] && lrb_rows[j] < r) ? 1 : 0;
+        live[rank] = r;
+        atomicAdd(&lrb_count, 1);
+    }
+    __syncthreads();
+    if (threadIdx.x == 0 && count) *count = lrb_count;
+}
+extern "C" int vlp_live_rows_build(const int64_t* pos, int32_t B, int32_t P, int32_t L, const int32_t* row_off, int32_t* live, int32_t* count, void* stream) {
+    VLP_CHECK_ARG(pos && live && B > 0 && P > 0 && L > 0 && (int64_t)B * P <= 12288, "vlp_live_rows_build: bad args (B * P <= 12288)");
+    VLP_ENTER(pos, "vlp_live_rows_build");
+    VLP_ONCE_PER_DEVICE((void)hipFuncSetAttribute((const void*)live_rows_build_kernel, hipFuncAttributeMaxDynamicSharedMemorySize, 2 * 12288 * 4));
+    hipLaunchKernelGGL(live_rows_build_kernel, dim3(1), dim3(256), (size_t)2 * B * P * sizeof(int32_t), (hipStream_t)stream, pos, B, P, L, row_off, live, count);
+    VLP_CHECK_LAUNCH("vlp_live_rows_build");
     return VLP_OK;
 }
 
diff --git a/vlp_amd/csrc/gemm_nt.hip b/vlp_amd/csrc/gemm_nt.hip
--- a/vlp_amd/csrc/gemm_nt.hip
+++ b/vlp_amd/csrc/gemm_nt.hip
@@ -16,8 +16,8 @@
 DEVFN int swz_x(int r) { return r & 7; }
 DEVFN int swz_w(int r) { return (((r >> 4) & 3) << 1) | ((r >> 1) & 1); }
 
-template <int VARIANT, int BM_T, int BN_T, bool SG, int NSR = 0, int EPI = 0>
-__global__ __launch_bounds__((BM_T / 64) * (BN_T / 64) * 64, (VARIANT == 3 ? (BN_T == 256 ? 4 : BM_T / 128) : ((VARIANT == 2 || BN_T == 256) ? 4 : 2))) void gemm_nt_kernel(GemmNtParams p) {
+template <int VARIANT, int BM_T, int BN_T, bool SG, int NSR, int EPI, bool ROWS>
+DEVFN void gemm_nt_body(const GemmNtParams& p, const int32_t* __restrict__ live, int live_flags) {
     extern __shared__ __attribute__((aligned(16))) char smem_raw[];
     f16* smem = reinterpret_cast<f16*>(smem_raw);
     constexpr int WN_ = BN_T / 64;
@@ -49,7 +49,8 @@
 #pragma unroll
     for (int i = 0; i < XP; ++i) {
         const int r = srow + RPP * i;
-        const int mr = min(m0 + r, p.M - 1);
+        int mr = min(m0 + r, p.M - 1);
+        if (ROWS && (live_flags & VLP_ROWS_X)) mr = max(live[mr], 0);
         xsrc[i] = p.X + (int64_t)mr * p.ldx + (sx ^ swz_x(r)) * 8;
         lds_off[i] = r * BK + sx * 8;
     }
@@ -296,6 +297,21 @@
     for (int tm = 0; tm < 4; ++tm) {
         const int m = m0 + wm * 64 + 16 * tm + li;
         if (m >= p.M) continue;
+        if constexpr (ROWS) {
+            const int lm = live[m];
+            if (lm < 0) continue;
+            const uint32_t rkey = p.drop.thresh ? drop_rowkey(p.drop, p.row_map ? (uint64_t)(uint32_t)p.row_map[lm] : (uint64_t)lm) : 0u;
+            float v[16];
+#pragma unroll
+            for (int tn = 0; tn < 4; ++tn)
+#pragma unroll
+                for (int r = 0; r < 4; ++r) v[tn * 4 + r] = acc[tm][tn][r] * p.alpha + bias_v[tn * 4 + r];
+#pragma unroll
+            for (int h = 0; h < 2; ++h)
+                nt_epilogue8_rows<SG>(p, (live_flags & VLP_ROWS_Y) ? lm : m, (live_flags & VLP_ROWS_MUL) ? lm : m, (live_flags & VLP_ROWS_RES) ? lm : m,
+                                      ncol0 + 8 * h, v + 8 * h, rkey, true);
+            continue;
+        }
         const uint32_t rkey = p.drop.thresh ? drop_rowkey(p.drop, nt_drop_row(p, m)) : 0u;
         float v[16];
 #pragma unroll
@@ -311,6 +327,14 @@
     asm volatile("s_waitcnt vmcnt(0)" ::: "memory");
     NT_TRACE(3);
 #endif
+}
+
+template <int VARIANT, int BM_T, int BN_T, bool SG, int NSR = 0, int EPI = 0>
+__global__ __launch_bounds__((BM_T / 64) * (BN_T / 64) * 64, (VARIANT == 3 ? (BN_T == 256 ? 4 : BM_T / 128) : ((VARIANT == 2 || BN_T == 256) ? 4 : 2))) void gemm_nt_kernel(GemmNtParams p) {
+    gemm_nt_body<VARIANT, BM_T, BN_T, SG, NSR, EPI, false>(p, nullptr, 0);
+}
+__global__ __launch_bounds__(256, 1) void gemm_nt_rows_kernel(GemmNtParams p, const int32_t* __restrict__ live, int live_flags) {
+    gemm_nt_body<3, 128, 128, false, 0, 0, true>(p, live, live_flags);
 }
 
 int vlp_gemm_nt_fill_params(const vlp_gemm_nt_args* a, GemmNtParams& p) {
@@ -449,6 +473,25 @@
     return VLP_OK;
 }
 
+extern "C" int vlp_gemm_nt_rows(const vlp_gemm_nt_args* a, const int32_t* live, int32_t flags, void* stream) {
+    VLP_ENTER(a ? a->X : nullptr, "vlp_gemm_nt_rows");
+    GemmNtParams p;
+    const int frc = vlp_gemm_nt_fill_params(a, p);
+    if (frc != VLP_OK) return frc;
+    VLP_CHECK_ARG(live != nullptr, "vlp_gemm_nt_rows: null row list");
+    VLP_CHECK_ARG((flags & ~(VLP_ROWS_X | VLP_ROWS_MUL | VLP_ROWS_RES | VLP_ROWS_Y)) == 0, "vlp_gemm_nt_rows: bad flags %d", flags);
+    VLP_CHECK_ARG(!a->preact && nt_epilogue_is_light(p) && a->act != VLP_ACT_GELU_SAVE_GRAD,
+                  "vlp_gemm_nt_rows: the listed-row form carries the dgrad epilogues (bias, stored multiplier, dropout, residual) only");
+    p.xcd_remap = (a->variant & 8) ? 1 : 0;
+    t_last_variant = 17 | (a->variant & 8);
+    const size_t smem = (size_t)4 * (128 + 128) * BK * sizeof(f16);
+    VLP_ONCE_PER_DEVICE((void)hipFuncSetAttribute((const void*)gemm_nt_rows_kernel, hipFuncAttributeMaxDynamicSharedMemorySize, (int)smem));
+    p.tiles_n = cdiv(a->N, 128);
+    hipLaunchKernelGGL(gemm_nt_rows_kernel, dim3(cdiv(a->M, 128) * p.tiles_n), dim3(256), smem, (hipStream_t)stream, p, live, (int)flags);
+    VLP_CHECK_LAUNCH("vlp_gemm_nt_rows");
+    return VLP_OK;
+}
+
 extern "C" int vlp_gemm_nt_splitk(const vlp_gemm_nt_args* a, int32_t splits, void* workspace, int64_t workspace_bytes, void* stream) {
     VLP_ENTER(a ? a->X : nullptr, "vlp_gemm_nt_splitk");
     GemmNtParams p;
diff --git a/vlp_amd/csrc/gemm_nt_epilogue.h b/vlp_amd/csrc/gemm_nt_epilogue.h
--- a/vlp_amd/csrc/gemm_nt_epilogue.h
+++ b/vlp_amd/csrc/gemm_nt_epilogue.h
@@ -15,7 +15,7 @@
     return (p.act == VLP_ACT_NONE || p.act == VLP_ACT_RELU) && p.mulmode != VLP_MUL_GELU_GRAD;
 }
 template <bool SG = false, bool LIGHT = false>
-DEVFN void nt_epilogue8(const GemmNtParams& p, int m, int nc, float* vv, uint32_t rkey, bool bias_done = false) {
+DEVFN void nt_epilogue8_rows(const GemmNtParams& p, int m, int m_mul, int m_res, int nc, float* vv, uint32_t rkey, bool bias_done) {
     if (nc >= p.N) return;
     if (p.bias && !bias_done) {
         if (nc + 8 <= p.N) {
@@ -65,7 +65,7 @@
         }
     }
     if (p.mulmode != VLP_MUL_NONE) {
-        const f16x8 s = ld8(p.mulsrc + (int64_t)m * p.ldm + nc);
+        const f16x8 s = ld8(p.mulsrc + (int64_t)m_mul * p.ldm + nc);
         if (!LIGHT && p.mulmode == VLP_MUL_GELU_GRAD) {
 #pragma unroll
             for (int j = 0; j < 8; ++j) vv[j] *= gelu_grad_f((float)s[j]);
@@ -81,7 +81,7 @@
         drop_mult8(p.drop, rkey, (uint32_t)nc, vv);
     }
     if (p.residual) {
-        const f16x8 r = ld8(p.residual + (int64_t)m * p.ldr + nc);
+        const f16x8 r = ld8(p.residual + (int64_t)m_res * p.ldr + nc);
 #pragma unroll
         for (int j = 0; j < 8; ++j) vv[j] += (float)r[j];
     }
@@ -90,3 +90,7 @@
     for (int j = 0; j < 8; ++j) o[j] = (nc + j < p.N) ? (f16)vv[j] : (f16)0.f;
     ST8_OUT(p, p.Y + (int64_t)m * p.ldy + nc, o);
 }
+template <bool SG = false, bool LIGHT = false>
+DEVFN void nt_epilogue8(const GemmNtParams& p, int m, int nc, float* vv, uint32_t rkey, bool bias_done = false) {
+    nt_epilogue8_rows<SG, LIGHT>(p, m, m, m, nc, vv, rkey, bias_done);
+}
diff --git a/vlp_amd/csrc/gemm_tn.hip b/vlp_amd/csrc/gemm_tn.hip
--- a/vlp_amd/csrc/gemm_tn.hip
+++ b/vlp_amd/csrc/gemm_tn.hip
@@ -16,6 +16,8 @@
     f16* bias_out;
     int M, N, K, beta, splits, rows_per_split;
     int tiles_k, tiles_n, xcd_remap, split_major;
+    const int32_t* live;
+    int a_listed;
 };
 
 typedef __fp16 fp16x4_t __attribute__((__vector_size__(4 * sizeof(__fp16))));
@@ -183,7 +185,7 @@
 #define TN_SK_WRITE 1
 #define TN_SK_FINAL 2
 #define TN_SK_SLOTS 20
-template <int BN_T, int BK_T, int NS = 2, int BM_T = TN_BM, bool SK = false>
+template <int BN_T, int BK_T, int NS = 2, int BM_T = TN_BM, bool SK = false, bool LISTED = false>
 DEVFN void tn_glds_tile(const GemmTnParams& p, int bid, f16* smem, int sk_m_begin = 0, int sk_m_end = 0, int sk_role = 0, float* sk_part = nullptr,
                         int* sk_flag = nullptr) {
     constexpr int WK_ = BK_T / 64;
@@ -243,7 +245,28 @@
         f16* as = smem + buf * (ATILE + BTILE);
         f16* bs = as + ATILE;
         const int mbase = m_begin + st * BM_T;
-        if (mbase + BM_T <= m_end) {
+        if (LISTED) {
+#pragma unroll
+            for (int i = 0; i < AP; ++i) {
+                const int r = arow + ARP * i, m = mbase + r;
+                u32x4 v = (u32x4){0, 0, 0, 0};
+                if (m < m_end) {
+                    const int lr = p.live[m];
+                    if (lr >= 0) v = *reinterpret_cast<const u32x4*>(p.A + (int64_t)(p.a_listed ? lr : m) * p.lda + acol[i]);
+                }
+                *reinterpret_cast<u32x4*>(as + r * BN_T + apc * 8) = v;
+            }
+#pragma unroll
+            for (int i = 0; i < BP; ++i) {
+                const int r = brow + BRP * i, m = mbase + r;
+                u32x4 v = (u32x4){0, 0, 0, 0};
+                if (m < m_end) {
+                    const int lr = p.live[m];
+                    if (lr >= 0) v = *reinterpret_cast<const u32x4*>(p.B + (int64_t)lr * p.ldb + bcol[i]);
+                }
+                *reinterpret_cast<u32x4*>(bs + r * BK_T + bpc * 8) = v;
+            }
+        } else if (mbase + BM_T <= m_end) {
             const uint32_t as_l = smem_lds + (uint32_t)(buf * (ATILE + BTILE)) * 2u, bs_l = as_l + (uint32_t)ATILE * 2u;
             const int64_t aoff = (int64_t)st * BM_T * p.lda, boff = (int64_t)st * BM_T * p.ldb;
 #pragma unroll
@@ -302,10 +325,11 @@
             if (i < nstages) stage(i, i);
         int buf = 0, nbuf = NS - 1;
         const bool tail_ragged = ((m_end - m_begin) % BM_T) != 0;
+        const bool listed = LISTED;
         for (int st = 0; st < nstages; ++st) {
             const int left = nstages - 1 - st;
             int younger = left < NS - 2 ? left : NS - 2;
-            if (tail_ragged && st + younger >= nstages - 1) younger = 0;
+            if ((tail_ragged && st + younger >= nstages - 1) || listed) younger = 0;
             if (NS >= 4 && younger == 2) asm volatile("s_waitcnt vmcnt(%0) lgkmcnt(0)" ::"n"(2 * LPS) : "memory");
             else if (NS >= 3 && younger >= 1) asm volatile("s_waitcnt vmcnt(%0) lgkmcnt(0)" ::"n"(LPS) : "memory");
             else asm volatile("s_waitcnt vmcnt(0) lgkmcnt(0)" ::: "memory");
@@ -397,6 +421,7 @@
     f16* C; int64_t ldc;
     f16* bias_out;
     int M, N, K, beta, tiles_k, tile_begin;
+    const int32_t* live; int a_listed;
 };
 struct TnGroupParams {
     TnGroupEntry e[TN_GROUP_MAX];
@@ -419,7 +444,9 @@
     p.slab = nullptr; p.bias_slab = nullptr; p.bias_out = e.bias_out;
     p.M = e.M; p.N = e.N; p.K = e.K; p.beta = e.beta; p.splits = 1; p.rows_per_split = (e.M + TN_BM - 1) / TN_BM * TN_BM;
     p.tiles_k = e.tiles_k; p.tiles_n = 0; p.xcd_remap = 0; p.split_major = 0;
-    tn_glds_tile<BN_T, BK_T, NS, BM_T>(p, bid - e.tile_begin, reinterpret_cast<f16*>(smem_raw));
+    p.live = e.live; p.a_listed = e.a_listed;
+    if (e.live) tn_glds_tile<BN_T, BK_T, NS, BM_T, false, true>(p, bid - e.tile_begin, reinterpret_cast<f16*>(smem_raw));
+    else tn_glds_tile<BN_T, BK_T, NS, BM_T>(p, bid - e.tile_begin, reinterpret_cast<f16*>(smem_raw));
 }
 
 #ifdef VLP_LAB_BUILD
@@ -444,6 +471,7 @@
         p.slab = nullptr; p.bias_slab = nullptr; p.bias_out = e.bias_out;
         p.M = e.M; p.N = e.N; p.K = e.K; p.beta = e.beta; p.splits = 1; p.rows_per_split = 0;
         p.tiles_k = e.tiles_k; p.tiles_n = 0; p.xcd_remap = 0; p.split_major = 0;
+        p.live = nullptr; p.a_listed = 0;
         if (j < 6)
             tn_glds_tile<BN_T, BK_T, NS, BM_T, true>(p, tile - e.tile_begin, reinterpret_cast<f16*>(smem_raw), 0, cut * BM_T, TN_SK_FINAL,
                                                        part + (int64_t)tile * (TN_SK_SLOTS * T * 4), flags + grp);
@@ -544,6 +572,7 @@
     p.tiles_n = cdiv(a->N, TN_BN);
     p.xcd_remap = (a->variant & 8) ? 1 : 0;
     p.split_major = (a->variant & 16) ? 1 : 0;
+    p.live = nullptr; p.a_listed = 0;
     if (splits > 1) {
         const int64_t need = (int64_t)splits * a->N * a->K * (int64_t)sizeof(float) + (a->bias_out ? (int64_t)splits * a->N * (int64_t)sizeof(float) : 0);
         if (!a->workspace || a->workspace_bytes < need)
@@ -605,9 +634,7 @@
     return VLP_OK;
 }
 
-extern "C" int vlp_gemm_tn_grouped(const vlp_gemm_tn_args* list, int32_t count, void* stream) {
-    VLP_CHECK_ARG(list != nullptr && count >= 1 && count <= TN_GROUP_MAX, "vlp_gemm_tn_grouped: 1..%d problems", TN_GROUP_MAX);
-    VLP_ENTER(list[0].A, "vlp_gemm_tn_grouped");
+static int tn_grouped_launch(const vlp_gemm_tn_args* list, const int32_t* const* live, const int32_t* lflags, int32_t count, void* stream) {
     int mode = TN_GROUP_DEFAULT_MODE;
 #ifdef VLP_LAB_BUILD
     if (const char* e = getenv("VLP_TN_GROUP_MODE")) { mode = atoi(e); if (mode < 0 || mode > 5) mode = 0; }
@@ -623,6 +650,8 @@
         e.A = (const f16*)a->A; e.lda = a->lda; e.B = (const f16*)a->B; e.ldb = a->ldb; e.C = (f16*)a->C; e.ldc = a->ldc;
         e.bias_out = (f16*)a->bias_out;
         e.M = a->M; e.N = a->N; e.K = a->K; e.beta = a->beta;
+        e.live = live ? live[i] : nullptr;
+        e.a_listed = (e.live && lflags && (lflags[i] & VLP_ROWS_X)) ? 1 : 0;
         e.tiles_k = cdiv(a->K, bk);
         e.tile_begin = tiles;
         tiles += e.tiles_k * cdiv(a->N, bn);
@@ -636,7 +665,7 @@
         hipLaunchKernelGGL((gemm_tn_grouped_kernel<BNT, BKT, NSV, BMV>), dim3(tiles), dim3(((BNT) / 64) * ((BKT) / 64) * 64), smem, (hipStream_t)stream, gp); \
     } while (0)
 #ifdef VLP_LAB_BUILD
-    bool sk = (mode == 5);
+    bool sk = (mode == 5) && !live;
     if (sk) {
         const int64_t need = vlp_gemm_tn_grouped_workspace_bytes(tiles);
         sk = tiles % 6 == 0 && list[0].workspace != nullptr && list[0].workspace_bytes >= need && (uintptr_t)list[0].workspace % 16 == 0 && cdiv(list[0].M, 64) >= 14;
@@ -665,3 +694,15 @@
     VLP_CHECK_LAUNCH("vlp_gemm_tn_grouped");
     return VLP_OK;
 }
+
+extern "C" int vlp_gemm_tn_grouped(const vlp_gemm_tn_args* list, int32_t count, void* stream) {
+    VLP_CHECK_ARG(list != nullptr && count >= 1 && count <= TN_GROUP_MAX, "vlp_gemm_tn_grouped: 1..%d problems", TN_GROUP_MAX);
+    VLP_ENTER(list[0].A, "vlp_gemm_tn_grouped");
+    return tn_grouped_launch(list, nullptr, nullptr, count, stream);
+}
+
+extern "C" int vlp_gemm_tn_grouped_rows(const vlp_gemm_tn_args* list, const int32_t* const* live, const int32_t* flags, int32_t count, void* stream) {
+    VLP_CHECK_ARG(list != nullptr && live != nullptr && count >= 1 && count <= TN_GROUP_MAX, "vlp_gemm_tn_grouped_rows: 1..%d problems and their row lists", TN_GROUP_MAX);
+    VLP_ENTER(list[0].A, "vlp_gemm_tn_grouped_rows");
+    return tn_grouped_launch(list, live, flags, count, stream);
+}
diff --git a/vlp_amd/csrc/layernorm.hip b/vlp_amd/csrc/layernorm.hip
--- a/vlp_amd/csrc/layernorm.hip
+++ b/vlp_amd/csrc/layernorm.hip
@@ -187,11 +187,12 @@
     }
 }
 
-template <int NP, bool EXACT, bool HAS_DXD, bool HAS_MAP>
+template <int NP, bool EXACT, bool HAS_DXD, bool HAS_MAP, bool LIST = false>
 __global__ __launch_bounds__(LNB_THREADS, NP <= 3 ? 4 : (NP == 4 ? 3 : 2)) void layernorm_bwd_kernel(
     const f16* __restrict__ dy, int64_t lddy, const f16* __restrict__ x, int64_t ldx, const f16* __restrict__ gamma,
     const float* __restrict__ mean, const float* __restrict__ rstd, f16* __restrict__ dx, int64_t lddx,
-    f16* __restrict__ dxd, int64_t lddxd, float* __restrict__ part, int M, int H_, DropCtx dyd, DropCtx outd, const int32_t* __restrict__ row_map) {
+    f16* __restrict__ dxd, int64_t lddxd, float* __restrict__ part, int M, int H_, DropCtx dyd, DropCtx outd, const int32_t* __restrict__ row_map,
+    const int32_t* __restrict__ live = nullptr, int lflags = 0) {
     const int H = EXACT ? 256 * NP : H_;
     const int lane = threadIdx.x & 63;
     const int wave = blockIdx.x * LNB_WAVES + (threadIdx.x >> 6);
@@ -209,7 +210,24 @@
     f16x4 xc[NP], dc[NP], xn[NP], dn[NP];
     float mu_c, rs_c, mu_n, rs_n;
     int map_c = 0, map_n = 0;
-    auto fetch = [&](int row, f16x4 (&X)[NP], f16x4 (&D)[NP], float& m_, float& r_, int& mp_) {
+    int lr_c = 0, lr_n = 0;
+    auto fetch = [&](int row, f16x4 (&X)[NP], f16x4 (&D)[NP], float& m_, float& r_, int& mp_, int& lr_) {
+        if constexpr (LIST) {
+            lr_ = live[row];
+            const int src = max(lr_, 0);
+#pragma unroll
+            for (int k = 0; k < NP; ++k) {
+                const int c = 256 * k + 4 * lane;
+                if (EXACT || c < H) {
+                    X[k] = ld4(x + (int64_t)src * ldx + c);
+                    D[k] = ld4(dy + (int64_t)((lflags & VLP_ROWS_X) ? src : row) * lddy + c);
+                }
+            }
+            m_ = mean[src];
+            r_ = rstd[src];
+            if constexpr (HAS_MAP) mp_ = row_map[src];
+            return;
+        }
 #pragma unroll
         for (int k = 0; k < NP; ++k) {
             const int c = 256 * k + 4 * lane;
@@ -222,15 +240,10 @@
         r_ = rstd[row];
         if constexpr (HAS_MAP) mp_ = row_map[row];
     };
-    if (wave >= M) {
-        mu_c = rs_c = 0.f;
-    } else {
-        fetch(wave, xc, dc, mu_c, rs_c, map_c);
-    }
-    for (int row = wave; row < M; row += nwaves) {
-        fetch(min(row + nwaves, M - 1), xn, dn, mu_n, rs_n, map_n);
+    auto row_body = [&](int row) {
         const float mu = mu_c, rs = rs_c;
-        const uint64_t drow = HAS_MAP ? (uint64_t)(uint32_t)map_c : (uint64_t)row;
+        const int orow = (LIST && (lflags & VLP_ROWS_Y)) ? lr_c : row;
+        const uint64_t drow = HAS_MAP ? (uint64_t)(uint32_t)map_c : (uint64_t)(LIST ? lr_c : row);
         const uint32_t rk_dy = dyd.thresh ? drop_rowkey(dyd, drow) : 0u;
         const uint32_t rk_out = outd.thresh ? drop_rowkey(outd, drow) : 0u;
         float xh[NP][4], d[NP][4];
@@ -271,15 +284,39 @@
                     o[e] = (f16)t;
                     od[e] = (f16)(t * m4[e]);
                 }
-                st4_out<VLP_SS_LN>(dx + (int64_t)row * lddx + c, o);
+                st4_out<VLP_SS_LN>(dx + (int64_t)orow * lddx + c, o);
                 if (HAS_DXD) st4_out<VLP_SS_LN>(dxd + (int64_t)row * lddxd + c, od);
             }
         }
-#pragma unroll
-        for (int k = 0; k < NP; ++k) { xc[k] = xn[k]; dc[k] = dn[k]; }
-        mu_c = mu_n;
-        rs_c = rs_n;
-        map_c = map_n;
+    };
+    if constexpr (LIST) {
+        for (int base = 0; base < M; base += 64) {
+            const int e = base + lane;
+            const int lv = e < M ? live[e] : -1;
+            unsigned long long mask = __ballot(lv >= 0 && (lv % nwaves) == wave);
+            while (mask) {
+                const int bit = __ffsll(mask) - 1;
+                mask &= mask - 1;
+                fetch(base + bit, xc, dc, mu_c, rs_c, map_c, lr_c);
+                row_body(base + bit);
+            }
+        }
+    } else {
+        if (wave >= M) {
+            mu_c = rs_c = 0.f;
+        } else {
+            fetch(wave, xc, dc, mu_c, rs_c, map_c, lr_c);
+        }
+        for (int row = wave; row < M; row += nwaves) {
+            fetch(min(row + nwaves, M - 1), xn, dn, mu_n, rs_n, map_n, lr_n);
+            row_body(row);
+#pragma unroll
+            for (int k = 0; k < NP; ++k) { xc[k] = xn[k]; dc[k] = dn[k]; }
+            mu_c = mu_n;
+            rs_c = rs_n;
+            map_c = map_n;
+            lr_c = lr_n;
+        }
     }
     lnb_block_partials<NP, EXACT>([&](int k, int b) { return b ? (f32x4){db[k][0], db[k][1], db[k][2], db[k][3]} : (f32x4){dg[k][0], dg[k][1], dg[k][2], dg[k][3]}; },
                                   part, H);
@@ -326,26 +363,26 @@
     return (int64_t)LNB_BLOCKS * 2 * H * (int64_t)sizeof(float);
 }
 
-template <int NP, bool EXACT, bool HAS_DXD, bool HAS_MAP>
-static void launch_ln_bwd(const vlp_layernorm_bwd_args* a, int blocks, const DropCtx& dyd, const DropCtx& outd, hipStream_t s) {
-    const auto kernel = layernorm_bwd_kernel<NP, EXACT, HAS_DXD, HAS_MAP>;
+template <int NP, bool EXACT, bool HAS_DXD, bool HAS_MAP, bool LIST = false>
+static void launch_ln_bwd(const vlp_layernorm_bwd_args* a, int blocks, const DropCtx& dyd, const DropCtx& outd, hipStream_t s, const int32_t* live = nullptr,
+                          int lflags = 0) {
+    const auto kernel = layernorm_bwd_kernel<NP, EXACT, HAS_DXD, HAS_MAP, LIST>;
     VLP_ONCE_PER_DEVICE((void)hipFuncSetAttribute((const void*)kernel, hipFuncAttributeMaxDynamicSharedMemorySize, LNB_WAVES * 2 * 256 * NP * 4));
     const size_t lnb_smem = (size_t)LNB_WAVES * 2 * a->H * sizeof(float);
     hipLaunchKernelGGL(kernel, dim3(blocks), dim3(LNB_THREADS), lnb_smem, s, (const f16*)a->dy, a->lddy, (const f16*)a->x, a->ldx, (const f16*)a->gamma,
-                       a->mean, a->rstd, (f16*)a->dx, a->lddx, (f16*)a->dx_drop, a->lddxd, (float*)a->workspace, a->M, a->H, dyd, outd, a->row_map);
-}
-template <int NP, bool EXACT>
-static void launch_ln_bwd(const vlp_layernorm_bwd_args* a, int blocks, const DropCtx& dyd, const DropCtx& outd, hipStream_t s) {
+                       a->mean, a->rstd, (f16*)a->dx, a->lddx, (f16*)a->dx_drop, a->lddxd, (float*)a->workspace, a->M, a->H, dyd, outd, a->row_map, live, lflags);
+}
+template <int NP, bool EXACT, bool LIST = false>
+static void launch_ln_bwd(const vlp_layernorm_bwd_args* a, int blocks, const DropCtx& dyd, const DropCtx& outd, hipStream_t s, const int32_t* live = nullptr,
+                          int lflags = 0) {
     const bool hd = a->dx_drop != nullptr, hm = a->row_map != nullptr && (dyd.thresh || outd.thresh);
-    if (hd && hm) launch_ln_bwd<NP, EXACT, true, true>(a, blocks, dyd, outd, s);
-    else if (hd) launch_ln_bwd<NP, EXACT, true, false>(a, blocks, dyd, outd, s);
-    else if (hm) launch_ln_bwd<NP, EXACT, false, true>(a, blocks, dyd, outd, s);
-    else launch_ln_bwd<NP, EXACT, false, false>(a, blocks, dyd, outd, s);
-}
-
-extern "C" int vlp_layernorm_bwd(const vlp_layernorm_bwd_args* a, void* stream) {
-    VLP_CHECK_ARG(a && a->dy && a->x && a->gamma && a->mean && a->rstd && a->dx && a->dgamma && a->dbeta, "vlp_layernorm_bwd: null operand");
-    VLP_ENTER(a->dy, "vlp_layernorm_bwd");
+    if (hd && hm) launch_ln_bwd<NP, EXACT, true, true, LIST>(a, blocks, dyd, outd, s, live, lflags);
+    else if (hd) launch_ln_bwd<NP, EXACT, true, false, LIST>(a, blocks, dyd, outd, s, live, lflags);
+    else if (hm) launch_ln_bwd<NP, EXACT, false, true, LIST>(a, blocks, dyd, outd, s, live, lflags);
+    else launch_ln_bwd<NP, EXACT, false, false, LIST>(a, blocks, dyd, outd, s, live, lflags);
+}
+
+static int ln_bwd_launch(const vlp_layernorm_bwd_args* a, const int32_t* live, int lflags, int part_M, void* stream) {
     VLP_CHECK_ARG(a->M > 0 && a->H > 0 && a->H % 8 == 0 && a->H <= 2048, "vlp_layernorm_bwd: H=%d must be a multiple of 8 and <= 2048", a->H);
     VLP_CHECK_ARG(a->lddy % 8 == 0 && a->ldx % 8 == 0 && a->lddx % 8 == 0, "vlp_layernorm_bwd: leading dims");
     VLP_CHECK_ARG(((uintptr_t)a->dy | (uintptr_t)a->x | (uintptr_t)a->dx | (uintptr_t)a->gamma) % 16 == 0, "vlp_layernorm_bwd: alignment");
@@ -354,9 +391,15 @@
     if (!a->workspace || a->workspace_bytes < need) return vlp_set_error(VLP_ERR_WORKSPACE, "vlp_layernorm_bwd: workspace %lld < %lld", (long long)a->workspace_bytes, (long long)need);
     const DropCtx dyd = make_drop(a->dy_drop_p, a->dy_seed, a->dy_stream);
     const DropCtx outd = make_drop(a->out_drop_p, a->out_seed, a->out_stream);
-    const int blocks = lnb_blocks(a->M);
+    const int blocks = lnb_blocks(live ? part_M : a->M);
     hipStream_t s = (hipStream_t)stream;
-    if (a->H == 768) launch_ln_bwd<3, true>(a, blocks, dyd, outd, s);
+    if (live) {
+        if (a->H == 768) launch_ln_bwd<3, true, true>(a, blocks, dyd, outd, s, live, lflags);
+        else if (a->H <= 768) launch_ln_bwd<3, false, true>(a, blocks, dyd, outd, s, live, lflags);
+        else if (a->H <= 1024) launch_ln_bwd<4, false, true>(a, blocks, dyd, outd, s, live, lflags);
+        else launch_ln_bwd<8, false, true>(a, blocks, dyd, outd, s, live, lflags);
+    }
+    else if (a->H == 768) launch_ln_bwd<3, true>(a, blocks, dyd, outd, s);
     else if (a->H <= 768) launch_ln_bwd<3, false>(a, blocks, dyd, outd, s);
     else if (a->H <= 1024) launch_ln_bwd<4, false>(a, blocks, dyd, outd, s);
     else launch_ln_bwd<8, false>(a, blocks, dyd, outd, s);
@@ -366,6 +409,19 @@
                        (f16*)a->dbeta, a->beta);
     VLP_CHECK_LAUNCH("vlp_layernorm_bwd_reduce");
     return VLP_OK;
+}
+
+extern "C" int vlp_layernorm_bwd(const vlp_layernorm_bwd_args* a, void* stream) {
+    VLP_CHECK_ARG(a && a->dy && a->x && a->gamma && a->mean && a->rstd && a->dx && a->dgamma && a->dbeta, "vlp_layernorm_bwd: null operand");
+    VLP_ENTER(a->dy, "vlp_layernorm_bwd");
+    return ln_bwd_launch(a, nullptr, 0, 0, stream);
+}
+
+extern "C" int vlp_layernorm_bwd_rows(const vlp_layernorm_bwd_args* a, const int32_t* live, int32_t flags, int32_t part_M, void* stream) {
+    VLP_CHECK_ARG(a && a->dy && a->x && a->gamma && a->mean && a->rstd && a->dx && a->dgamma && a->dbeta && live, "vlp_layernorm_bwd_rows: null operand");
+    VLP_ENTER(a->dy, "vlp_layernorm_bwd_rows");
+    VLP_CHECK_ARG((flags & ~(VLP_ROWS_X | VLP_ROWS_Y)) == 0 && part_M > 0, "vlp_layernorm_bwd_rows: bad flags %d / part_M %d", flags, part_M);
+    return ln_bwd_launch(a, live, flags, part_M, stream);
 }
 
 extern "C" int vlp_layernorm_bwd_reduce_batched(const float* parts, const void* const* dst, int32_t count, int32_t M, int32_t H, int32_t beta, void* stream) {
diff --git a/vlp_amd/engine.py b/vlp_amd/engine.py
--- a/vlp_amd/engine.py
+++ b/vlp_amd/engine.py
@@ -100,6 +100,7 @@
         self._pk_cache = {}
         self._pk_lens = {}
         self.last_packed_rows = None
+        self._live_n = None
 
     def _ordered_names(self, model):
         cfg = model.config
@@ -303,6 +304,8 @@
             ws.update(sel=h(R, H), tz=h(R, H), tg=h(R, H), tln=h(R, H), tstat=(f(R), f(R)), logits=h(R, Vp), dlogits=h(R, Vp),
                       dlT=h(Vp, _ru(R, 64)),
                       lse_ce=f(R), coef=f(R), row_loss=f(R), dtln=h(R, H), dtg=h(R, H), dtz=h(R, H), dsel=h(R, H))
+            ws.update(lv_rows=torch.empty(R, device=dev, dtype=torch.int32), lv_n=torch.zeros(1, device=dev, dtype=torch.int32),
+                      lv_dpre2=h(R, H), lv_dpre2_d=h(R, H), lv_dz=h(R, I), lv_dx1=h(R, H), lv_dpre1_d=h(R, H))
         ws["loss"] = f(260)
         if model.tasks == "vqa2":
             NA = model.num_answers
@@ -1141,9 +1144,57 @@
         var, sp = self._tn_splits(a, b, c, M, N, Kd, ws)
         K.gemm_tn(a, b, c, M, N, Kd, beta=beta, workspace=ws[ws_key], variant=var, bias_out=bias, splits=sp, **kw)
 
+    @property
+    def last_live_rows(self):
+        return None if self._live_n is None else int(self._live_n.item())
+
     def _bucket_done(self, idx):
         if self.grad_ready_hook is not None:
             self.grad_ready_hook(idx)
+
+    def _layer_bwd_live(self, i, st, ws, sh, ds, live, R, M, rm, ro, beta, grouped, on_side, use_side, side, ln_slot, scale):
+        model = self._model()
+        cfg = model.config
+        H, I, A = cfg.hidden_size, cfg.intermediate_size, cfg.num_attention_heads
+        B, L, seed = st.B, st.L, st.seed
+        p, pa = st.p_drop
+        Ln = "bert.encoder.layer.%d." % i
+        a, s = ws["layers"][i], sh["layers"][i]
+        x_in = ws["layers"][i - 1]["x2"] if i > 0 else ws["x0"]
+        dx, dctx, dpre1 = ws["dx"], ws["dctx"], ds["dpre1"]
+        K.layernorm_bwd_rows(dx, a["pre2"], self.P(Ln + "output.LayerNorm.weight"), a["st2"][0], a["st2"][1], ws["lv_dpre2"],
+                             self.G(Ln + "output.LayerNorm.weight"), self.G(Ln + "output.LayerNorm.bias"), live, K.ROWS_X, R, H, ln_slot(2 * i + 1), M,
+                             beta=beta, dx_drop=ws["lv_dpre2_d"] if p > 0 else None, out_drop=(p, seed, 16 * i + 3), defer_reduce=True, row_map=rm)
+        dy2 = ws["lv_dpre2_d"] if p > 0 else ws["lv_dpre2"]
+        K.gemm_nt_rows(dy2, s["w2T"], ws["lv_dz"], live, K.ROWS_MUL, R, I, H, mul_src=a["z"], mul_mode=K.MUL_PLAIN)
+        K.gemm_nt_rows(ws["lv_dz"], s["w1T"], ws["lv_dx1"], live, 0, R, H, I, residual=ws["lv_dpre2"])
+        K.layernorm_bwd_rows(ws["lv_dx1"], a["pre1"], self.P(Ln + "attention.output.LayerNorm.weight"), a["st1"][0], a["st1"][1], dpre1,
+                             self.G(Ln + "attention.output.LayerNorm.weight"), self.G(Ln + "attention.output.LayerNorm.bias"), live, K.ROWS_Y, R, H,
+                             ln_slot(2 * i), M, beta=beta, dx_drop=ws["lv_dpre1_d"] if p > 0 else None, out_drop=(p, seed, 16 * i + 2),
+                             defer_reduce=True, row_map=rm)
+        dy1, dy1_fl = (ws["lv_dpre1_d"], 0) if p > 0 else (dpre1, K.ROWS_X)
+        K.gemm_nt_rows(dy1, s["oT"], dctx, live, dy1_fl | K.ROWS_Y, R, H, H)
+        dqkv = ds["dqkv"]
+        K.attn_bwd(a["qkv"], ws["maskb"], ws["maskt"], a["ctx"], dctx, a["lse"], dqkv, ws["delta"], B, L, A, scale, dropout_p=pa, seed=seed,
+                   rng_stream=16 * i + 1, row_off=ro)
+
+        def last_wgrad():
+            listed = [(dy2, a["g"], self.G(Ln + "output.dense.weight"), R, H, I, beta, self.G(Ln + "output.dense.bias"), live, 0),
+                      (ws["lv_dz"], a["x1"], self.G(Ln + "intermediate.dense.weight"), R, I, H, beta, self.G(Ln + "intermediate.dense.bias"), live, 0),
+                      (dy1, a["ctx"], self.G(Ln + "attention.output.dense.weight"), R, H, H, beta, self.G(Ln + "attention.output.dense.bias"), live, dy1_fl)]
+            qkv = (dqkv, x_in, self.G(Ln + "attention.self.query.weight"), M, 3 * H, H, beta, self.G(Ln + "attention.self.query.bias"))
+            if grouped:
+                K.gemm_tn_grouped_rows(listed[:2] + [qkv + (None, 0)] + listed[2:])
+            else:
+                K.gemm_tn_grouped_rows(listed)
+                self._tn(*qkv[:6], ws, beta, bias=qkv[7])
+            self._bucket_done(cfg.num_hidden_layers - i)
+            if use_side:
+                ev = torch.cuda.Event()
+                ev.record(side)
+                self._side_done[i & 1] = ev
+        on_side(last_wgrad)
+        self._nt(dqkv, s["qkvT"], dx, M, H, 3 * H, residual=dpre1)
 
     def backward(self, st, gscale, task, g_pretext=None, g_rows=None):
         if st.gen != self.gen:
@@ -1193,6 +1244,21 @@
         if use_side:
             self._side_busy = True
         head_wgrads = []
+
+        live = live_ready = None
+        if (task != "vqa2" and task != "logprob" and st.has_mlm and P > 0 and st.pretext is None
+                and os.environ.get("VLP_LAST_LAYER_LIVE", "1") != "0"):
+            live, Rl = ws["lv_rows"], B * P
+
+            def live_prologue():
+                K.live_rows_build(masked_pos.contiguous(), B, P, L, live, ws["lv_n"], row_off=ro)
+                ws["dctx"][:M].zero_()
+                ws["dyset"][(NL - 1) & 1]["dpre1"][:M].zero_()
+            on_side(live_prologue)
+            if use_side:
+                live_ready = torch.cuda.Event()
+                live_ready.record(side)
+        self._live_n = ws["lv_n"] if live is not None else None
 
         if task == "vqa2":
             NA, NAp = model.num_answers, ws["NAp"]
@@ -1271,6 +1337,11 @@
             ds = ws["dyset"][i & 1]
             if use_side and self._side_done[i & 1] is not None:
                 main.wait_event(self._side_done[i & 1])
+            if live is not None and i == NL - 1:
+                if live_ready is not None:
+                    main.wait_event(live_ready)
+                self._layer_bwd_live(i, st, ws, sh, ds, live, Rl, M, rm, ro, beta, grouped, on_side, use_side, side, ln_slot, scale)
+                continue
             dpre = ds["dpre2"]
             K.layernorm_bwd(dx, a["pre2"], self.P(Ln + "output.LayerNorm.weight"), a["st2"][0], a["st2"][1], dpre,
                             self.G(Ln + "output.LayerNorm.weight"), self.G(Ln + "output.LayerNorm.bias"), M, H, ln_slot(2 * i + 1), beta=beta,
```

Result: faster. 6893 samples/s, median of 6 (+1.0%).
